# ilovepose/fast-human-pose-estimation.pytorch

Hardware: AMD Instinct MI355X
Metric: images/sec FPD train step (4-stack HG student, 8-stack teacher) 256x256 (higher is better)
Workload: dtype bf16; 1 GPU; configs[1]: hourglass student S=4 F=128 + teacher S=8 F=256, 256x256, batch 32/GPU, fused FPD step incl. Adam, teacher forward one batch ahead on a 2nd stream; global_batch=32, parallelism=dp1, backend=mfma, launch=one native plan call per phase, kernels launched eagerly on 3 streams, ranks=1, finite=True

## Files before the change

### fast-human-pose-estimation.pytorch_amd/csrc/api.hip

```cpp
#include <cstdarg>
#include <cstdio>
#include <cstdlib>
#include <cstring>
#include <string>
#include <vector>

#include "conv_dispatch.h"

int g_fpd_backend = FPD_BACKEND_MFMA;
static thread_local char g_err[512] = "";

static FILE* g_launch_log_file = nullptr;
static bool launch_log_open() {
    const char* path = getenv("FPD_LAUNCH_LOG");
    if (path == nullptr || path[0] == 0) return false;
    g_launch_log_file = fopen(path, "w");
    if (g_launch_log_file == nullptr) fprintf(stderr, "[fpd_amd] FPD_LAUNCH_LOG: cannot open %s\n", path);
    return g_launch_log_file != nullptr;
}
bool g_fpd_launch_log = launch_log_open();
static thread_local char g_op_tag[256] = "-";
void fpd_log_launch(const char* kernel, const dim3& grid, const dim3& block) {
    if (g_launch_log_file == nullptr) return;
    fprintf(g_launch_log_file, "%s\t%u\t%u\t%s\n", kernel, grid.x * grid.y * grid.z, block.x * block.y * block.z, g_op_tag);
// ... 16 lines not shown

static int validate_conv_dims(int N, int H, int W, int C, int K, int R, int S, int stride, int pad, int P, int Q) {
    FPD_REQUIRE(N > 0 && H > 0 && W > 0 && C > 0 && K > 0 && R > 0 && S > 0 && stride > 0 && pad >= 0,
                "conv: non-positive dimension");
    FPD_REQUIRE(P == (H + 2 * pad - R) / stride + 1 && Q == (W + 2 * pad - S) / stride + 1,
                "conv: output %dx%d inconsistent with input %dx%d k=%dx%d stride=%d pad=%d", P, Q, H, W, R, S, stride, pad);
    FPD_REQUIRE((int64_t)N * H * W * C < (1ll << 31) && (int64_t)N * P * Q * K < (1ll << 31), "conv: tensor too large for 32-bit indexing");
    return 0;
}

int fpd_bneck_blocks_option(int value);
int fpd_head_blocks_option(int value);

extern "C" {

const char* fpd_last_error(void) { return g_err; }
int fpd_abi_version(void) { return FPD_ABI_VERSION; }
int64_t fpd_stats_words(int32_t channels) { return FPD_STATS_WORDS(channels); }
int fpd_set_backend(int32_t backend) {
    const int prev = g_fpd_backend;
    if (backend == FPD_BACKEND_MFMA || backend == FPD_BACKEND_NAIVE || backend == FPD_BACKEND_MFMA_GENERIC) g_fpd_backend = backend;
    return prev;
}

static int g_wgrad_tile_only = 0;

int fpd_set_option(const char* name, int32_t value) {
    FPD_REQUIRE(name, "set_option: null name");
    if (!strcmp(name, "conv_pp")) return fpd_conv_pp_option(0, value);
    if (!strcmp(name, "conv_pp_blocks")) return fpd_conv_pp_option(1, value);
    if (!strcmp(name, "conv_c1")) return fpd_conv_c1_option(0, value);
    if (!strcmp(name, "conv_c1_blocks")) return fpd_conv_c1_option(1, value);
    if (!strcmp(name, "conv_c1_launches")) return fpd_conv_c1_option(2, value);
    if (!strcmp(name, "conv_c3")) return fpd_conv_c3_option(0, value);
    if (!strcmp(name, "conv_c3_blocks")) return fpd_conv_c3_option(1, value);
    if (!strcmp(name, "conv_c3_launches")) return fpd_conv_c3_option(2, value);
    if (!strcmp(name, "bneck_blocks")) return fpd_bneck_blocks_option(value);
    if (!strcmp(name, "head_blocks")) return fpd_head_blocks_option(value);
    if (!strcmp(name, "wgrad_tile_only")) { g_wgrad_tile_only = value; return 0; }
    return fpd_fail(-2, "set_option: unknown option '%s'", name);
}

int fpd_abi_sizeof(const char* n) {
#define SZ(T) if (!strcmp(n, #T)) return (int)sizeof(T)
    SZ(fpd_bn_t); SZ(fpd_conv_t); SZ(fpd_wgrad_t); SZ(fpd_stem_t); SZ(fpd_ew_t); SZ(fpd_loss_t); SZ(fpd_adam_t);
    SZ(fpd_wprep_entry_t); SZ(fpd_bnupd_entry_t); SZ(fpd_memset_t); SZ(fpd_table_t); SZ(fpd_wreduce_entry_t); SZ(fpd_bneck_t); SZ(fpd_conv_pair_t); SZ(fpd_bneck_pair_t); SZ(fpd_ew_pair_t); SZ(fpd_pck_t); SZ(fpd_head_t); SZ(fpd_affsum_t); SZ(fpd_layout_t);
    SZ(fpd_conv_f8_t); SZ(fpd_wquant_entry_t); SZ(fpd_flipmerge_t); SZ(fpd_finalpreds_t); SZ(fpd_targets_t); SZ(fpd_warp_src_t); SZ(fpd_warp_t);
    SZ(fpd_loss_ohkm_t); SZ(fpd_sgd_t);
#undef SZ
    return -1;
}

static int validate_conv(const fpd_conv_t* a) {
    FPD_REQUIRE(a && a->x && a->w && a->y, "conv: null pointer");
    int rc = validate_conv_dims(a->N, a->H, a->W, a->C, a->K, a->R, a->S, a->stride, a->pad, a->P, a->Q);
    if (rc) return rc;
    FPD_REQUIRE(a->dtype == FPD_F32 || a->dtype == FPD_BF16, "conv: bad dtype %d", a->dtype);
    FPD_REQUIRE(a->bn.mode == FPD_BN_NONE || (a->bn.gamma && a->bn.beta), "conv: BN prologue without gamma/beta");
    FPD_REQUIRE(a->bn.mode != FPD_BN_TRAIN || a->bn.stats, "conv: train-mode BN without statistics");
    FPD_REQUIRE(a->bn.mode != FPD_BN_EVAL || (a->bn.running_mean && a->bn.running_var), "conv: eval-mode BN without running stats");
    FPD_REQUIRE(a->epi == FPD_EPI_PLAIN || (a->epi_x && a->epi_stats && a->epi_bn.mode == FPD_BN_TRAIN && a->epi_bn.stats),
                "conv: BNRELU_BWD epilogue needs epi_x, epi_stats and a train-mode epi_bn");
    return 0;
}

constexpr unsigned ON_MFMA = 1u << FPD_BACKEND_MFMA, ON_GENERIC = ON_MFMA | 1u << FPD_BACKEND_MFMA_GENERIC, ON_ANY = ON_GENERIC | 1u << FPD_BACKEND_NAIVE;
struct ConvBackend {
    const char* name;
    unsigned backends;
    int (*route)(const fpd_conv_t& a, const fpd_conv_t* b, ConvAsk ask, ConvRoute& r);
    int (*launch)(const fpd_conv_t& a, const fpd_conv_t* b, hipStream_t st);
};
static const ConvBackend g_conv_backends[] = {
    {"conv_c1", ON_MFMA, fpd_conv_c1_route, fpd_conv_c1_launch},
    {"conv_c3", ON_MFMA, fpd_conv_c3_route, fpd_conv_c3_launch},
    {"conv_pp", ON_MFMA, fpd_conv_pp_route, fpd_conv_pp_launch},
    {"conv_tile", ON_MFMA, fpd_conv_tile_route, fpd_conv_tile_launch},
    {"conv_mfma", ON_GENERIC, nullptr, [](const fpd_conv_t& a, const fpd_conv_t*, hipStream_t st) { return fpd_conv_mfma_launch(a, st); }},
    {"conv_smallc", ON_GENERIC, nullptr, [](const fpd_conv_t& a, const fpd_conv_t*, hipStream_t st) { return fpd_conv_smallc_launch(a, st); }},
    {"conv_naive", ON_ANY, nullptr, [](const fpd_conv_t& a, const fpd_conv_t*, hipStream_t st) { return fpd_conv_naive_launch(a, st); }},
};
static bool eligible(unsigned backends) { return (backends >> g_fpd_backend & 1u) != 0; }

static const ConvBackend* route_conv(const fpd_conv_t& a, const fpd_conv_t* b, ConvAsk ask, ConvRoute& r) {
    r = ConvRoute{false, 0, 0};
    for (const ConvBackend& e : g_conv_backends) {
        if (!eligible(e.backends)) continue;
        if (e.route == nullptr ? b == nullptr : e.route(a, b, ask, r) == 0) return &e;
    }
    return nullptr;
}

static int launch_conv(const fpd_conv_t& a, const fpd_conv_t* b, hipStream_t st) {
    ConvRoute r;
    const ConvBackend* e = route_conv(a, b, fpd_conv_ask(a, b), r);
    if (e == nullptr) {
        const int rc = launch_conv(a, nullptr, st);
        return rc ? rc : launch_conv(*b, nullptr, st);
    }
    FPD_REQUIRE(!(a.wg_partial != nullptr && r.slabs_a == 0) && !(b != nullptr && b->wg_partial != nullptr && r.slabs_b == 0),
                "conv: the launch asks for a fused weight gradient (wg_partial), which its route (%s) does not offer; %s() reports 0 for it",
                e->name, b ? "fpd_conv_pair_fused_wgrad_partials" : "fpd_conv_fused_wgrad_partials");
    FPD_REQUIRE(r.folds || (a.fold_x == nullptr && (b == nullptr || b->fold_x == nullptr)),
                "conv: the launch asks for a folded BN-backward apply (fold_x), which its route (%s) does not offer; %s() reports 0 for it",
                e->name, b ? "fpd_conv_pair_fold_supported" : "fpd_conv_fold_supported");
    int rc = e->launch(a, b, st);
    for (++e; rc == 1 && e != std::end(g_conv_backends); ++e)
        if (e->route == nullptr && eligible(e->backends)) rc = e->launch(a, b, st);
    return rc;
}

int fpd_conv_forward(const fpd_conv_t* a, fpd_stream_t stream) {
    int rc = validate_conv(a);
    if (rc) return rc;
    rc = launch_conv(*a, nullptr, (hipStream_t)stream);
    return rc ? rc : check_launch();
}

int fpd_conv_fold_supported(const fpd_conv_t* a) {
    ConvRoute r;
    if (!a || validate_conv(a) != 0) return 0;
    route_conv(*a, nullptr, ConvAsk{true, a->wg_partial != nullptr}, r);
    return r.folds ? 1 : 0;
}
int fpd_conv_pair_fold_supported(const fpd_conv_pair_t* p) {
    ConvRoute r;
    if (!p || validate_conv(&p->a) != 0 || validate_conv(&p->b) != 0) return 0;
    if (route_conv(p->a, &p->b, ConvAsk{true, fpd_conv_ask(p->a, &p->b).wg}, r) != nullptr) return r.folds ? 1 : 0;
    return (fpd_conv_fold_supported(&p->a) && fpd_conv_fold_supported(&p->b)) ? 1 : 0;
}

int fpd_conv_fused_wgrad_partials(const fpd_conv_t* a) {
    ConvRoute r;
    if (!a || validate_conv(a) != 0) return 0;
    route_conv(*a, nullptr, ConvAsk{a->fold_x != nullptr, true}, r);
    return r.slabs_a;
}
int fpd_conv_pair_fused_wgrad_partials(const fpd_conv_pair_t* p, int32_t* n_a, int32_t* n_b) {
    FPD_REQUIRE(p && n_a && n_b, "conv_pair_fused_wgrad_partials: null pointer");
    *n_a = *n_b = 0;
    if (validate_conv(&p->a) != 0 || validate_conv(&p->b) != 0) return 0;
    ConvRoute r;
    route_conv(p->a, &p->b, ConvAsk{fpd_conv_ask(p->a, &p->b).fold, true}, r);
    *n_a = r.slabs_a; *n_b = r.slabs_b;
    return 0;
}

int fpd_conv_f8_in_domain(const fpd_conv_t* c) { return (c && fpd_conv_f8_domain(*c)) ? 1 : 0; }

int fpd_conv_forward_f8(const fpd_conv_f8_t* a, fpd_stream_t stream) {
    FPD_REQUIRE(a, "conv_f8: null pointer");
    int rc = validate_conv(&a->c);
    if (rc) return rc;
    FPD_REQUIRE(a->w8 && a->w8_scale, "conv_f8: null fp8 weights / scales");
    FPD_REQUIRE(((uintptr_t)a->w8 & 15) == 0, "conv_f8: w8 must be 16-byte aligned");
    rc = 1;
    if (g_fpd_backend == FPD_BACKEND_MFMA) rc = fpd_conv_tile_f8_launch(a->c, a->w8, a->w8_scale, (hipStream_t)stream);
    if (rc == 1) rc = launch_conv(a->c, nullptr, (hipStream_t)stream);
    return rc ? rc : check_launch();
}

int fpd_weight_quant_f8(const fpd_wquant_entry_t* t, int32_t n, fpd_stream_t stream) {
    FPD_REQUIRE(n == 0 || t != nullptr, "weight_quant_f8: null table");
    int rc = fpd_weight_quant_f8_launch(t, n, (hipStream_t)stream);
    return rc ? rc : check_launch();
}

int fpd_conv_forward_pair(const fpd_conv_pair_t* p, fpd_stream_t stream) {
    FPD_REQUIRE(p, "conv_pair: null pointer");
    int rc = validate_conv(&p->a);
    if (rc) return rc;
    rc = validate_conv(&p->b);
    if (rc) return rc;
    rc = launch_conv(p->a, &p->b, (hipStream_t)stream);
    return rc ? rc : check_launch();
}

static int validate_bneck_bns(const fpd_bneck_t* a) {
    const fpd_bn_t* bns[3] = {&a->bn1, &a->bn2, &a->bn3};
    for (int i = 0; i < 3; ++i)
        FPD_REQUIRE(bns[i]->mode == FPD_BN_EVAL && bns[i]->relu && bns[i]->gamma && bns[i]->beta && bns[i]->running_mean &&
                    bns[i]->running_var, "bottleneck: bn%d must be an eval-mode BN+ReLU with running statistics", i + 1);
    return 0;
}

int fpd_bottleneck_fold(const fpd_bneck_t* a, fpd_stream_t stream) {
    FPD_REQUIRE(a && a->folded, "bottleneck_fold: null pointer");
    int rc = validate_bneck_bns(a);
    if (rc) return rc;
    rc = fpd_bneck_fold_launch(*a, const_cast<float*>(a->folded), (hipStream_t)stream);
    if (rc == 1) return fpd_fail(-3, "bottleneck_fold: C=%d P=%d is outside the fused kernel's domain", a->C, a->P);
    return rc ? rc : check_launch();
}

int fpd_bottleneck_forward_pair(const fpd_bneck_pair_t* p, fpd_stream_t stream) {
    FPD_REQUIRE(p, "bottleneck_pair: null pointer");
    const fpd_bneck_t* ab[2] = {&p->a, &p->b};
    for (const fpd_bneck_t* a : ab) {
        FPD_REQUIRE(a->x && a->y && a->w1 && a->w2 && a->w3 && a->x != a->y, "bottleneck_pair: null pointer or y aliases x");
        FPD_REQUIRE((int64_t)a->N * a->H * a->W * a->C < ((int64_t)1 << 31), "bottleneck_pair: tensor too large for 32-bit indexing");
        int rc = validate_bneck_bns(a);
        if (rc) return rc;
    }
    int rc = fpd_bneck_fused_pair_launch(p->a, p->b, (hipStream_t)stream);
    if (rc == 1) {
        rc = fpd_bottleneck_forward(&p->a, stream);
// ... 23 lines not shown
};
static const WgradBackend g_wgrad_backends[] = {
    {ON_MFMA, fpd_wgrad_tile_partials, fpd_wgrad_tile_launch},
    {ON_GENERIC, fpd_wgrad_mfma_partials, fpd_wgrad_mfma_launch},
    {ON_GENERIC, fpd_wgrad_smallc_partials, fpd_wgrad_smallc_launch},
    {ON_ANY, fpd_wgrad_naive_partials, fpd_wgrad_naive_launch},
};

int fpd_conv_wgrad(const fpd_wgrad_t* a, fpd_stream_t stream) {
    FPD_REQUIRE(a && a->x && a->dy && a->dw, "wgrad: null pointer");
    int rc = validate_conv_dims(a->N, a->H, a->W, a->C, a->K, a->R, a->S, a->stride, a->pad, a->P, a->Q);
    if (rc) return rc;
    FPD_REQUIRE(a->dtype == FPD_F32 || a->dtype == FPD_BF16, "wgrad: bad dtype %d", a->dtype);
    FPD_REQUIRE(a->partial == nullptr || a->partial_stride >= (int64_t)a->K * a->R * a->S * a->C + a->K,
                "wgrad: partial_stride %lld smaller than weight + bias", (long long)a->partial_stride);
    rc = 1;
    for (const WgradBackend& e : g_wgrad_backends) {
        FPD_REQUIRE(!(g_wgrad_tile_only && &e != g_wgrad_backends), "wgrad: option wgrad_tile_only is set and the halo-tile kernel declines N=%d H=%d W=%d C=%d K=%d R=%d", a->N, a->H, a->W, a->C, a->K, a->R);
        if (eligible(e.backends)) rc = e.launch(*a, (hipStream_t)stream);
        if (rc != 1) break;
    }
    return rc ? rc : check_launch();
}

int fpd_wgrad_num_partials(const fpd_wgrad_t* a) {
    int n = 0;
    for (const WgradBackend& e : g_wgrad_backends)
        if (a && n == 0 && eligible(e.backends)) n = e.partials(*a);
    return n;
}

struct StemBackend {
    unsigned backends;
    int (*forward)(const fpd_stem_t& a, hipStream_t st);
    int (*wgrad_partials)(const fpd_stem_t& a);
    int (*wgrad)(const fpd_stem_t& a, hipStream_t st);
};
static const StemBackend g_stem_backends[] = {
    {ON_MFMA, fpd_stem_forward_s2d_launch, fpd_stem_wgrad_s2d_partials, fpd_stem_wgrad_s2d_launch},
    {ON_MFMA, fpd_stem_forward_mfma_launch, fpd_stem_wgrad_mfma_partials, fpd_stem_wgrad_mfma_launch},
    {ON_ANY, fpd_stem_forward_launch, fpd_stem_wgrad_partials, fpd_stem_wgrad_launch},
};

int fpd_stem_wgrad_num_partials(const fpd_stem_t* a) {
    int n = 0;
    for (const StemBackend& e : g_stem_backends)
        if (a && n == 0 && eligible(e.backends)) n = e.wgrad_partials(*a);
    return n;
}

int fpd_wgrad_reduce(const fpd_wreduce_entry_t* t, int32_t n, int64_t max_elems, fpd_stream_t stream) {
    int rc = fpd_wreduce_launch(t, n, max_elems, (hipStream_t)stream);
    return rc ? rc : check_launch();
}

int fpd_stem_forward(const fpd_stem_t* a, fpd_stream_t stream) {
    FPD_REQUIRE(a && a->x && a->w && a->bias && a->y, "stem: null pointer");
    FPD_REQUIRE(a->P == (a->H + 6 - 7) / 2 + 1 && a->Q == (a->W + 6 - 7) / 2 + 1, "stem: bad output size");
    int rc = 1;
    for (const StemBackend& e : g_stem_backends)
        if (rc == 1 && eligible(e.backends)) rc = e.forward(*a, (hipStream_t)stream);
    return rc ? rc : check_launch();
}

int fpd_stem_wgrad(const fpd_stem_t* a, fpd_stream_t stream) {
    FPD_REQUIRE(a && a->x && a->dy && a->dw, "stem wgrad: null pointer");
    FPD_REQUIRE(a->partial == nullptr || a->partial_stride >= (int64_t)a->K * 148, "stem wgrad: partial_stride %lld smaller than weight + bias",
                (long long)a->partial_stride);
    int rc = 1;
    for (const StemBackend& e : g_stem_backends)
        if (rc == 1 && eligible(e.backends)) rc = e.wgrad(*a, (hipStream_t)stream);
    return rc ? rc : check_launch();
}

int fpd_affsum(const fpd_affsum_t* a, fpd_stream_t stream) {
    FPD_REQUIRE(a && a->y, "affsum: null pointer");
    FPD_REQUIRE(a->nterms >= 1 && a->nterms <= FPD_AFFSUM_MAX, "affsum: %d terms (1..%d supported)", a->nterms, FPD_AFFSUM_MAX);
    FPD_REQUIRE(a->dtype == FPD_F32 || a->dtype == FPD_BF16, "affsum: bad dtype %d", a->dtype);
    for (int j = 0; j < a->nterms; ++j) {
        const int up = a->t[j].up;
        FPD_REQUIRE(a->t[j].x, "affsum: term %d has no input", j);
        FPD_REQUIRE((up == 1 || up == 2 || up == 4 || up == 8) && a->H % up == 0 && a->W % up == 0,
                    "affsum: term %d: up-sampling factor %d does not divide %dx%d", j, up, a->H, a->W);
        const fpd_bn_t& bn = a->t[j].bn;
        FPD_REQUIRE(bn.mode == FPD_BN_NONE || (bn.gamma && bn.beta), "affsum: term %d: BN without gamma/beta", j);
        FPD_REQUIRE(bn.mode != FPD_BN_TRAIN || bn.stats, "affsum: term %d: train-mode BN without statistics", j);
        FPD_REQUIRE(bn.mode != FPD_BN_EVAL || (bn.running_mean && bn.running_var), "affsum: term %d: eval-mode BN without running stats", j);
    }
    int rc = fpd_affsum_launch(*a, (hipStream_t)stream);
    return rc ? rc : check_launch();
}
// ... 227 lines not shown
    memcpy(&o.u, args, want);
    p->ops.push_back(o);
    p->sched.emplace_back();
    return (int)p->ops.size() - 1;
}

int fpd_plan_set_schedule(fpd_plan* p, int32_t op, int32_t lane, const int32_t* wait_ops, int32_t n_waits) {
    FPD_REQUIRE(p && op >= 0 && op < (int)p->ops.size(), "plan_set_schedule: bad op index %d", op);
    FPD_REQUIRE(lane >= 0 && lane < FPD_MAX_LANES, "plan_set_schedule: lane %d outside [0,%d)", lane, FPD_MAX_LANES);
    FPD_REQUIRE(n_waits >= 0 && (n_waits == 0 || wait_ops != nullptr), "plan_set_schedule: bad wait list");
    for (int i = 0; i < n_waits; ++i)
        FPD_REQUIRE(wait_ops[i] >= 0 && wait_ops[i] < op, "plan_set_schedule: op %d may only wait for earlier ops (got %d)", op, wait_ops[i]);
    fpd_sched& s = p->sched[op];
    s.lane = lane;
    s.waits.assign(wait_ops, wait_ops + n_waits);
    for (int i = 0; i < n_waits; ++i) p->sched[wait_ops[i]].record = true;
    return 0;
}

int fpd_plan_mark_event(fpd_plan* p, int32_t op) {
    FPD_REQUIRE(p && op >= 0 && op < (int)p->ops.size(), "plan_mark_event: bad op index %d", op);
    p->sched[op].record = true;
    return 0;
}

int fpd_plan_wait_op(fpd_plan* p, int32_t op, fpd_stream_t stream) {
    FPD_REQUIRE(p && op >= 0 && op < (int)p->ops.size(), "plan_wait_op: bad op index %d", op);
    FPD_REQUIRE(p->sched[op].record && p->sched[op].done, "plan_wait_op: op %d has no recorded event (mark it, then run its range)", op);
    FPD_CHECK_HIP(hipStreamWaitEvent((hipStream_t)stream, p->sched[op].done, 0));
    return 0;
}

static void conv_tag(char* p, size_t n, const char* what, const fpd_conv_t& c) {
    snprintf(p, n, "%s N=%d H=%d W=%d C=%d K=%d R=%d s=%d %s%s%s%s", what, c.N, c.H, c.W, c.C, c.K, c.R, c.stride,
             c.epi == FPD_EPI_BNRELU_BWD ? "dgrad" : "fwd", c.bn.mode == FPD_BN_EVAL ? " evalbn" : "", c.wg_partial ? " +wgrad" : "", c.fold_x ? " +fold" : "");
}
static void set_op_tag(int idx, const fpd_op& o) {
    char t[200] = "";
    static const char* ew_names[] = {"bnrelu_fwd", "bnrelu_bwd_r", "bn_bwd_apply", "maxpool_fwd", "maxpool_bwd", "upadd_fwd", "sumpool", "add", "relu_mask", "dilate2"};
    auto ewn = [&](int op) { return (op >= 0 && op < 10) ? ew_names[op] : "ew"; };
    switch (o.type) {
        case FPD_OP_CONV: conv_tag(t, sizeof(t), "conv", o.u.conv); break;
        case FPD_OP_CONV_F8: conv_tag(t, sizeof(t), "conv_f8", o.u.conv8.c); break;
        case FPD_OP_CONV_PAIR: {
            char a[90], b[90];
            conv_tag(a, sizeof(a), "conv2", o.u.pair.a);
            snprintf(b, sizeof(b), " | H=%d W=%d", o.u.pair.b.H, o.u.pair.b.W);
            snprintf(t, sizeof(t), "%s%s", a, b);
            break;
        }
        case FPD_OP_WGRAD: snprintf(t, sizeof(t), "wgrad N=%d H=%d W=%d C=%d K=%d R=%d s=%d", o.u.wgrad.N, o.u.wgrad.H, o.u.wgrad.W, o.u.wgrad.C, o.u.wgrad.K, o.u.wgrad.R, o.u.wgrad.stride); break;
        case FPD_OP_BNECK: snprintf(t, sizeof(t), "bneck N=%d H=%d W=%d C=%d P=%d", o.u.bneck.N, o.u.bneck.H, o.u.bneck.W, o.u.bneck.C, o.u.bneck.P); break;
        case FPD_OP_BNECK_PAIR: snprintf(t, sizeof(t), "bneck2 N=%d H=%d W=%d C=%d P=%d | H=%d W=%d", o.u.bpair.a.N, o.u.bpair.a.H, o.u.bpair.a.W, o.u.bpair.a.C, o.u.bpair.a.P, o.u.bpair.b.H, o.u.bpair.b.W); break;
        case FPD_OP_HEAD: snprintf(t, sizeof(t), "head N=%d H=%d W=%d C=%d J=%d", o.u.head.N, o.u.head.H, o.u.head.W, o.u.head.C, o.u.head.J); break;
        case FPD_OP_EW: snprintf(t, sizeof(t), "ew %s N=%d H=%d W=%d C=%d", ewn(o.u.ew.op), o.u.ew.N, o.u.ew.H, o.u.ew.W, o.u.ew.C); break;
        case FPD_OP_EW_PAIR: snprintf(t, sizeof(t), "ew2 %s N=%d H=%d W=%d C=%d | H=%d W=%d", ewn(o.u.epair.a.op), o.u.epair.a.N, o.u.epair.a.H, o.u.epair.a.W, o.u.epair.a.C, o.u.epair.b.H, o.u.epair.b.W); break;
        case FPD_OP_STEM_FWD: case FPD_OP_STEM_WGRAD: snprintf(t, sizeof(t), "%s N=%d H=%d W=%d K=%d", o.type == FPD_OP_STEM_FWD ? "stem_fwd" : "stem_wgrad", o.u.stem.N, o.u.stem.H, o.u.stem.W, o.u.stem.K); break;
        case FPD_OP_AFFSUM: snprintf(t, sizeof(t), "affsum N=%d H=%d W=%d C=%d terms=%d", o.u.affsum.N, o.u.affsum.H, o.u.affsum.W, o.u.affsum.C, o.u.affsum.nterms); break;
        case FPD_OP_LOSS: snprintf(t, sizeof(t), "loss B=%d J=%d H=%d W=%d S=%d", o.u.loss.B, o.u.loss.J, o.u.loss.H, o.u.loss.W, o.u.loss.S); break;
        case FPD_OP_LOSS_OHKM: snprintf(t, sizeof(t), "loss_ohkm B=%d J=%d H=%d W=%d S=%d k=%d,%d", o.u.lossk.base.B, o.u.lossk.base.J, o.u.lossk.base.H, o.u.lossk.base.W, o.u.lossk.base.S, o.u.lossk.topk_pose, o.u.lossk.topk_kd); break;
        case FPD_OP_ADAM: snprintf(t, sizeof(t), "adam n=%lld", (long long)o.u.adam.n); break;
        case FPD_OP_SGD: snprintf(t, sizeof(t), "sgd n=%lld momentum=%g wd=%g%s", (long long)o.u.sgd.n, (double)o.u.sgd.momentum, (double)o.u.sgd.weight_decay, o.u.sgd.nesterov ? " nesterov" : ""); break;
        case FPD_OP_WREDUCE: snprintf(t, sizeof(t), "wreduce entries=%d", o.u.table.n); break;
        case FPD_OP_WPREP: snprintf(t, sizeof(t), "wprep entries=%d", o.u.table.n); break;
        case FPD_OP_BNUPD: snprintf(t, sizeof(t), "bnupd entries=%d", o.u.table.n); break;
        default: snprintf(t, sizeof(t), "op%d", o.type); break;
    }
    snprintf(g_op_tag, sizeof(g_op_tag), "%d\t%s", idx, t);
}

static int run_op(const fpd_op& o, fpd_stream_t s) {
    switch (o.type) {
        case FPD_OP_CONV: return fpd_conv_forward(&o.u.conv, s);
        case FPD_OP_CONV_F8: return fpd_conv_forward_f8(&o.u.conv8, s);
        case FPD_OP_WQUANT: return fpd_weight_quant_f8((const fpd_wquant_entry_t*)o.u.table.table, o.u.table.n, s);
        case FPD_OP_WGRAD: return fpd_conv_wgrad(&o.u.wgrad, s);
        case FPD_OP_CONV_PAIR: return fpd_conv_forward_pair(&o.u.pair, s);
        case FPD_OP_BNECK_PAIR: return fpd_bottleneck_forward_pair(&o.u.bpair, s);
        case FPD_OP_EW_PAIR: return fpd_elementwise_pair(&o.u.epair, s);
        case FPD_OP_PCK: return fpd_pck(&o.u.pck, s);
        case FPD_OP_HEAD: return fpd_head_forward(&o.u.head, s);
        case FPD_OP_HEAD_FOLD: return fpd_head_fold(&o.u.head, s);
        case FPD_OP_BNECK: return fpd_bottleneck_forward(&o.u.bneck, s);
        case FPD_OP_BNECK_FOLD: return fpd_bottleneck_fold(&o.u.bneck, s);
        case FPD_OP_STEM_FWD: return fpd_stem_forward(&o.u.stem, s);
        case FPD_OP_STEM_WGRAD: return fpd_stem_wgrad(&o.u.stem, s);
        case FPD_OP_EW: return fpd_elementwise(&o.u.ew, s);
        case FPD_OP_LOSS: return fpd_loss(&o.u.loss, s);
        case FPD_OP_LOSS_OHKM: return fpd_loss_ohkm(&o.u.lossk, s);
        case FPD_OP_ADAM: return fpd_adam(&o.u.adam, s);
// ... 118 lines not shown
```

### fast-human-pose-estimation.pytorch_amd/csrc/conv_c1.hip

```cpp
#include <algorithm>
#include <cstdlib>
#include <type_traits>

#include "conv_dispatch.h"
#include "mfma_frag.h"

namespace {

constexpr int C1_NW = 8;

typedef short s16x2 __attribute__((ext_vector_type(2)));
__device__ __forceinline__ f32x2 c1_unpack(unsigned w) {
    f32x2 r = {__uint_as_float(w << 16), __uint_as_float(w & 0xffff0000u)};
    return r;
}
__device__ __forceinline__ unsigned c1_pack(f32x2 v) { return f2bf_pk(v[0], v[1]); }
__device__ __forceinline__ unsigned c1_floor(unsigned w, short lo) {
    s16x2 a = *reinterpret_cast<const s16x2*>(&w);
    const s16x2 b = {lo, lo};
    a = __builtin_elementwise_max(a, b);
    return *reinterpret_cast<const unsigned*>(&a);
}

template <int C, int K, bool BWD, bool WG>
struct C1Geo {
    static constexpr int CV = C / 8, KV = K / 8;
    static constexpr int NV = C / 16, NK = K / 16;
    static constexpr int KT = K / 32, KS = C / 16;
    static constexpr int PXA = C * 2 + 16, PXO = K * 2 + 16;
    static constexpr int TILE_A = 32 * PXA, TILE_O = 32 * PXO;
    static constexpr int WAVE_LDS = WG ? TILE_A + TILE_O : (TILE_A > TILE_O ? TILE_A : TILE_O);
    static constexpr int FLUSH = C1_NW * 64 * 16 * 4 + C1_NW * K * 4 + 8 * 2 * K * 8;
    static constexpr int REGION = C1_NW * WAVE_LDS > FLUSH ? C1_NW * WAVE_LDS : FLUSH;
    static constexpr int TABLES = (2 * C + (BWD ? 3 * C + 4 * K : 0) + K) * 4;
    static constexpr int LDS = TABLES + K * C * 2 + REGION;
    static constexpr int NT = (C / 32) * (K / 32);
    static constexpr int NTW = NT / C1_NW;
    static_assert(!WG || (BWD && NT % C1_NW == 0 && NTW >= 1), "fused weight gradient: every wave owns whole tiles of dW");
    static_assert(64 % CV == 0 && 64 % KV == 0, "a lane keeps its channel chunk");
};

#define C1_PHASE() do { asm volatile("" ::: "memory"); __builtin_amdgcn_sched_barrier(0); } while (0)

#ifdef FPD_C1_TIMING
#define C1_STAMP() do { if (lane == 0 && (wave == 0 || wave == 7) && c1_ns < 40) c1_stamp[(wave ? 40 : 0) + c1_ns++] = clock64(); } while (0)
#else
#define C1_STAMP() do { } while (0)
#endif

template <int C, int K, bool BWD, bool FOLD, bool WG, bool RES>
__device__ __forceinline__ void c1_body(const fpd_conv_t& a, const int bi, const int nblk) {
    using G = C1Geo<C, K, BWD, WG>;
    constexpr int CV = G::CV, KV = G::KV, NV = G::NV, NK = G::NK, KT = G::KT, KS = G::KS, PXA = G::PXA, PXO = G::PXO;
    constexpr int RPB = CV >= 16 ? 1 : 16 / CV;
    extern __shared__ __attribute__((aligned(16))) unsigned char smem[];

    const int tid = threadIdx.x, lane = tid & 63, l31 = lane & 31, hh = lane >> 5;
    const int wave = __builtin_amdgcn_readfirstlane(tid >> 6);
    const int M = a.N * a.H * a.W;
    const int ntile = M >> 5;
    const int nround = (ntile + C1_NW - 1) / C1_NW;
    const int r_beg = fpd_cut(bi, nround, nblk), r_end = fpd_cut(bi + 1, nround, nblk);

    float* s_scale = reinterpret_cast<float*>(smem);
    float* s_shift = s_scale + C;
    float* s_fold = s_shift + C;
    float* s_epi = s_fold + (BWD ? 3 * C : 0);
    float* s_bias = s_epi + (BWD ? 4 * K : 0);
    unsigned char* sW = reinterpret_cast<unsigned char*>(s_bias + K);
    unsigned char* sT = sW + K * C * 2;
    unsigned char* tA = sT + wave * G::WAVE_LDS;
    unsigned char* tO = WG ? tA + G::TILE_A : tA;

    const bf16_t* __restrict__ x = reinterpret_cast<const bf16_t*>(a.x);
    const bf16_t* __restrict__ w = reinterpret_cast<const bf16_t*>(a.w);
    bf16_t* y = reinterpret_cast<bf16_t*>(a.y);
    const bf16_t* res = reinterpret_cast<const bf16_t*>(a.residual);
    const bf16_t* ex = reinterpret_cast<const bf16_t*>(a.epi_x);
    const bf16_t* __restrict__ fx = reinterpret_cast<const bf16_t*>(a.fold_x != nullptr ? a.fold_x : a.x);
    const bool fold = FOLD && a.fold_x != nullptr;
    bf16_t* fo = fold ? reinterpret_cast<bf16_t*>(a.fold_out) : nullptr;
    const bool has_bn = !BWD && a.bn.mode != FPD_BN_NONE;
    constexpr bool has_res = RES;
    const bool want_stats = BWD || a.out_stats != nullptr;
    const bool wg = WG && a.wg_partial != nullptr;
    const bool wg_bias = wg && a.wg_bias;
#ifdef FPD_C1_TIMING
    long long* c1_stamp = reinterpret_cast<long long*>(smem + G::LDS);
    int c1_ns = 0;
#endif
    C1_STAMP();

    BnRaw braw;
    float bias_raw;
    const int te = tid - 128, tb = tid - 256;
    const bool r_bn = has_bn && tid < C;
    const bool r_fold = fold && tid < C;
    const bool r_epi = BWD && te >= 0 && te < K;
    const bool r_bias = tb >= 0 && tb < K;
    StatRaw fs1, fs2;
    if (r_bn) bn_request(a.bn, tid, C, braw);
    else if (r_fold) {
        bn_request(a.fold_bn, tid, C, braw);
        stat_request(a.fold_stats, C, 0, tid, fs1);
        stat_request(a.fold_stats, C, 1, tid, fs2);
    }
    else if (r_epi) bn_request(a.epi_bn, te, K, braw);
    else if (r_bias) { bias_raw = 0.f; if (a.bias != nullptr) bias_raw = a.bias[tb]; }
    __builtin_amdgcn_sched_barrier(0);

    uint4 rx[NV];
    uint4 ru[FOLD ? NV : 1];
    uint4 rr[NK];
    auto load_x = [&](int t) {
        const uint4* px = reinterpret_cast<const uint4*>(x) + ((size_t)t * 32 * CV + lane);
#pragma unroll
        for (int i = 0; i < NV; ++i) rx[i] = px[i * 64];
        if constexpr (FOLD) {
            const uint4* pu = reinterpret_cast<const uint4*>(fx) + ((size_t)t * 32 * CV + lane);
#pragma unroll
            for (int i = 0; i < NV; ++i) ru[i] = pu[i * 64];
        }
    };
    auto load_r = [&](int t) {
        const uint4* pr = reinterpret_cast<const uint4*>(BWD ? ex : res) + ((size_t)t * 32 * KV + lane);
#pragma unroll
        for (int i = 0; i < NK; ++i) rr[i] = pr[i * 64];
    };
    int tile = r_beg * C1_NW + wave;
    {
        constexpr int NWV = (K * CV + 511) / 512;
        uint4 rw[NWV];
#pragma unroll
        for (int i = 0; i < NWV; ++i) {
            const int v = tid + i * 512;
            rw[i] = make_uint4(0, 0, 0, 0);
            if (v < K * CV) rw[i] = *reinterpret_cast<const uint4*>(w + (size_t)v * 8);
        }
        __builtin_amdgcn_sched_barrier(0);
        {
            const int t0 = min(tile, ntile - 1);
            load_x(t0);
            if constexpr (BWD || has_res) load_r(t0);
        }
        __builtin_amdgcn_sched_barrier(0);
        if (r_bn) {
            float sc, sh, mu, is;
            bn_resolve(braw, (double)M, sc, sh, mu, is);
            s_scale[tid] = sc;
            s_shift[tid] = sh;
        } else if (r_fold) {
            const double s1 = stat_resolve(braw.s1), s2 = stat_resolve(braw.s2), b1 = stat_resolve(fs1), b2 = stat_resolve(fs2);
            const double cnt = (double)M, mu = s1 / cnt;
            double var = s2 / cnt - mu * mu;
            if (var < 0.0) var = 0.0;
            const double is = 1.0 / sqrt(var + (double)braw.eps), gi = (double)braw.g * is;
            const double m1 = b1 / cnt, m2 = b2 / cnt;
            s_fold[tid] = (float)gi;
            s_fold[C + tid] = (float)(-gi * is * m2);
            s_fold[2 * C + tid] = (float)(gi * (mu * is * m2 - m1));
            if (bi == 0) {
                if (a.fold_dgamma != nullptr) a.fold_dgamma[tid] = (float)b2;
                if (a.fold_dbeta != nullptr) a.fold_dbeta[tid] = (float)b1;
            }
        } else if (r_epi) {
            float sc, sh, mu, is;
            bn_resolve(braw, (double)M, sc, sh, mu, is);
            s_epi[te] = sc; s_epi[K + te] = sh; s_epi[2 * K + te] = mu; s_epi[3 * K + te] = is;
        } else if (r_bias) {
            s_bias[tb] = bias_raw;
        }
#pragma unroll
        for (int i = 0; i < NWV; ++i) {
            const int v = tid + i * 512;
            if (v < K * CV) {
                const int k = v / CV, ch = v % CV;
                const int sw = (k / RPB) & (CV - 1);
                *reinterpret_cast<uint4*>(sW + (k * CV + (ch ^ sw)) * 16) = rw[i];
            }
        }
    }
    C1_STAMP();
    __syncthreads();
    C1_STAMP();

    const int cch = lane % CV, kch = lane % KV;
    const int pxa0 = lane / CV, pxo0 = lane / KV;
    f32x2 p_sc[4], p_sh[4];
    if (has_bn) {
#pragma unroll
        for (int e = 0; e < 4; ++e) {
            p_sc[e] = *reinterpret_cast<const f32x2*>(s_scale + cch * 8 + 2 * e);
            p_sh[e] = *reinterpret_cast<const f32x2*>(s_shift + cch * 8 + 2 * e);
        }
    }
    const short relu_floor = a.bn.relu ? (short)0 : (short)-32768;
    const short epi_floor = a.epi_bn.relu ? (short)0 : (short)-32768;
    const float relu_gate = a.epi_bn.relu ? 0.f : -3.4e38f;
    f32x2 F1[4], F2[4], CS[4];
#pragma unroll
    for (int e = 0; e < 4; ++e) { F1[e] = f32x2{0.f, 0.f}; F2[e] = f32x2{0.f, 0.f}; CS[e] = f32x2{0.f, 0.f}; }
    const int wsw = (l31 / RPB) & (CV - 1);
    f32x16 wacc[WG ? G::NTW : 1], bacc[WG ? G::NTW : 1];
#pragma unroll
    for (int j = 0; j < (WG ? G::NTW : 1); ++j)
#pragma unroll
        for (int e = 0; e < 16; ++e) { wacc[j][e] = 0.f; bacc[j][e] = 0.f; }

    auto stage = [&](const int t, auto modec) {
        constexpr int MODE = decltype(modec)::value;
        f32x2 f_a[4], f_b[4], f_d[4];
// ... 3 lines not shown
                f_a[e] = *reinterpret_cast<const f32x2*>(s_fold + cch * 8 + 2 * e);
                f_b[e] = *reinterpret_cast<const f32x2*>(s_fold + C + cch * 8 + 2 * e);
                f_d[e] = *reinterpret_cast<const f32x2*>(s_fold + 2 * C + cch * 8 + 2 * e);
            }
        }
#pragma unroll
        for (int i = 0; i < NV; ++i) {
            uint4 val = rx[i];
            if constexpr (MODE == 2) {
                const uint4 uu = ru[i];
                const unsigned gw[4] = {val.x, val.y, val.z, val.w}, uw[4] = {uu.x, uu.y, uu.z, uu.w};
                unsigned ow[4];
#pragma unroll
                for (int e = 0; e < 4; ++e) {
                    const f32x2 tt = __builtin_elementwise_fma(f_b[e], c1_unpack(uw[e]), f_d[e]);
                    ow[e] = c1_pack(__builtin_elementwise_fma(f_a[e], c1_unpack(gw[e]), tt));
                }
                val = make_uint4(ow[0], ow[1], ow[2], ow[3]);
            } else if constexpr (MODE == 1) {
                val.x = c1_floor(c1_pack(__builtin_elementwise_fma(c1_unpack(val.x), p_sc[0], p_sh[0])), relu_floor);
                val.y = c1_floor(c1_pack(__builtin_elementwise_fma(c1_unpack(val.y), p_sc[1], p_sh[1])), relu_floor);
                val.z = c1_floor(c1_pack(__builtin_elementwise_fma(c1_unpack(val.z), p_sc[2], p_sh[2])), relu_floor);
                val.w = c1_floor(c1_pack(__builtin_elementwise_fma(c1_unpack(val.w), p_sc[3], p_sh[3])), relu_floor);
            }
            rx[i] = val;
            *reinterpret_cast<uint4*>(tA + (pxa0 + i * (64 / CV)) * PXA + cch * 16) = val;
        }
        if (MODE == 2 && fo != nullptr) {
            uint4* po = reinterpret_cast<uint4*>(fo) + ((size_t)t * 32 * CV + lane);
#pragma unroll
            for (int i = 0; i < NV; ++i) po[i * 64] = rx[i];
        }
    };
    auto finish = [&](const f32x16& accv, const int kt, auto resc) {
        constexpr bool HASRES = decltype(resc)::value;
        {
#pragma unroll
            for (int q = 0; q < 4; ++q) {
                unsigned char* p = tO + l31 * PXO + (kt * 32 + 8 * q + 4 * hh) * 2;
                f32x2 v0 = {accv[4 * q], accv[4 * q + 1]}, v1 = {accv[4 * q + 2], accv[4 * q + 3]};
                if constexpr (!BWD) {
                    if constexpr (HASRES) {
                        const uint2 r2 = *reinterpret_cast<const uint2*>(p);
                        v0 += c1_unpack(r2.x);
                        v1 += c1_unpack(r2.y);
                    }
                    const f32x4 b4 = *reinterpret_cast<const f32x4*>(s_bias + kt * 32 + 8 * q + 4 * hh);
                    v0 += f32x2{b4[0], b4[1]};
                    v1 += f32x2{b4[2], b4[3]};
                }
                *reinterpret_cast<uint2*>(p) = make_uint2(c1_pack(v0), c1_pack(v1));
            }
        }
    };
    auto perchan = [&](const int t, const bool first, auto statc) {
        constexpr bool STATS = decltype(statc)::value;
        uint4* py = reinterpret_cast<uint4*>(y) + ((size_t)t * 32 * KV + lane);
        f32x2 e_sc[4], e_sh[4], e_mu[4], e_is[4];
        if constexpr (BWD) {
#pragma unroll
            for (int e = 0; e < 4; ++e) {
                e_sc[e] = *reinterpret_cast<const f32x2*>(s_epi + kch * 8 + 2 * e);
                e_sh[e] = *reinterpret_cast<const f32x2*>(s_epi + K + kch * 8 + 2 * e);
                e_mu[e] = *reinterpret_cast<const f32x2*>(s_epi + 2 * K + kch * 8 + 2 * e);
                e_is[e] = *reinterpret_cast<const f32x2*>(s_epi + 3 * K + kch * 8 + 2 * e);
            }
        }
        if (!BWD && STATS && first) {
            const uint4 c4 = *reinterpret_cast<const uint4*>(tO + kch * 16);
            CS[0] = c1_unpack(c4.x); CS[1] = c1_unpack(c4.y); CS[2] = c1_unpack(c4.z); CS[3] = c1_unpack(c4.w);
        }
#pragma unroll
        for (int i = 0; i < NK; ++i) {
            unsigned char* p = tO + (pxo0 + i * (64 / KV)) * PXO + kch * 16;
            const uint4 o4 = *reinterpret_cast<const uint4*>(p);
            unsigned ow[4] = {o4.x, o4.y, o4.z, o4.w};
            if constexpr (BWD) {
                const unsigned xw[4] = {rr[i].x, rr[i].y, rr[i].z, rr[i].w};
                unsigned aw[4];
#pragma unroll
// ... 47 lines not shown
            for (int h = 0; h < 2; ++h) {
#pragma unroll
                for (int j = 0; j < (WG ? G::NTW : 1); ++j) {
                    wacc[j] = __builtin_amdgcn_mfma_f32_32x32x16_bf16(af[b][h][j], bfr[b][h][j], wacc[j], 0, 0, 0);
                    if constexpr (BIAS) bacc[j] = __builtin_amdgcn_mfma_f32_32x32x16_bf16(af[b][h][j], ones, bacc[j], 0, 0, 0);
                }
            }
        };
        if (round * C1_NW + C1_NW <= ntile) {
            wg_frags(0, af[0], bfr[0]);
#pragma unroll
            for (int s = 0; s < C1_NW; ++s) {
                if (s + 1 < C1_NW) wg_frags(s + 1, af[(s + 1) & 1], bfr[(s + 1) & 1]);
                mult(s & 1);
                __builtin_amdgcn_sched_barrier(0);
            }
        } else {
#pragma unroll 1
            for (int s = 0; s < C1_NW; ++s) {
                if (round * C1_NW + s < ntile) {
                    wg_frags(s, af[0], bfr[0]);
                    mult(0);
                }
            }
        }
    };

    bool first = true;
    for (int round = r_beg; round < r_end; ++round) {
        tile = round * C1_NW + wave;
        const bool live = tile < ntile;
        const bool pf = round + 1 < r_end && tile + C1_NW < ntile;
        if (live) {
            if (FOLD && fold) { if constexpr (FOLD) stage(tile, std::integral_constant<int, 2>{}); }
            else if (has_bn) { if constexpr (!BWD) stage(tile, std::integral_constant<int, 1>{}); }
            else stage(tile, std::integral_constant<int, 0>{});
            if (pf) load_x(tile + C1_NW);
            C1_PHASE();
            C1_STAMP();
            bf16x8 bf[KS];
#pragma unroll
            for (int kk = 0; kk < KS; ++kk) bf[kk] = *reinterpret_cast<const bf16x8*>(tA + l31 * PXA + kk * 32 + hh * 16);
            if constexpr (has_res) {
                C1_PHASE();
#pragma unroll
                for (int i = 0; i < NK; ++i)
                    *reinterpret_cast<uint4*>(tO + (pxo0 + i * (64 / KV)) * PXO + kch * 16) = make_uint4(rr[i].x, rr[i].y, rr[i].z, rr[i].w);
                C1_PHASE();
            }
#pragma unroll
            for (int k0 = 0; k0 < KT; k0 += 2) {
                f32x16 acc0, acc1;
#pragma unroll
                for (int e = 0; e < 16; ++e) { acc0[e] = 0.f; acc1[e] = 0.f; }
                const unsigned char* wrow0 = sW + (k0 * 32 + l31) * (C * 2);
#pragma unroll
                for (int kk = 0; kk < KS; ++kk) {
                    const bf16x8 wf0 = *reinterpret_cast<const bf16x8*>(wrow0 + ((2 * kk + hh) ^ wsw) * 16);
                    acc0 = __builtin_amdgcn_mfma_f32_32x32x16_bf16(wf0, bf[kk], acc0, 0, 0, 0);
                    if (k0 + 1 < KT) {
                        const bf16x8 wf1 = *reinterpret_cast<const bf16x8*>(wrow0 + 32 * (C * 2) + ((2 * kk + hh) ^ wsw) * 16);
                        acc1 = __builtin_amdgcn_mfma_f32_32x32x16_bf16(wf1, bf[kk], acc1, 0, 0, 0);
                    }
                }
                finish(acc0, k0, std::integral_constant<bool, has_res>{});
                if (k0 + 1 < KT) finish(acc1, k0 + 1, std::integral_constant<bool, has_res>{});
            }
            if constexpr (!BWD && has_res) { if (pf) load_r(tile + C1_NW); }
            C1_PHASE();
            C1_STAMP();
            if (want_stats) perchan(tile, first, std::true_type{}); else perchan(tile, first, std::false_type{});
            if (BWD && pf) load_r(tile + C1_NW);
            C1_PHASE();
            C1_STAMP();
            first = false;
        }
        if (WG) {
            __syncthreads();
            if (wg) {
                if (wg_bias && (wave % KT) == 0) wg_round(round, std::true_type{}); else wg_round(round, std::false_type{});
            }
            __syncthreads();
            C1_STAMP();
        }
    }
    C1_STAMP();

    if (WG && wg) {
        float* slab = a.wg_partial + (size_t)bi * a.wg_stride;
#pragma unroll
        for (int j = 0; j < (WG ? G::NTW : 1); ++j) {
            const int tw = wave + C1_NW * j, ci = tw / KT, ko = tw % KT;
#pragma unroll
            for (int e = 0; e < 16; ++e) {
                const int row = ci * 32 + (e & 3) + 8 * (e >> 2) + 4 * hh;
                slab[(size_t)row * K + ko * 32 + l31] = wacc[j][e];
                if (wg_bias && ko == 0 && l31 == 0) slab[(size_t)C * K + row] = bacc[j][e];
            }
        }
// ... 43 lines not shown
                    }
                }
                s_part[part * 2 * K + rem] = tot;
            }
        }
        __syncthreads();
        if (tid < 2 * K) {
            double tot = 0.0;
#pragma unroll
            for (int q = 0; q < NPART; ++q) tot += s_part[q * 2 * K + tid];
            stat_atomic_add(st, K, tid / K, tid % K, tot);
        }
    }
#ifdef FPD_C1_TIMING
    C1_STAMP();
    if (lane == 0 && (wave == 0 || wave == 7)) c1_stamp[(wave ? 40 : 0) + 39] = c1_ns;
    __syncthreads();
    if (tid == 0 && (blockIdx.x == 0 || blockIdx.x == gridDim.x / 2 + 1)) {
        for (int wv = 0; wv < 2; ++wv) {
            const long long* sp = c1_stamp + wv * 40;
            const long long t0 = c1_stamp[0];
            long long d[16];
            for (int q = 0; q < 16; ++q) d[q] = q < (int)sp[39] ? sp[q] - t0 : -1;
            printf("conv_c1 C=%d K=%d bwd %d fold %d wg %d blk %d wave %d rounds %d: %lld %lld %lld | %lld %lld %lld %lld | %lld %lld %lld %lld | %lld %lld %lld %lld %lld\n",
                   C, K, (int)BWD, (int)FOLD, (int)WG, (int)blockIdx.x, wv * 7, r_end - r_beg,
                   d[0], d[1], d[2], d[3], d[4], d[5], d[6], d[7], d[8], d[9], d[10], d[11], d[12], d[13], d[14], d[15]);
        }
    }
#endif
}

struct C1Args { fpd_conv_t c[2]; int nblk[2]; };

template <int C, int K, bool BWD, bool FOLD, bool WG, bool RES>
__global__ __launch_bounds__(512, 2) void c1_kernel(const C1Args p) {
    const int bid = blockIdx.x, n = gridDim.x, nb = p.nblk[1];
    const int fb0 = fpd_cut(bid, nb, n), fb1 = fpd_cut(bid + 1, nb, n);
    const int isb = fb1 > fb0 ? 1 : 0;
    const int u = isb ? fb0 : bid - fb0;
    c1_body<C, K, BWD, FOLD, WG, RES>(p.c[isb], u, p.nblk[isb]);
}

int g_c1_mode = -1, g_c1_blocks = -1;
std::atomic<int> g_c1_launches{0};
int c1_mode() {
    if (g_c1_mode < 0) { const char* e = getenv("FPD_C1"); g_c1_mode = e ? atoi(e) : 1; }
    return g_c1_mode;
}
int c1_blocks() {
    if (g_c1_blocks < 0) { const char* e = getenv("FPD_C1_BLOCKS"); g_c1_blocks = e ? atoi(e) : 192; }
    return g_c1_blocks < 1 ? 1 : g_c1_blocks;
}
int c1_min_px() {
    static int v = -1;
    if (v < 0) { const char* e = getenv("FPD_C1_MIN_PX"); v = e ? atoi(e) : 512; }
    return v;
}
int c1_min_px_bwd() {
    static int v = -1;
    if (v < 0) { const char* e = getenv("FPD_C1_MIN_PX_BWD"); v = e ? atoi(e) : 2048; }
    return v;
}
int c1_fuse_wgrad() { return 1; }

bool c1_chan(int c) { return c == 32 || c == 64 || c == 128; }
bool c1_aligned(const void* p) { return (reinterpret_cast<uintptr_t>(p) & 15) == 0; }

bool c1_domain(const fpd_conv_t& a, bool fold) {
    if (a.dtype != FPD_BF16 || a.R != 1 || a.S != 1 || a.stride != 1 || a.pad != 0 || a.P != a.H || a.Q != a.W) return false;
    if (!(c1_chan(a.C) || (a.C == 16 && a.K == 128)) || !c1_chan(a.K)) return false;
    const long long M = (long long)a.N * a.H * a.W;
    if (M % 32 != 0 || M > (1ll << 30)) return false;
    if (!c1_aligned(a.x) || !c1_aligned(a.y) || !c1_aligned(a.w) || !c1_aligned(a.residual) || !c1_aligned(a.epi_x) ||
        !c1_aligned(a.fold_x) || !c1_aligned(a.fold_out)) return false;
    if (a.epi == FPD_EPI_BNRELU_BWD) {
        if (a.bias != nullptr || a.residual != nullptr || a.bn.mode != FPD_BN_NONE) return false;
        if (a.C == 16) { if (fold) return false; }
        else if ((a.C / 32) * (a.K / 32) != C1_NW && !(a.C == 128 && a.K == 128 && !fold)) return false;
    } else {
        if (a.epi != FPD_EPI_PLAIN || a.y == a.x) return false;
    }
    return true;
}
int c1_rounds(const fpd_conv_t& a) { return cdiv(a.N * a.H * a.W / 32, C1_NW); }

struct C1Plan { int na, nb, grid; bool wg; };
bool c1_route(const fpd_conv_t& a, const fpd_conv_t* b, ConvAsk ask, ConvRoute& r, C1Plan& pl) {
    const int mode = c1_mode();
    if (mode == 0 || !c1_domain(a, ask.fold)) return false;
    const bool bwd = a.epi == FPD_EPI_BNRELU_BWD;
    long long px = (long long)a.N * a.H * a.W;
    if (b != nullptr) {
        if (!c1_domain(*b, ask.fold) || a.K != b->K || a.C != b->C || a.epi != b->epi) return false;
        if ((a.residual != nullptr) != (b->residual != nullptr)) return false;
        px += (long long)b->N * b->H * b->W;
    }
    if (mode == 1 && px < (bwd ? c1_min_px_bwd() : c1_min_px())) return false;
    const int ra = c1_rounds(a), rb = b ? c1_rounds(*b) : 0;
    int total = std::max(1, std::min(c1_blocks(), ra + rb));
    total = cdiv(ra + rb, cdiv(ra + rb, total));
    pl.nb = 0;
    if (b != nullptr) {
        if (total < 2) return false;
        pl.nb = std::max(1, std::min(total - 1, (int)((long long)total * rb / (ra + rb))));
    }
    pl.na = total - pl.nb;
    pl.grid = total;
    pl.wg = ask.wg && c1_fuse_wgrad() != 0 && bwd && (a.C / 32) * (a.K / 32) == C1_NW;
    r.folds = ask.fold && bwd;
    r.slabs_a = pl.wg ? pl.na : 0;
    r.slabs_b = pl.wg ? pl.nb : 0;
    return true;
}

template <int C, int K, bool BWD, bool FOLD, bool WG, bool RES>
int c1_launch_t(const fpd_conv_t& a, const fpd_conv_t* b, const C1Plan& pl, hipStream_t st) {
    static LdsAttr configured;
#ifdef FPD_C1_TIMING
    constexpr size_t lds = C1Geo<C, K, BWD, WG>::LDS + 1024;
#else
    constexpr size_t lds = C1Geo<C, K, BWD, WG>::LDS;
#endif
    static_assert(lds <= 160 * 1024, "conv_c1: LDS budget");
    if (int rc_ = configured.ensure(reinterpret_cast<const void*>(&c1_kernel<C, K, BWD, FOLD, WG, RES>), lds)) return rc_;
    C1Args args;
    args.c[0] = a; args.c[1] = b ? *b : a; args.nblk[0] = pl.na; args.nblk[1] = pl.nb;
    FPD_LAUNCH((c1_kernel<C, K, BWD, FOLD, WG, RES>), dim3(pl.grid), dim3(512), lds, st, args);
    g_c1_launches.fetch_add(1, std::memory_order_relaxed);
    return 0;
}

template <int C, int K>
int c1_launch_ck(const fpd_conv_t& a, const fpd_conv_t* b, const C1Plan& pl, hipStream_t st) {
    if (a.epi == FPD_EPI_BNRELU_BWD) {
        if constexpr ((C / 32) * (K / 32) == C1_NW) {
            if (a.fold_x != nullptr || (b != nullptr && b->fold_x != nullptr))
                return pl.wg ? c1_launch_t<C, K, true, true, true, false>(a, b, pl, st) : c1_launch_t<C, K, true, true, false, false>(a, b, pl, st);
            return pl.wg ? c1_launch_t<C, K, true, false, true, false>(a, b, pl, st) : c1_launch_t<C, K, true, false, false, false>(a, b, pl, st);
        } else if constexpr (C == 16 || (C == 128 && K == 128)) {
            return c1_launch_t<C, K, true, false, false, false>(a, b, pl, st);
        } else {
            return 1;
        }
    }
    if (a.residual != nullptr) return c1_launch_t<C, K, false, false, false, true>(a, b, pl, st);
    return c1_launch_t<C, K, false, false, false, false>(a, b, pl, st);
}

template <int C>
int c1_launch_c(const fpd_conv_t& a, const fpd_conv_t* b, const C1Plan& pl, hipStream_t st) {
    switch (a.K) {
        case 32: return c1_launch_ck<C, 32>(a, b, pl, st);
        case 64: return c1_launch_ck<C, 64>(a, b, pl, st);
        default: return c1_launch_ck<C, 128>(a, b, pl, st);
    }
}

}

int fpd_conv_c1_option(int which, int value) {
    if (which == 2) return g_c1_launches.load(std::memory_order_relaxed);
    int& g = which == 0 ? g_c1_mode : g_c1_blocks;
    const int prev = which == 0 ? c1_mode() : c1_blocks();
    g = value;
    return prev;
}

int fpd_conv_c1_route(const fpd_conv_t& a, const fpd_conv_t* b, ConvAsk ask, ConvRoute& r) {
    C1Plan pl;
    return c1_route(a, b, ask, r, pl) ? 0 : 1;
}
int fpd_conv_c1_launch(const fpd_conv_t& a, const fpd_conv_t* b, hipStream_t st) {
    ConvRoute r;
    C1Plan pl;
    if (!c1_route(a, b, fpd_conv_ask(a, b), r, pl)) return 1;
    if (int rc = fpd_conv_check_slabs(a, r.slabs_a, "conv_c1")) return rc;
    if (b != nullptr) {
        if (int rc = fpd_conv_check_slabs(*b, r.slabs_b, "conv_c1")) return rc;
        FPD_REQUIRE((a.wg_partial == nullptr) == (b->wg_partial == nullptr), "conv_pair: both or neither convolution of a pair take a fused weight gradient");
    }
    switch (a.C) {
        case 16: return c1_launch_ck<16, 128>(a, b, pl, st);
        case 32: return c1_launch_c<32>(a, b, pl, st);
        case 64: return c1_launch_c<64>(a, b, pl, st);
        default: return c1_launch_c<128>(a, b, pl, st);
    }
}
```

### fast-human-pose-estimation.pytorch_amd/csrc/conv_c3.hip

```cpp
#include <algorithm>
#include <atomic>
#include <cstdlib>
#include <type_traits>

#include "conv_dispatch.h"

namespace {

constexpr int C3_NW = 8, C3_C = 64, C3_STRIP = 256;
constexpr int C3_CV = C3_C / 8;
constexpr int C3_NVH = 6;
constexpr int C3_NK = C3_C / 16;
constexpr int C3_WBYTES = 9 * C3_C * C3_C * 2;
constexpr int C3_TILE_O = 32 * C3_C * 2;
constexpr int C3_TABLES = (2 * C3_C + 3 * C3_C + 4 * C3_C + C3_C) * 4;
constexpr int C3_FLUSH = C3_NW * 64 * 16 * 4 + C3_NW * C3_C * 4 + 8 * 2 * C3_C * 8;

typedef short s16x2 __attribute__((ext_vector_type(2)));
typedef unsigned u32x4 __attribute__((ext_vector_type(4)));
__device__ __forceinline__ f32x2 c3_unpack(unsigned w) {
    f32x2 r = {__uint_as_float(w << 16), __uint_as_float(w & 0xffff0000u)};
    return r;
}
__device__ __forceinline__ unsigned c3_pack(f32x2 v) { return f2bf_pk(v[0], v[1]); }
// ... 420 lines not shown
    return g;
}
struct C3Plan { C3Geo ga, gb; int grid; size_t lds; };
bool c3_plan(const fpd_conv_t& a, const fpd_conv_t* b, C3Plan& pl) {
    pl.ga = c3_geo(a);
    pl.gb = b ? c3_geo(*b) : pl.ga;
    pl.gb.nblk = 0;
    const int sa = pl.ga.nstrip, sb = b ? pl.gb.nstrip : 0;
    int total = std::max(1, std::min(c3_blocks(), sa + sb));
    total = cdiv(sa + sb, cdiv(sa + sb, total));
    if (b != nullptr) {
        if (total < 2) return false;
        pl.gb.nblk = std::max(1, std::min(total - 1, (int)((long long)total * sb / (sa + sb))));
    }
    pl.ga.nblk = total - pl.gb.nblk;
    pl.grid = total;
    const int img = std::max(pl.ga.img_bytes, b ? pl.gb.img_bytes : 0);
    pl.ga.img_bytes = pl.gb.img_bytes = img;
    pl.lds = (size_t)C3_TABLES + C3_WBYTES + std::max(img + C3_NW * C3_TILE_O, C3_FLUSH);
    return pl.lds <= 160 * 1024;
}

template <bool BWD, bool FOLD>
int c3_launch_t(const fpd_conv_t& a, const fpd_conv_t* b, const C3Plan& pl, hipStream_t st) {
    static LdsAttr configured;
    if (int rc_ = configured.ensure(reinterpret_cast<const void*>(&c3_kernel<BWD, FOLD>), pl.lds)) return rc_;
    C3Args args;
    args.c[0] = a; args.c[1] = b ? *b : a; args.g[0] = pl.ga; args.g[1] = pl.gb;
    FPD_LAUNCH((c3_kernel<BWD, FOLD>), dim3(pl.grid), dim3(512), pl.lds, st, args);
    g_c3_launches.fetch_add(1, std::memory_order_relaxed);
    return 0;
}
bool c3_route(const fpd_conv_t& a, const fpd_conv_t* b, ConvAsk ask, ConvRoute& r, C3Plan& pl) {
    if (!c3_takes(a, b) || !c3_plan(a, b, pl)) return false;
    r = ConvRoute{ask.fold && a.epi == FPD_EPI_BNRELU_BWD, 0, 0};
    return true;
}

}

int fpd_conv_c3_option(int which, int value) {
    if (which == 2) return g_c3_launches.load(std::memory_order_relaxed);
    int& g = which == 0 ? g_c3_mode : g_c3_blocks;
    const int prev = which == 0 ? c3_mode() : c3_blocks();
    g = value;
    return prev;
}
int fpd_conv_c3_route(const fpd_conv_t& a, const fpd_conv_t* b, ConvAsk ask, ConvRoute& r) {
    C3Plan pl;
    return c3_route(a, b, ask, r, pl) ? 0 : 1;
}
int fpd_conv_c3_launch(const fpd_conv_t& a, const fpd_conv_t* b, hipStream_t st) {
    ConvRoute r;
    C3Plan pl;
    if (!c3_route(a, b, fpd_conv_ask(a, b), r, pl)) return 1;
    if (a.epi != FPD_EPI_BNRELU_BWD) return c3_launch_t<false, false>(a, b, pl, st);
    return r.folds ? c3_launch_t<true, true>(a, b, pl, st) : c3_launch_t<true, false>(a, b, pl, st);
}
```

### fast-human-pose-estimation.pytorch_amd/csrc/conv_dispatch.h

```cpp
#pragma once
#include "common.h"

struct ConvAsk { bool fold, wg; };
struct ConvRoute { bool folds; int slabs_a, slabs_b; };
inline ConvAsk fpd_conv_ask(const fpd_conv_t& a, const fpd_conv_t* b) {
    return ConvAsk{a.fold_x != nullptr || (b != nullptr && b->fold_x != nullptr), a.wg_partial != nullptr || (b != nullptr && b->wg_partial != nullptr)};
}
inline int fpd_conv_check_slabs(const fpd_conv_t& c, int slabs, const char* unit) {
    if (c.wg_partial == nullptr) return 0;
    FPD_REQUIRE(c.wg_stride >= (int64_t)c.C * c.K + c.C, "conv: wg_stride %lld smaller than weight + bias", (long long)c.wg_stride);
    FPD_REQUIRE(c.wg_count == slabs, "conv: the launch writes %d weight-gradient slabs but the caller sized its workspace for %d "
                "(fpd_conv_fused_wgrad_partials: has a %s option changed since?)", slabs, c.wg_count, unit);
    return 0;
}
int fpd_conv_c1_route(const fpd_conv_t& a, const fpd_conv_t* b, ConvAsk ask, ConvRoute& r);
int fpd_conv_c1_launch(const fpd_conv_t& a, const fpd_conv_t* b, hipStream_t st);
int fpd_conv_c3_route(const fpd_conv_t& a, const fpd_conv_t* b, ConvAsk ask, ConvRoute& r);
int fpd_conv_c3_launch(const fpd_conv_t& a, const fpd_conv_t* b, hipStream_t st);
int fpd_conv_pp_route(const fpd_conv_t& a, const fpd_conv_t* b, ConvAsk ask, ConvRoute& r);
int fpd_conv_pp_launch(const fpd_conv_t& a, const fpd_conv_t* b, hipStream_t st);
int fpd_conv_tile_route(const fpd_conv_t& a, const fpd_conv_t* b, ConvAsk ask, ConvRoute& r);
int fpd_conv_tile_launch(const fpd_conv_t& a, const fpd_conv_t* b, hipStream_t st);
int fpd_conv_c1_option(int which, int value);
int fpd_conv_c3_option(int which, int value);
int fpd_conv_pp_option(int which, int value);
int fpd_conv_mfma_launch(const fpd_conv_t& a, hipStream_t st);
int fpd_conv_smallc_launch(const fpd_conv_t& a, hipStream_t st);
int fpd_conv_naive_launch(const fpd_conv_t& a, hipStream_t st);
bool fpd_conv_f8_domain(const fpd_conv_t& a);
int fpd_conv_tile_f8_launch(const fpd_conv_t& a, const void* w8, const float* wscale, hipStream_t st);
int fpd_weight_quant_f8_launch(const fpd_wquant_entry_t* table, int n, hipStream_t st);

int fpd_wgrad_tile_partials(const fpd_wgrad_t& a);
int fpd_wgrad_tile_launch(const fpd_wgrad_t& a, hipStream_t st);
int fpd_wgrad_mfma_partials(const fpd_wgrad_t& a);
int fpd_wgrad_mfma_launch(const fpd_wgrad_t& a, hipStream_t st);
int fpd_wgrad_smallc_partials(const fpd_wgrad_t& a);
int fpd_wgrad_smallc_launch(const fpd_wgrad_t& a, hipStream_t st);
int fpd_wgrad_naive_partials(const fpd_wgrad_t& a);
int fpd_wgrad_naive_launch(const fpd_wgrad_t& a, hipStream_t st);
int fpd_wreduce_launch(const fpd_wreduce_entry_t* table, int n, int64_t max_elems, hipStream_t st);

int fpd_stem_forward_s2d_launch(const fpd_stem_t& a, hipStream_t st);
int fpd_stem_wgrad_s2d_partials(const fpd_stem_t& a);
int fpd_stem_wgrad_s2d_launch(const fpd_stem_t& a, hipStream_t st);
int fpd_stem_forward_mfma_launch(const fpd_stem_t& a, hipStream_t st);
int fpd_stem_wgrad_mfma_partials(const fpd_stem_t& a);
int fpd_stem_wgrad_mfma_launch(const fpd_stem_t& a, hipStream_t st);
int fpd_stem_forward_launch(const fpd_stem_t& a, hipStream_t st);
int fpd_stem_wgrad_partials(const fpd_stem_t& a);
int fpd_stem_wgrad_launch(const fpd_stem_t& a, hipStream_t st);

int fpd_bneck_fused_launch(const fpd_bneck_t& a, hipStream_t st);
int fpd_bneck_fused_pair_launch(const fpd_bneck_t& a, const fpd_bneck_t& b, hipStream_t st);
int fpd_bneck_fold_launch(const fpd_bneck_t& a, float* out, hipStream_t st);
int fpd_head_fused_launch(const fpd_head_t& a, hipStream_t st);
int fpd_head_fold_launch(const fpd_head_t& a, float* out, hipStream_t st);
int fpd_pck_launch(const fpd_pck_t& a, hipStream_t st);
int fpd_flip_w_launch(const float* x, float* y, int64_t rows, int W, hipStream_t st);
int fpd_flip_merge_launch(const fpd_flipmerge_t& p, hipStream_t st);
int fpd_final_preds_launch(const fpd_finalpreds_t& p, hipStream_t st);
int fpd_render_targets_launch(const fpd_targets_t& a, hipStream_t st);
int fpd_warp_affine_launch(const fpd_warp_t& a, hipStream_t st);
int fpd_elementwise_launch(const fpd_ew_t& a, hipStream_t st);
int fpd_elementwise_pair_launch(const fpd_ew_t& a, const fpd_ew_t& b, hipStream_t st);
int fpd_affsum_launch(const fpd_affsum_t& a, hipStream_t st);
int fpd_loss_launch(const fpd_loss_t& a, hipStream_t st);
int fpd_loss_ohkm_launch(const fpd_loss_ohkm_t& a, hipStream_t st);
int64_t fpd_loss_ohkm_scratch_size(const fpd_loss_t& a);
int fpd_adam_launch(const fpd_adam_t& a, hipStream_t st);
int fpd_sgd_launch(const fpd_sgd_t& a, hipStream_t st);
int fpd_weight_prep_launch(const fpd_wprep_entry_t* table, int n, int64_t max_elems, int dtype, hipStream_t st);
int fpd_bn_update_running_launch(const fpd_bnupd_entry_t* table, int n, hipStream_t st);
int fpd_cast_launch(const void* src, void* dst, int64_t n, int sd, int dd, hipStream_t st);
int fpd_nchw_to_nhwc_launch(const float* src, void* dst, int N, int C, int H, int W, int dtype, hipStream_t st);
int fpd_nhwc_to_nchw_launch(const void* src, float* dst, int N, int C, int H, int W, int dtype, hipStream_t st);
// ... 1 lines not shown
```

### fast-human-pose-estimation.pytorch_amd/csrc/conv_pp.hip

```cpp
#include <algorithm>
#include <cstdlib>
#include <type_traits>

#include "conv_dispatch.h"
#include "conv_epilogue.h"
#include "mfma_frag.h"

namespace {

constexpr int pp_ilog2(int v) { return v <= 1 ? 0 : 1 + pp_ilog2(v / 2); }

struct PPGeo {
    int nrows;
    int ntiles;
    int nblk;
    int region;
    unsigned mW, mWV, mH;
};
__device__ __forceinline__ int pp_qdiv(int v, unsigned magic) { return (int)__umulhi((unsigned)v, magic); }
static inline unsigned pp_magic(int d) { return (unsigned)((0x100000000ull / (unsigned long long)d) + 1ull); }

__device__ __forceinline__ int pp_fresh(int v) {
    asm volatile("" : "+v"(v));
    return v;
// ... 690 lines not shown

template <int R, int C, int KH, bool BWD, bool WG>
static int pp_launch_t(const fpd_conv_t& a, const fpd_conv_t* b, const PPPlan& pl, hipStream_t st) {
    static LdsAttr configured;
    if (int rc_ = configured.ensure(reinterpret_cast<const void*>(&conv_pp_kernel<R, C, KH, BWD, WG>), pl.lds)) return rc_;
    PPArgs args;
    args.c[0] = a; args.c[1] = b ? *b : a; args.g[0] = pl.ga; args.g[1] = pl.gb; args.ks = pl.ks;
    FPD_LAUNCH((conv_pp_kernel<R, C, KH, BWD, WG>), dim3(pl.grid), dim3(512), pl.lds, st, args);
    return 0;
}

template <int R, int C>
static int pp_launch_c(const fpd_conv_t& a, const fpd_conv_t* b, const PPPlan& pl, hipStream_t st) {
    const bool bwd = a.epi == FPD_EPI_BNRELU_BWD;
    if constexpr (R == 1 && C >= 32) {
        if (pl.wg) return a.K > 32 ? pp_launch_t<R, C, 2, true, true>(a, b, pl, st) : pp_launch_t<R, C, 1, true, true>(a, b, pl, st);
    }
    if (a.K > 32) return bwd ? pp_launch_t<R, C, 2, true, false>(a, b, pl, st) : pp_launch_t<R, C, 2, false, false>(a, b, pl, st);
    return bwd ? pp_launch_t<R, C, 1, true, false>(a, b, pl, st) : pp_launch_t<R, C, 1, false, false>(a, b, pl, st);
}

static bool pp_takes(const fpd_conv_t& a, const fpd_conv_t* b) {
    const int mode = pp_mode();
    if (mode == 0 || !pp_domain(a)) return false;
    int tiles = pp_tiles(a);
    if (b != nullptr) {
        if (!pp_domain(*b) || a.K != b->K || a.C != b->C || a.R != b->R || a.epi != b->epi) return false;
        tiles += pp_tiles(*b);
    }
    return mode != 1 || tiles >= pp_min_tiles();
}

static bool pp_route(const fpd_conv_t& a, const fpd_conv_t* b, ConvAsk ask, ConvRoute& r, PPPlan& pl) {
    if (!pp_takes(a, b) || !pp_plan(a, b, ask, pl)) return false;
    auto foldable = [](const fpd_conv_t& c) { return c.epi == FPD_EPI_BNRELU_BWD && c.bn.mode == FPD_BN_NONE; };
    PPPlan other;
    r.folds = ask.fold && foldable(a) && (b == nullptr || foldable(*b)) &&
              (!(pp_wg_shape(a) && (b == nullptr || pp_wg_shape(*b))) || pp_plan(a, b, ConvAsk{ask.fold, !ask.wg}, other));
    r.slabs_a = pl.wg ? pl.ga.nblk : 0;
    r.slabs_b = pl.wg ? pl.gb.nblk : 0;
    return true;
}

}

int fpd_conv_pp_option(int which, int value) {
    int& g = which == 0 ? g_pp_mode : g_pp_blocks;
    const int prev = which == 0 ? pp_mode() : pp_blocks();
    g = value;
    return prev;
}

int fpd_conv_pp_route(const fpd_conv_t& a, const fpd_conv_t* b, ConvAsk ask, ConvRoute& r) {
    PPPlan pl;
    return pp_route(a, b, ask, r, pl) ? 0 : 1;
}
int fpd_conv_pp_launch(const fpd_conv_t& a, const fpd_conv_t* b, hipStream_t st) {
    ConvRoute r;
    PPPlan pl;
    if (!pp_route(a, b, fpd_conv_ask(a, b), r, pl)) return 1;
    if (int rc = fpd_conv_check_slabs(a, r.slabs_a, "conv_pp")) return rc;
    if (b != nullptr) if (int rc = fpd_conv_check_slabs(*b, r.slabs_b, "conv_pp")) return rc;
    if (a.R == 3) {
        if (a.C == 64) return pp_launch_c<3, 64>(a, b, pl, st);
        if (a.C == 32) return pp_launch_c<3, 32>(a, b, pl, st);
        return pp_launch_c<3, 16>(a, b, pl, st);
    }
// ... 8 lines not shown
```

### fast-human-pose-estimation.pytorch_amd/csrc/conv_tile.hip

```cpp
#include <algorithm>
#include <cstdlib>

#include "conv_dispatch.h"
#include "conv_epilogue.h"

namespace {

template <typename T>
struct TapMma;
template <>
struct TapMma<bf16_t> {
    template <int TN, int BK, int LD>
    static __device__ __forceinline__ void run(const bf16_t* arow, const bf16_t* sB, int lane, f32x16* acc) {
        const int koff = 8 * (lane >> 5);
        const bf16_t* brow = sB + (lane & 31) * LD + koff;
#pragma unroll
        for (int kk = 0; kk < BK / 16; ++kk) {
            const bf16x8 a = *reinterpret_cast<const bf16x8*>(arow + kk * 16 + koff);
#pragma unroll
            for (int tn = 0; tn < TN; ++tn) {
                const bf16x8 b = *reinterpret_cast<const bf16x8*>(brow + tn * 32 * LD + kk * 16);
                acc[tn] = __builtin_amdgcn_mfma_f32_32x32x16_bf16(a, b, acc[tn], 0, 0, 0);
            }
        }
// ... 339 lines not shown

constexpr size_t LDS_MAX = 160 * 1024;
static int tile_rows(int W) { return std::max(1, 128 / W); }
static int tiles_of(const fpd_conv_t& a) { return cdiv(a.N * a.H, tile_rows(a.W)); }
template <typename T, int BK>
static TileGeo make_geo(const fpd_conv_t& a) {
    constexpr int VPR = BK / DT<T>::VEC;
    TileGeo g;
    g.nrows = tile_rows(a.W);
    g.mW = magic_of(a.W);
    g.mWV = magic_of(a.W * VPR);
    return g;
}

static int tile_tn(int K, int mt) {
    int tn = K > 64 ? 4 : (K > 32 ? 2 : 1);
    while (tn > 1 && mt * cdiv(K, 32 * tn) < 128) tn >>= 1;
    return tn;
}

static bool tile_domain(const fpd_conv_t& a) {
    if ((long long)a.N * a.H * a.W * a.C >= (1ll << 31)) return false;
    if (a.stride != 1 || a.R != a.S || (a.R != 1 && a.R != 3) || a.pad != (a.R - 1) / 2) return false;
    if (a.P != a.H || a.Q != a.W || a.W > 128 || a.W < 2) return false;
    if (a.C % 16 != 0 || a.C > FPD_MAXC) return false;
    if (a.epi == FPD_EPI_BNRELU_BWD && a.K > FPD_MAXC) return false;
    return true;
}
static bool halo_fits(const fpd_conv_t& a, int vpr) { return (tile_rows(a.W) + a.R - 1) * a.W * vpr <= 2048; }

struct TilePlan { int esz, bk, tn, tiles; bool allw, fold; size_t lds; };

static bool tile_route(const fpd_conv_t& a, const fpd_conv_t* b, ConvAsk ask, ConvRoute& r, TilePlan& pl) {
    if (!tile_domain(a)) return false;
    if (b != nullptr && (!tile_domain(*b) || a.dtype != b->dtype || a.K != b->K || a.C != b->C || a.R != b->R)) return false;
    pl.esz = a.dtype == FPD_BF16 ? 2 : 4;
    const int vec = 16 / pl.esz;
    auto fits = [&](int bk) { return halo_fits(a, bk / vec) && (b == nullptr || halo_fits(*b, bk / vec)); };
    pl.bk = pl.esz == 2 ? 64 : 32;
    while (a.C % pl.bk != 0) pl.bk >>= 1;
    if (pl.esz == 2 && b == nullptr)
        while (pl.bk > 16 && !fits(pl.bk)) pl.bk >>= 1;
    if (!fits(pl.bk)) return false;
    pl.tiles = tiles_of(a) + (b ? tiles_of(*b) : 0);
    pl.tn = tile_tn(a.K, pl.tiles);
    const bool bwd = a.epi == FPD_EPI_BNRELU_BWD || (b != nullptr && b->epi == FPD_EPI_BNRELU_BWD);
    const int LD = pl.bk + vec;
    auto lds_of = [&](bool allw) {
        auto halo = [&](const fpd_conv_t& c) {
            return (size_t)((tile_rows(c.W) + c.R - 1) * (c.W + c.R - 1) + 3) * LD * pl.esz + (size_t)(allw ? 9 : 2) * 32 * pl.tn * LD * pl.esz;
        };
        const size_t epi = std::max((size_t)128 * (32 * pl.tn + 4) * sizeof(float), (size_t)4 * 32 * pl.tn * 2 * sizeof(double));
        return (size_t)((bwd ? 5 : 2) * a.C + 4 * 32 * pl.tn) * sizeof(float) + std::max({halo(a), b ? halo(*b) : (size_t)0, epi});
    };
    pl.allw = (pl.bk == 64 || (pl.bk == 32 && pl.esz == 4)) && a.R == 3 && a.C == pl.bk &&
              pl.tiles * cdiv(a.K, 32 * pl.tn) <= allw_max_blocks() && lds_of(true) <= LDS_MAX;
    pl.lds = lds_of(pl.allw);
    if (pl.lds > LDS_MAX) return false;
    auto foldable = [](const fpd_conv_t& c) { return c.epi == FPD_EPI_BNRELU_BWD && c.bn.mode == FPD_BN_NONE && c.C <= 128 && c.K <= 128; };
    pl.fold = ask.fold && pl.tn <= 2 && foldable(a) && (b == nullptr || foldable(*b));
    r = ConvRoute{pl.fold, 0, 0};
    return true;
}

template <typename T, int TN, int BK, bool ALLW>
int launch_tile_v(const fpd_conv_t& a, const fpd_conv_t* bp, const TilePlan& pl, hipStream_t st) {
    const size_t lds = pl.lds;
// ... 60 lines not shown
```

### fast-human-pose-estimation.pytorch_amd/csrc/stem_s2d.hip

```cpp
#include <algorithm>
#include <cstdlib>

#include "common.h"

namespace {

constexpr int S2_PIXB = 48;
constexpr int S2_WROW = 16 * 16 * 2 + 16;
constexpr int S2_NV = 4;

#ifdef S2_TIMING
__shared__ long long s2_stamp[48];
__shared__ int s2_ns;
#define S2_STAMP() do { if (threadIdx.x == 0 && blockIdx.x == 0 && s2_ns < 48) s2_stamp[s2_ns++] = clock64(); } while (0)
#else
#define S2_STAMP() do { } while (0)
#endif

template <int TN>
__global__ __launch_bounds__(256) void stem_s2d_fwd_kernel(const fpd_stem_t a, const int logQ, const int ntiles) {
    extern __shared__ __attribute__((aligned(16))) unsigned char smem[];
    const int tid = threadIdx.x, lane = tid & 63, wave = __builtin_amdgcn_readfirstlane(tid >> 6);
    const int l31 = lane & 31, hh = lane >> 5;
    const int K = a.K, P = a.P, Q = a.Q, H = a.H, W = a.W;
    const int rows = 128 >> logQ, QP = Q + 3, RING = 2 * rows + 3;
    const unsigned RSs = (unsigned)QP * S2_PIXB, RINGB = (unsigned)RING * RSs;
    const int M = a.N * P * Q;
    unsigned char* sS = smem;
    unsigned char* sW = sS + RINGB;
    const float* __restrict__ x = a.x;
    auto wrap = [&](unsigned v) { return min(v, v - RINGB); };

#ifdef S2_TIMING
    if (threadIdx.x == 0) s2_ns = 0;
    __syncthreads();
#endif
    S2_STAMP();
    const int t_beg = fpd_cut((int)blockIdx.x, ntiles, (int)gridDim.x), t_end = fpd_cut((int)blockIdx.x + 1, ntiles, (int)gridDim.x);
    if (t_beg >= t_end) return;

    {
        const int e = tid, tap = e >> 4, ch = e & 15;
        const int kr = tap >> 2, ks = tap & 3, dx = ch & 1, dc = ch >> 1, dy = dc >= 3 ? 1 : 0, cch = dc - 3 * dy;
        const int r = 2 * kr + dy - 1, s_ = 2 * ks + dx - 1;
        const bool tap_ok = ch < 12 && r >= 0 && s_ >= 0;
        const int woff = tap_ok ? (r * 7 + s_) * 3 + cch : 0;
        float wv[32 * TN];
#pragma unroll
        for (int k = 0; k < 32 * TN; ++k) wv[k] = a.w[(unsigned)(min(k, K - 1) * 147 + woff)];
#pragma unroll
        for (int k = 0; k < 32 * TN; ++k) *reinterpret_cast<bf16_t*>(sW + k * S2_WROW + tap * 32 + ch * 2) = f2bf((tap_ok && k < K) ? wv[k] : 0.f);
    }
// ... 18 lines not shown
            int rl[8], dcv[8], ccv[8];
#pragma unroll
            for (int i = 0; i < 8; ++i) {
                const int idx = min(base + tid + i * 256, total - 1);
                rl[i] = idx / per_row;
                const int rem = idx - rl[i] * per_row;
                dcv[i] = rem / QP; ccv[i] = rem - dcv[i] * QP;
                v[i] = s_load(n, R0 + rl[i], dcv[i], ccv[i]);
            }
#pragma unroll
            for (int i = 0; i < 8; ++i)
                if (base + tid + i * 256 < total) s_row_store(n, R0 + rl[i], dcv[i], ccv[i], v[i]);
        }
    };
    int v_rl[S2_NV], v_dc[S2_NV], v_cc[S2_NV];
    const int per_row = 6 * QP, nnew = rows * per_row;
#pragma unroll
    for (int i = 0; i < S2_NV; ++i) {
        const int idx = min(tid + i * 256, nnew - 1);
        v_rl[i] = idx / per_row;
        const int rem = idx - v_rl[i] * per_row;
        v_dc[i] = rem / QP;
        v_cc[i] = rem - v_dc[i] * QP;
    }
    float2 pv0, pv1, pv2, pv3;
#define S2_PREF(i, PV, n_, R0_) PV = (tid + i * 256 < nnew) ? s_load(n_, (R0_) + v_rl[i], v_dc[i], v_cc[i]) : make_float2(0.f, 0.f);
#define S2_PUT(i, PV, n_, R0_) if (tid + i * 256 < nnew) s_row_store(n_, (R0_) + v_rl[i], v_dc[i], v_cc[i], PV);

    const int ml = wave * 32 + l31, ti = ml >> logQ, tj = ml & (Q - 1);
    const unsigned a_lane = (unsigned)tj * S2_PIXB + (unsigned)hh * 16;
    const unsigned char* wrow = sW + l31 * S2_WROW + hh * 16;

    bf16_t* __restrict__ y = reinterpret_cast<bf16_t*>(a.y);
    const bool want_stats = a.out_stats != nullptr;
    f32x4 bias4[TN][4], f1[TN][4], f2[TN][4];
#pragma unroll
    for (int tn = 0; tn < TN; ++tn)
#pragma unroll
        for (int j = 0; j < 4; ++j) {
            const int k = 32 * tn + 8 * j + 4 * hh;
            bias4[tn][j] = (k < K) ? f32x4{a.bias[k], a.bias[k + 1], a.bias[k + 2], a.bias[k + 3]} : f32x4{0.f, 0.f, 0.f, 0.f};
            f1[tn][j] = f32x4{0.f, 0.f, 0.f, 0.f};
            f2[tn][j] = f32x4{0.f, 0.f, 0.f, 0.f};
        }

    int ring_n = -1, ring_hi = 0;
    bool pref = false;
    for (int t = t_beg; t < t_end; ++t) {
        const int g0 = t * rows, n = g0 / P, p0 = g0 - n * P;
        S2_STAMP();
        __syncthreads();
        if (pref && n == ring_n && p0 + 3 == ring_hi) {
            S2_PUT(0, pv0, n, ring_hi) S2_PUT(1, pv1, n, ring_hi) S2_PUT(2, pv2, n, ring_hi) S2_PUT(3, pv3, n, ring_hi)
        } else {
            full_load(n, p0, p0 + rows + 3);
        }
        ring_n = n; ring_hi = p0 + rows + 3;
        S2_STAMP();
        __syncthreads();
        pref = false;
        if (t + 1 < t_end && p0 + rows < P) {
            S2_PREF(0, pv0, n, ring_hi) S2_PREF(1, pv1, n, ring_hi) S2_PREF(2, pv2, n, ring_hi) S2_PREF(3, pv3, n, ring_hi)
            pref = true;
        }
        S2_STAMP();
        f32x16 acc[TN];
#pragma unroll
        for (int tn = 0; tn < TN; ++tn)
#pragma unroll
            for (int e = 0; e < 16; ++e) acc[tn][e] = 0.f;
        const unsigned r0 = (unsigned)((p0 + ti) % RING) * RSs;
#pragma unroll
        for (int kr = 0; kr < 4; ++kr) {
            const unsigned char* arow = sS + wrap(r0 + (unsigned)kr * RSs) + a_lane;
#pragma unroll
            for (int ks = 0; ks < 4; ++ks) {
                const bf16x8 av = *reinterpret_cast<const bf16x8*>(arow + ks * S2_PIXB);
#pragma unroll
                for (int tn = 0; tn < TN; ++tn) {
                    const bf16x8 bv = *reinterpret_cast<const bf16x8*>(wrow + tn * 32 * S2_WROW + (kr * 4 + ks) * 32);
                    acc[tn] = __builtin_amdgcn_mfma_f32_32x32x16_bf16(bv, av, acc[tn], 0, 0, 0);
                }
            }
        }
        S2_STAMP();
        bf16_t* yrow = y + (size_t)(t * 128 + ml) * K + 4 * hh;
#pragma unroll
        for (int tn = 0; tn < TN; ++tn)
#pragma unroll
            for (int j = 0; j < 4; ++j) {
                if (32 * tn + 8 * j < K) {
                    const f32x4 b = bias4[tn][j];
                    const float v0 = acc[tn][4 * j] + b[0], v1 = acc[tn][4 * j + 1] + b[1], v2 = acc[tn][4 * j + 2] + b[2], v3 = acc[tn][4 * j + 3] + b[3];
                    const unsigned p0 = f2bf_pk(v0, v1), p1 = f2bf_pk(v2, v3);
                    *reinterpret_cast<uint2*>(yrow + 32 * tn + 8 * j) = make_uint2(p0, p1);
                    if (want_stats) {
                        const f32x4 d = {__uint_as_float(p0 << 16) - b[0], __uint_as_float(p0 & 0xffff0000u) - b[1],
                                         __uint_as_float(p1 << 16) - b[2], __uint_as_float(p1 & 0xffff0000u) - b[3]};
                        f1[tn][j] += d;
                        f2[tn][j] = __builtin_elementwise_fma(d, d, f2[tn][j]);
                    }
                }
            }
    }
    if (want_stats) {
        float* s_t = reinterpret_cast<float*>(smem);
        __syncthreads();
#pragma unroll
        for (int tn = 0; tn < TN; ++tn)
#pragma unroll
            for (int j = 0; j < 4; ++j)
#pragma unroll
                for (int i = 0; i < 4; ++i) {
                    const int k = 32 * tn + 8 * j + 4 * hh + i;
                    s_t[((wave * 32 * TN + k) * 2 + 0) * 33 + l31] = f1[tn][j][i];
                    s_t[((wave * 32 * TN + k) * 2 + 1) * 33 + l31] = f2[tn][j][i];
                }
        __syncthreads();
        double* s_red2 = reinterpret_cast<double*>(s_t + 4 * 32 * TN * 2 * 33);
        for (int task = tid; task < 4 * 32 * TN * 2; task += 256) {
            float tot = 0.f;
#pragma unroll 8
            for (int l = 0; l < 32; ++l) tot += s_t[task * 33 + l];
            s_red2[task] = (double)tot;
        }
        __syncthreads();
        if (tid < K) {
// ... 174 lines not shown
        __syncthreads();
        for (int id = tid; id < 2 * 16 * 64; id += 256) {
            const int t2 = id >> 10, e = (id >> 6) & 15, l = id & 63;
            float sum = s_red[((0 * 2 + t2) * 16 + e) * 64 + l];
#pragma unroll
            for (int w = 1; w < 4; ++w) sum += s_red[((w * 2 + t2) * 16 + e) * 64 + l];
            const int k = (e & 3) + 8 * (e >> 2) + 4 * (l >> 5), col = l & 31;
            const int ks = t2 + 2 * (col >> 4), ch = col & 15, dx = ch & 1, dc = ch >> 1, dyy = dc >= 3 ? 1 : 0, c = dc - 3 * dyy;
            const int r = 2 * kr + dyy - 1, sx = 2 * ks + dx - 1;
            if (k < K && ch < 12 && r >= 0 && sx >= 0) {
                const size_t idx = ((size_t)(k * 7 + r) * 7 + sx) * 3 + c;
                if (slab != nullptr) slab[idx] = sum; else a.dw[idx] += sum;
            }
        }
    }
    if (do_bias) {
        __syncthreads();
        if ((lane & 15) < 2) {
#pragma unroll
            for (int e = 0; e < 4; ++e) s_red[wave * 32 + 16 * (lane & 15) + 4 * (lane >> 4) + e] = accb[e];
        }
        __syncthreads();
        if (tid < K) {
            float tot = 0.f;
#pragma unroll
            for (int w = 0; w < 4; ++w) tot += s_red[w * 32 + tid];
            if (slab != nullptr) slab[(size_t)K * 147 + tid] = tot; else a.dbias[tid] += tot;
        }
    }
}

}

int fpd_stem_forward_s2d_launch(const fpd_stem_t& a, hipStream_t st) {
    if (a.dtype != FPD_BF16 || a.K % 8 != 0 || a.K > 64) return 1;
    if (a.Q > 128 || a.Q < 16 || (a.Q & (a.Q - 1)) != 0 || a.H != 2 * a.P || a.W != 2 * a.Q) return 1;
    int logQ = 0;
    while ((1 << logQ) < a.Q) ++logQ;
    const int rows = 128 >> logQ;
    if (a.P % rows != 0) return 1;
    const int TN = a.K > 32 ? 2 : 1;
    const int ring = 2 * rows + 3;
    const size_t lds = std::max((size_t)ring * (a.Q + 3) * S2_PIXB + (size_t)32 * TN * S2_WROW,
                                (size_t)4 * 32 * TN * 2 * (33 * sizeof(float) + sizeof(double)));
    const int tiles = a.N * a.P * a.Q / 128;
    static const int cap = 0;
    const int blocks = std::max(1, std::min(tiles, cap > 0 ? cap : (TN == 1 ? 512 : 256)));
    static LdsAttr cfg1, cfg2;
    if (TN == 1) {
        if (int rc_ = cfg1.ensure(reinterpret_cast<const void*>(&stem_s2d_fwd_kernel<1>), lds)) return rc_;
        FPD_LAUNCH((stem_s2d_fwd_kernel<1>), dim3(blocks), dim3(256), lds, st, a, logQ, tiles);
    } else {
        if (int rc_ = cfg2.ensure(reinterpret_cast<const void*>(&stem_s2d_fwd_kernel<2>), lds)) return rc_;
        FPD_LAUNCH((stem_s2d_fwd_kernel<2>), dim3(blocks), dim3(256), lds, st, a, logQ, tiles);
    }
    return 0;
}

static bool s2d_wgrad_ok(const fpd_stem_t& a, int& logQ, int& blocks) {
    if (a.dtype != FPD_BF16 || a.K % 8 != 0 || a.K > 32) return false;
    if (a.Q > 128 || a.Q < 16 || (a.Q & (a.Q - 1)) != 0 || a.H != 2 * a.P || a.W != 2 * a.Q) return false;
    logQ = 0;
    while ((1 << logQ) < a.Q) ++logQ;
    if (a.P % (128 >> logQ) != 0) return false;
    const int tiles = a.N * a.P * a.Q / 128;
    static const int cap = 256;
    blocks = std::max(1, std::min(tiles, cap));
    return true;
}

int fpd_stem_wgrad_s2d_partials(const fpd_stem_t& a) {
    int logQ, blocks;
    return s2d_wgrad_ok(a, logQ, blocks) ? blocks : 0;
}

int fpd_stem_wgrad_s2d_launch(const fpd_stem_t& a, hipStream_t st) {
    int logQ, blocks;
    if (!s2d_wgrad_ok(a, logQ, blocks)) return 1;
    if (a.partial == nullptr) blocks = 1;
    const int rows = 128 >> logQ, ring = 2 * rows + 3;
    const size_t lds = std::max((size_t)ring * (a.Q + 3) * S2_PIXB + (size_t)128 * 64 + 1024, (size_t)4 * 2 * 16 * 64 * sizeof(float));
    const int tiles = a.N * a.P * a.Q / 128;
    static LdsAttr cfg;
    if (int rc_ = cfg.ensure(reinterpret_cast<const void*>(&stem_s2d_wgrad_kernel), lds)) return rc_;
    FPD_LAUNCH(stem_s2d_wgrad_kernel, dim3(blocks), dim3(256), lds, st, a, logQ, tiles);
    return 0;
}
// ... 1 lines not shown
```

### fast-human-pose-estimation.pytorch_amd/executor.py

```python
import ctypes as C
import os

import torch

from . import graph as G
from . import runtime as R
from .schedule import PhaseSchedule

_EW = {'bnrelu_fwd': R.EW_BNRELU_FWD, 'bnrelu_bwd_r': R.EW_BNRELU_BWD_R, 'bn_bwd_apply': R.EW_BN_BWD_APPLY,
       'maxpool_fwd': R.EW_MAXPOOL_FWD, 'maxpool_bwd': R.EW_MAXPOOL_BWD, 'upadd_fwd': R.EW_UPADD_FWD,
       'sumpool': R.EW_SUMPOOL, 'add': R.EW_ADD, 'relu_mask': R.EW_RELU_MASK, 'dilate2': R.EW_DILATE2}
_ARENA_DTYPE = {'param': torch.float32, 'grad': torch.float32, 'rstat': torch.float32, 'nbt': torch.int64,
                'stats': torch.int64, 'losses': torch.float64, 'image': torch.float32, 'target': torch.float32,
                'weight': torch.float32, 'adam_m': torch.float32, 'adam_v': torch.float32, 'fold': torch.float32,
                'w8': torch.uint8, 'w8s': torch.float32, 'ohkm_scratch': torch.float64, 'ohkm_masks': torch.int32}


def act_torch_dtype(dtype):
    return torch.bfloat16 if dtype == R.BF16 else torch.float32


_STAT_HI, _STAT_LO = float(2 ** 20), float(2 ** 60)


# ... 85 lines not shown

    def __init__(self, arenas, dtype):
        self.A, self.dtype = arenas, dtype
        self.keep = []
        self.use_partials = False
        self.partials, self.partial_elems = {}, 0
        self.fused = set()
        self.reduces = []

    def bn(self, bn):
        s = R.BnT()
        if bn is None:
            s.mode = R.BN_NONE
            return s
        s.mode = R.BN_TRAIN if bn.mode == 'train' else R.BN_EVAL
        s.relu = 1 if bn.relu else 0
        s.eps = G.BN_EPS
        s.stats = self.A.ptr(bn.stats) if bn.mode == 'train' else None
        s.gamma, s.beta = self.A.ptr(bn.gamma), self.A.ptr(bn.beta)
        s.running_mean, s.running_var = self.A.ptr(bn.rmean), self.A.ptr(bn.rvar)
        return s

    def conv(self, op, plain=False):
        s = R.ConvT()
        (s.N, s.H, s.W, s.C, s.K, s.R, s.S, s.stride, s.pad, s.P, s.Q) = op.dims
        s.dtype = self.dtype
        s.epi = R.EPI_BNRELU_BWD if op.epi == 'bnrelu_bwd' else R.EPI_PLAIN
        p = self.A.ptr
        s.x, s.w, s.bias, s.residual, s.y = p(_abuf(op.x)), p(op.w), p(op.bias), p(_abuf(op.residual)), p(_abuf(op.y))
        s.out_stats = p(op.out_stats)
        s.bn = self.bn(op.bn)
        s.epi_x, s.epi_bn, s.epi_stats = p(_abuf(op.epi_x)), self.bn(op.epi_bn), p(op.epi_stats)
        s.wg_partial, s.wg_stride, s.wg_bias, s.wg_count = None, 0, 0, 0
        if not plain and getattr(op, 'fused_wgrad', None) is not None and self.use_partials:
            n = R.lib().fpd_conv_fused_wgrad_partials(C.byref(s))
            if n > 0:
                self._fuse_wgrad(op, s, n)
        if not plain:
            self._fill_fold(op, s)
        if getattr(op, 'w8', None) is not None and not plain:
            f = R.ConvF8T()
            f.c, f.w8, f.w8_scale = s, p(op.w8), p(op.w8s)
            return R.OP_CONV_F8, f
        return R.OP_CONV, s

    def plan_folds(self, ops):
        if os.environ.get('FPD_FOLD_APPLY', '1') == '0':
            return
        l = R.lib()
        members_of = lambda top: [m for m in ((top.a, top.b) if top.kind in ('conv2', 'ew2', 'bneck2') else (top,)) if m is not None]
        for i, op in enumerate(ops):
            if op is None or op.kind not in ('conv', 'conv2'):
                continue
            members = members_of(op)
            cands = [m for m in members if getattr(m, 'fold_apply', None) is not None and not getattr(m.fold_apply, 'folded', False)]
            if not cands or any(getattr(m, 'w8', None) is not None for m in members):
                continue
            early = False
            for m in cands:
                y = _abuf(m.fold_apply.y)
                own = (id(m), id(m.fold_apply), id(getattr(m, 'fold_wgrad', None)))
                m.fold_other_readers = False
                for j, top in enumerate(ops):
                    if top is None:
                        continue
                    for o in members_of(top):
                        if id(o) in own or not any(_abuf(t) is y for t in o.acts_in()):
                            continue
                        if j < i:
                            early = True
                        m.fold_other_readers = True
            if early:
                continue
            if op.kind == 'conv2':
                ps = R.ConvPairT()
                ps.a, ps.b = self.conv(op.a, plain=True)[1], self.conv(op.b, plain=True)[1]
                ok = l.fpd_conv_pair_fold_supported(C.byref(ps)) == 1
            else:
                ok = l.fpd_conv_fold_supported(C.byref(self.conv(op, plain=True)[1])) == 1
            if ok:
                for m in cands:
                    m.fold_active = True
                    m.fold_apply.folded = True

    def _fill_fold(self, op, s):
        if not getattr(op, 'fold_active', False):
            return
        ap, p = op.fold_apply, self.A.ptr
        assert ap.add is None and _abuf(ap.y) is _abuf(op.x), 'fold: the apply must produce exactly this operand'
        s.x = p(_abuf(ap.dy))
        s.fold_x, s.fold_bn, s.fold_stats = p(_abuf(ap.x)), self.bn(ap.bn), p(ap.bstats)
        s.fold_dgamma, s.fold_dbeta = p(ap.dgamma), p(ap.dbeta)
        skip = getattr(op, 'fused_active', False) and not getattr(op, 'fold_other_readers', False)
        s.fold_out = None if skip else p(_abuf(ap.y))

    def _fuse_wgrad(self, op, s, n):
        fw = op.fused_wgrad
        numel = fw.dw.numel
        assert numel == s.C * s.K, (numel, s.C, s.K)
        stride = (numel + s.C + 63) // 64 * 64
        self.partials[id(fw)] = [s, fw.dw, numel, stride, n, self.partial_elems, fw.dbias, s.C]
        self.partial_elems += n * stride
        s.wg_bias = 1 if fw.dbias is not None else 0
        s.wg_count = n
        self.fused.add(id(fw))
        op.fused_active = True

    def wquant(self, entries):
        ents = []
        for w, q, sc in entries:
            e = R.WquantEntryT()
            e.w, e.w8, e.scale = self.A.ptr(w), self.A.ptr(q), self.A.ptr(sc)
            e.K, e.RSC = w.shape[0], w.numel // w.shape[0]
            ents.append(e)
        s = R.TableT()
        s.table, s.n, s.dtype, s.max_elems = self._table(ents, R.WquantEntryT), len(ents), self.dtype, 0
# ... 54 lines not shown
        ws = torch.empty(self.partial_elems, dtype=torch.float32, device=self.A.device)
        self.keep.append(ws)
        for s, dw, numel, stride, n, off, dbias, nbias in self.partials.values():
            if isinstance(s, R.ConvT):
                s.wg_partial, s.wg_stride = ws.data_ptr() + 4 * off, stride
            else:
                s.partial, s.partial_stride = ws.data_ptr() + 4 * off, stride
        for op, t in self.reduces:
            ents, mx = [], 0
            for w in op.wgrads:
                rec = self.partials.get(id(w))
                if rec is None:
                    continue
                s, dw, numel, stride, n, off, dbias, nbias = rec
                base = ws.data_ptr() + 4 * off
                e = R.WreduceEntryT()
                e.partial, e.dw, e.n, e.stride, e.count = base, self.A.ptr(dw), numel, stride, n
                ents.append(e)
                if dbias is not None:
                    e = R.WreduceEntryT()
                    e.partial, e.dw, e.n, e.stride, e.count = base + 4 * numel, self.A.ptr(dbias), nbias, stride, n
                    ents.append(e)
                mx = max(mx, numel)
            t.table, t.n, t.dtype, t.max_elems = self._table(ents, R.WreduceEntryT), len(ents), self.dtype, mx

    def stem(self, op):
        s = R.StemT()
        (s.N, s.H, s.W, s.K, s.P, s.Q) = op.dims
        s.dtype = self.dtype
        p = self.A.ptr
        s.x = p(op.image)
        if op.kind == 'stem_fwd':
            s.w, s.bias, s.y, s.out_stats = p(op.w), p(op.bias), p(_abuf(op.y)), p(op.out_stats)
            return R.OP_STEM_FWD, s
        s.dy, s.dw, s.dbias = p(_abuf(op.dy)), p(op.dw), p(op.dbias)
        s.partial, s.partial_stride = None, 0
        if self.use_partials:
            n = R.lib().fpd_stem_wgrad_num_partials(C.byref(s))
            if n > 0:
                numel = op.dw.numel
                stride = (numel + s.K + 63) // 64 * 64
                self.partials[id(op)] = [s, op.dw, numel, stride, n, self.partial_elems, op.dbias, s.K]
                self.partial_elems += n * stride
        return R.OP_STEM_WGRAD, s

    def ew(self, op):
        if getattr(op, 'folded', False):
            return R.OP_NOP, R.MemsetT()
        s = R.EwT()
        s.op, s.dtype = _EW[op.op], self.dtype
        (s.N, s.H, s.W, s.C) = op.dims
        p = self.A.ptr
        s.x, s.x2, s.dy, s.add, s.y = p(_abuf(op.x)), p(_abuf(op.x2)), p(_abuf(op.dy)), p(_abuf(op.add)), p(_abuf(op.y))
        s.out_stats, s.bstats, s.dgamma, s.dbeta = p(op.out_stats), p(op.bstats), p(op.dgamma), p(op.dbeta)
        s.bn = self.bn(op.bn)
        return R.OP_EW, s

    def _table(self, entries, cls):
        arr = (cls * len(entries))(*entries)
        raw = torch.frombuffer(bytearray(bytes(arr)), dtype=torch.uint8).to(self.A.device)
        self.keep.append(raw)
        return raw.data_ptr()

    def bnupd(self, op):
        ents = []
        for bn in op.bns:
            e = R.BnupdEntryT()
            e.stats, e.running_mean, e.running_var = self.A.ptr(bn.stats), self.A.ptr(bn.rmean), self.A.ptr(bn.rvar)
            e.num_batches_tracked = self.A.ptr(bn.nbt)
            e.count, e.momentum, e.C = float(bn.count), G.BN_MOMENTUM, bn.C
            ents.append(e)
        s = R.TableT()
        s.table, s.n, s.dtype, s.max_elems = self._table(ents, R.BnupdEntryT), len(ents), self.dtype, 0
        return R.OP_BNUPD, s

    def wprep(self, entries):
        ents, mx = [], 0
        for w, wf, wb in entries:
            e = R.WprepEntryT()
            e.w, e.w_fwd, e.w_bwd = self.A.ptr(w), self.A.ptr(wf), self.A.ptr(wb)
# ... 63 lines not shown
        if op.kind == 'grad_ready':
            return R.OP_NOP, R.MemsetT()
        return {'conv': self.conv, 'bneck': self.bneck, 'wgrad': self.wgrad, 'stem_fwd': self.stem, 'stem_wgrad': self.stem, 'ew': self.ew,
                'bnupd': self.bnupd}[op.kind](op)


class ModelState:

    def __init__(self, table, device, dtype):
        self.table, self.device, self.dtype = table, device, dtype
        self.A = Arenas(device, dtype)
        for name in ('param', 'rstat', 'nbt'):
            self.A.alloc(name, table.sizes[name])
        self.A.alloc('grad', table.sizes['param'])


class GraphInstance:

    def __init__(self, state, cfg, batch, height, width, train, image=None, share_weights_with=None):
        self.state, self.train = state, train
        self._wlp_owner = share_weights_with
        self.dtype = state.dtype
        env = os.environ.get
        if cfg.get('arch') == 'hrnet':
            self.g = G.HRNetGraph(state.table, cfg['extra'], cfg['J'], batch, height, width, train,
                                  wlp_is_master=(self.dtype == R.F32),
                                  wgrad_batch=int(env('FPD_WGRAD_BATCH')) if env('FPD_WGRAD_BATCH') else None,
                                  fp8=bool(cfg.get('fp8', False)))
        else:
            self.g = G.HourglassGraph(state.table, cfg['F'], cfg['S'], cfg['J'], batch, height, width, train,
                                      num_blocks=cfg.get('num_blocks', 1), wlp_is_master=(self.dtype == R.F32),
                                      fuse_bneck=(self.dtype == R.BF16 and not train and env('FPD_FUSE_BNECK', '1') != '0'),
                                      pair_branches=env('FPD_PAIR', '1') != '0', fuse_head=env('FPD_FUSE_HEAD', '1') != '0',
                                      wgrad_batch=int(env('FPD_WGRAD_BATCH')) if env('FPD_WGRAD_BATCH') else None)
        self.A = Arenas(state.device, self.dtype, parent=state.A)
        self.low = Lowering(self.A, self.dtype)
        self.low.train = train
        self.plan = R.Plan()
        self.rng = {}
        self.graphs = {}
        self._image_ext = image
        self._finalized = False
        self.mid_ops = []
        self.mid_native = []

    def _schedule(self, name, ir_ops):
        b, e = self.rng[name]
        assert e - b == len(ir_ops), (name, b, e, len(ir_ops))
        if not self.lanes_enabled or not any(o is not None and o.lane for o in ir_ops):
            return
        sch = PhaseSchedule([((o.lane or 0), o.accesses()) if o is not None else (0, None) for o in ir_ops], self.g.n_lanes)
        for k in range(len(ir_ops)):
            if sch.lanes[k] or sch.waits[k]:
                self.plan.set_schedule(b + k, sch.lanes[k], [b + w for w in sch.waits[k]])
        self.schedules[name] = sch

    def finalize(self):
        g = self.g
        ops = g.fwd + self.mid_ops + g.bwd
        self.lanes_enabled = os.environ.get('FPD_LANES', '1') != '0'
        self.schedules = {}
        delay = int(os.environ.get('FPD_REUSE_DELAY', '400')) if self.lanes_enabled else 0
        if not self.train:
            delay = 0
        act = G.plan_memory(ops, reuse_delay=delay)
        self.act_elems = act
# ... 7 lines not shown
        else:
            self.A.alloc('wlp', g.wlp_size)
            self.A.alloc('fold', g.fold_size)
        if self._image_ext is not None:
            self.A.t['image'] = self._image_ext
        else:
            self.A.alloc('image', g.N * 3 * g.H * g.W)
        p = self.plan
        b = len(p)
        p.add(*self.low.memset('stats'))
        entries = []
        for k in self.state.table.conv_keys():
            if k in g.MASTER_ONLY:
                continue
            wf, wb = g.wfwd.get(k), g.wbwd.get(k)
            if wf is not None or wb is not None:
                entries.append((self.state.table[k], wf, wb))
        if entries:
            p.add(*self.low.wprep(entries))
        w8 = getattr(g, 'w8', None)
        if w8:
            self.A.alloc('w8', g.w8_size)
            self.A.alloc('w8s', g.w8s_size)
            p.add(*self.low.wquant([(self.state.table[k], q, sc) for k, (q, sc) in w8.items()]))
        for op in g.fwd:
            for sub in ((op.a, op.b) if op.kind == 'bneck2' else (op,)):
                if sub.kind == 'bneck' and getattr(sub, 'folded', None) is not None:
                    p.add(*self.low.op(G.Op('bneck_fold', target=sub)))
                if sub.kind == 'head' and getattr(sub, 'folded', None) is not None:
                    p.add(*self.low.op(G.Op('head_fold', target=sub)))
        self.rng['prep'] = (b, len(p))
        b = len(p)
        self.op_index = {}
        for op in g.fwd:
            self.op_index[id(op)] = p.add(*self.low.op(op))
        self.rng['fwd'] = (b, len(p))
        self._schedule('fwd', list(g.fwd))
        b = len(p)
        for fn in self.mid_native:
            fn(p)
        self.rng['mid'] = (b, len(p))
        if self.train:
            b = len(p)
            p.add(*self.low.memset('grad'))
            self.low.use_partials = True
            bwd_ir = [op for op in g.bwd if op.kind != 'seed']
            self.low.plan_folds(bwd_ir)
            lowered = [self.low.op(op) for op in bwd_ir]
            self.low.finish_partials()
            self.bucket_ops = {}
            for ir, (code, st) in zip(bwd_ir, lowered):
                k = self.op_index[id(ir)] = p.add(code, st)
                if ir.kind == 'grad_ready':
                    self.bucket_ops[ir.bucket] = k
                    p.mark_event(k)
            self.rng['bwd'] = (b, len(p))
            self._schedule('bwd', [None] + bwd_ir)
        self._finalized = True
        return self

    def run(self, name, stream=None):
        gid = self.graphs.get(name)
        if gid is not None:
            self.plan.replay(gid, stream)
            return
        b, e = self.rng[name]
# ... 313 lines not shown
```

### fast-human-pose-estimation.pytorch_amd/graph.py

```python
import os
from collections import OrderedDict

BN_EPS = 1e-5
BN_MOMENTUM = 0.1
STATS_REPLICAS = int(os.environ.get('FPD_STATS_REPLICAS', '4'))
WGRAD_LANES = 1
LANE_LEVELS = 0
FOLD_APPLY = os.environ.get('FPD_FOLD_APPLY', '1') != '0'
WREDUCE_MODE = os.environ.get('FPD_WREDUCE_MODE', 'lag')
WGRAD_BATCH = 8


class Buf:
    __slots__ = ('arena', 'off', 'shape', 'name')

    def __init__(self, arena, off, shape, name=''):
        self.arena, self.off, self.shape, self.name = arena, off, tuple(shape), name

    @property
    def numel(self):
        n = 1
        for s in self.shape:
            n *= s
        return n
# ... 41 lines not shown
    return (max(1, 128 // w) + R - 1) * w * (bk // 8) <= 2048


class Op:

    def __init__(self, kind, **kw):
        self.kind = kind
        self.lane = None
        self.__dict__.update(kw)

    def accesses(self):
        def b(a):
            return a.buf if isinstance(a, Act) else a

        def bn_bufs(bn):
            if bn is None:
                return []
            return [bn.gamma, bn.beta] + ([bn.stats] if bn.mode == 'train' else [bn.rmean, bn.rvar])
        k = self.kind
        if k in ('conv2', 'bneck2', 'ew2'):
            (ra, wa), (rb, wb) = self.a.accesses(), self.b.accesses()
            return ra + rb, wa + wb
        if k == 'conv':
            rd = [b(self.x), self.w, self.bias, b(self.residual), b(self.epi_x)] + bn_bufs(self.bn) + bn_bufs(self.epi_bn)
            rd += [getattr(self, 'w8', None), getattr(self, 'w8s', None)]
            wr = [b(self.y), self.out_stats, self.epi_stats]
            fw = getattr(self, 'fused_wgrad', None)
            if fw is not None and getattr(self, 'fused_active', False):
                wr += [fw.dw, fw.dbias]
            fa = getattr(self, 'fold_apply', None)
            if fa is not None and getattr(self, 'fold_active', False):
                rd += [b(fa.x), b(fa.dy), fa.bstats] + bn_bufs(fa.bn)
                wr += [b(fa.y), fa.dgamma, fa.dbeta]
        elif k == 'head':
            rd = [b(self.y0), b(self.x), self.w_fc, self.b_fc, self.w_score, self.b_score, self.w_fc2, self.b_fc2,
                  self.w_score2, self.b_score2] + bn_bufs(self.bn)
            wr = [b(self.score), b(self.next)]
        elif k == 'bneck':
            rd = [b(self.x), self.w1, self.b1, self.w2, self.b2, self.w3, self.b3] + bn_bufs(self.bn1) + \
                bn_bufs(self.bn2) + bn_bufs(self.bn3)
            wr = [b(self.y)]
        elif k == 'wgrad':
            rd = [b(self.x), b(self.dy)] + bn_bufs(self.bn)
            wr = [self.dw, self.dbias]
        elif k == 'affsum':
            rd = [b(t) for t, _, _ in self.terms]
            for _, bn, _ in self.terms:
                rd += bn_bufs(bn)
            wr = [b(self.y), self.out_stats]
        elif k == 'nchw2nhwc':
            rd, wr = [self.image], [b(self.y)]
        elif k == 'wreduce':
            rd, wr = list(self.bufs), list(self.bufs)
        elif k == 'grad_ready':
            rd, wr = [self.region], []
        elif k == 'stem_fwd':
            rd, wr = [self.image, self.w, self.bias], [b(self.y), self.out_stats]
        elif k == 'stem_wgrad':
            rd, wr = [self.image, b(self.dy)], [self.dw, self.dbias]
        elif k == 'ew':
            rd = [b(self.x), b(self.x2), b(self.dy), b(self.add)] + bn_bufs(self.bn)
            wr = [b(self.y), self.out_stats, self.bstats, self.dgamma, self.dbeta]
        else:
            return None
        return [x for x in rd if x is not None], [x for x in wr if x is not None]

    def acts_in(self):
        if self.kind in ('conv2', 'bneck2', 'ew2'):
            return self.a.acts_in() + self.b.acts_in()
        if self.kind == 'head':
            return [t for t in (self.y0, self.x) if t is not None]
        fa = getattr(self, 'fold_apply', None)
        folded = [t for t in (fa.x, fa.dy) if isinstance(t, Act)] if fa is not None else []
        return [getattr(self, f) for f in ('x', 'x2', 'dy', 'add', 'residual', 'epi_x') if
                isinstance(getattr(self, f, None), Act)] + [a for a in getattr(self, 'extra_in', []) if a is not None] + folded

    def acts_out(self):
        if self.kind in ('conv2', 'bneck2', 'ew2'):
            return self.a.acts_out() + self.b.acts_out()
        if self.kind == 'head':
            return [t for t in (self.score, self.next) if t is not None]
        return [getattr(self, f) for f in ('y',) if isinstance(getattr(self, f, None), Act)] + \
               [a for a in getattr(self, 'extra_out', []) if a is not None]


class ParamTable:

    def __init__(self, keys, bucket_of=None):
        self.keys = list(keys)
        self.entries = OrderedDict()
        self.logical = dict(self.keys)
        self.sizes = {'param': 0, 'rstat': 0, 'nbt': 0}
        self.bucket = {k: (bucket_of(k) if bucket_of else 0) for k, _ in self.keys}
        placed = {}
        self.buckets = []
        for k, shp in sorted(self.keys, key=lambda ks: self.bucket[ks[0]]):
            if k.endswith('num_batches_tracked'):
                arena = 'nbt'
            elif k.endswith('running_mean') or k.endswith('running_var'):
                arena = 'rstat'
            else:
                arena = 'param'
            n = 1
            for s in shp:
                n *= s
            phys = (shp[0], shp[2], shp[3], shp[1]) if len(shp) == 4 else tuple(shp)
            off = self.sizes[arena]
            placed[k] = Buf(arena, off, phys, k)
            step = 4 if arena != 'nbt' else 2
            self.sizes[arena] = off + (n + step - 1) // step * step
            if arena == 'param':
                b = self.bucket[k]
                while len(self.buckets) <= b:
                    self.buckets.append([off, off])
                self.buckets[b][1] = self.sizes[arena]
        for k, _ in self.keys:
# ... 68 lines not shown
        while limbo and limbo[0][0] + reuse_delay <= i:
            _, o, n = limbo.pop(0)
            release(o, n)
        for a in op.acts_in() + op.acts_out():
            if a.buf is None:
                o, n = alloc(a.numel)
                a.buf = Buf('act', o, a.shape, a.name)
                sizes[id(a)] = n
        seen = set()
        for a in op.acts_in() + op.acts_out():
            if id(a) in seen:
                continue
            seen.add(id(a))
            if last[id(a)] == i and not a.persistent and id(a) in sizes:
                limbo.append((i, a.buf.off, sizes.pop(id(a))))
    return top


class _OpList(list):

    def __init__(self, owner):
        super().__init__()
        self.owner = owner

    def append(self, op):
        if op.lane is None:
            op.lane = self.owner._lane
        super().append(op)


class HourglassGraph:

    def __init__(self, params, num_feats, num_stacks, num_joints, batch, height, width, train, num_blocks=1,
                 depth=4, wlp_is_master=True, lane_levels=None, wgrad_batch=None, fuse_bneck=False, pair_branches=True, fuse_head=True):
        self.p = params
        self.F, self.S, self.J = num_feats, num_stacks, num_joints
        self.N, self.H, self.W = batch, height, width
        self.train, self.num_blocks, self.depth = train, num_blocks, depth
        self.wlp_is_master = wlp_is_master
        self.fuse_bneck = fuse_bneck and not train
        self.fuse_head = fuse_head and self.fuse_bneck
        self.pair_branches = pair_branches
        self._pair_op = None
        self._pair_ew = None
        self.stats_size = 0
        self.fold_size = 0
        self.wlp_size = 0
        self.wfwd, self.wbwd = {}, {}
        self._lane = 0
        self.lane_levels = LANE_LEVELS if lane_levels is None else lane_levels
        self.wgrad_batch = WGRAD_BATCH if wgrad_batch is None else wgrad_batch
        self._setup()

    MASTER_ONLY = ('conv1.weight',)

    def _setup(self):
        self._wg_pending = []
        self.n_lanes = 1 + self.depth + WGRAD_LANES
        self.fwd, self.bwd = _OpList(self), _OpList(self)
        self.bns = []
        self.image = Buf('image', 0, (self.N, 3, self.H, self.W), 'image')
        self.outputs = []
        self._bn_pending = {}
        self._bn_uses = {}
        for k in self.p.conv_keys():
            if k in self.MASTER_ONLY:
                continue
            b = self.p[k]
            if not self.wlp_is_master:
                self.wfwd[k] = self._wlp(b)
            if self.train:
                K, R, S, C = b.shape
                self.wbwd[k] = self._wlp(Buf('param', 0, (C, R, S, K)))
        self.build_forward()
        if self.train:
# ... 70 lines not shown
        self.fwd.append(op)
        return y

    def maxpool(self, x, name):
        n, h, w, c = x.shape
        return self.ew('maxpool_fwd', x.shape, (n, h // 2, w // 2, c), name, x=x)

    def upadd(self, a, b, name):
        assert a.shape[1] == 2 * b.shape[1] and a.shape[2] == 2 * b.shape[2] and a.shape[3] == b.shape[3]
        return self.ew('upadd_fwd', a.shape, a.shape, name, x=a, x2=b)

    def bottleneck(self, x, p, sink=None):
        c_in = x.shape[3]
        planes = self.p[p + 'conv1.weight'].shape[0]
        if self._fused(x, p):
            n, h, w, _ = x.shape
            y = Act(x.shape, p + 'out')
            wb = (lambda k: self.p[k]) if self.wlp_is_master else (lambda k: self.wfwd[k])
            fold = Buf('fold', self.fold_size, (3 * c_in + 4 * planes,), 'fold:' + p)
            self.fold_size += 3 * c_in + 4 * planes
            op = Op('bneck', x=x, y=y, dims=(n, h, w, c_in, planes), folded=fold,
                    w1=wb(p + 'conv1.weight'), b1=self.p[p + 'conv1.bias'], w2=wb(p + 'conv2.weight'),
                    b2=self.p[p + 'conv2.bias'], w3=wb(p + 'conv3.weight'), b3=self.p[p + 'conv3.bias'],
                    bn1=self._bn(p + 'bn1', c_in), bn2=self._bn(p + 'bn2', planes), bn3=self._bn(p + 'bn3', planes))
            y.producer = op
            (self.fwd if sink is None else sink).append(op)
            return y
        t = self.conv(x, p + 'conv1', bn=self._bn(p + 'bn1', c_in), sink=sink)
        t = self.conv(t, p + 'conv2', bn=self._bn(p + 'bn2', planes), pad=1, sink=sink)
        skip = x
        if (p + 'downsample.0.weight') in self.p.entries:
            assert sink is None
            skip = self.conv(x, p + 'downsample.0')
        return self.conv(t, p + 'conv3', bn=self._bn(p + 'bn3', planes), residual=skip, sink=sink)

    def _fused(self, x, p):
        planes = self.p[p + 'conv1.weight'].shape[0]
        return (self.fuse_bneck and self.bneck_fusable(x.shape, planes) and
                (p + 'downsample.0.weight') not in self.p.entries)

    def bottleneck_pair(self, xa, pa, xb, pb):
        la, lb = [], []
        ya = self.bottleneck(xa, pa, sink=la)
        yb = self.bottleneck(xb, pb, sink=lb)
        assert len(la) == len(lb) and len(la) in (1, 3)
        for oa, ob in zip(la, lb):
            self.fwd.append(Op('conv2' if oa.kind == 'conv' else 'bneck2', a=oa, b=ob))
        return ya, yb

    @staticmethod
    def bneck_fusable(shape, planes):
        n, h, w, c = shape
        return (c == 2 * planes and planes in (64, 128) and 4 <= w <= 64 and w & (w - 1) == 0 and
                ((h * w) % 128 == 0 or 128 % (h * w) == 0))

    def residual_seq(self, x, p, nb):
        for b in range(nb):
            x = self.bottleneck(x, '%s%d.' % (p, b))
        return x

    def hour_glass(self, x, p, n):
        q = '%s%d.' % (p, n - 1)
        nb = self.num_blocks
        laned = n > self.depth - self.lane_levels
        pa, pb = q + '0.0.', q + '1.0.'
        n_, h_, w_, c_ = x.shape
        if (self.pair_branches and nb == 1 and not laned and
                self._fused(x, pa) == self._fused(Act((n_, h_ // 2, w_ // 2, c_)), pb) and
                (pa + 'downsample.0.weight') not in self.p.entries and (pb + 'downsample.0.weight') not in self.p.entries):
            low = self.maxpool(x, q + 'pool')
            up1, low = self.bottleneck_pair(x, pa, low, pb)
        else:
            outer = self._lane
            if laned:
                self._lane = n
            up1 = self.residual_seq(x, q + '0.', nb)
            self._lane = outer
            low = self.maxpool(x, q + 'pool')
            low = self.residual_seq(low, q + '1.', nb)
        if n > 1:
            low = self.hour_glass(low, p, n - 1)
        else:
            low = self.residual_seq(low, q + '3.', nb)
        low = self.residual_seq(low, q + '2.', nb)
        return self.upadd(up1, low, q + 'upadd')

    def build_forward(self):
        K = self.p['conv1.weight'].shape[0]
        P, Q = (self.H + 6 - 7) // 2 + 1, (self.W + 6 - 7) // 2 + 1
        x = Act((self.N, P, Q, K), 'stem')
        op = Op('stem_fwd', image=self.image, w=self.p['conv1.weight'], bias=self.p['conv1.bias'], y=x, out_stats=None,
                dims=(self.N, self.H, self.W, K, P, Q))
        x.producer = op
        self.fwd.append(op)
        bn1 = self._bn('bn1', K)
        self._use_bn(x, bn1)
        x = self.ew('bnrelu_fwd', x.shape, x.shape, 'stem_act', x=x, bn=bn1)
        x = self.residual_seq(x, 'layer1.', 1)
        x = self.maxpool(x, 'pool1')
        x = self.residual_seq(x, 'layer2.', 1)
        x = self.residual_seq(x, 'layer3.', 1)
        ch = x.shape[3]
        for i in range(self.S):
            y = self.hour_glass(x, 'hg.%d.hg.' % i, self.depth)
            y = self.residual_seq(y, 'res.%d.' % i, self.num_blocks)
            if self.fuse_head and ch == 256 and self.J == 16:
                wb = (lambda k: self.p[k]) if self.wlp_is_master else (lambda k: self.wfwd[k])
                last = i == self.S - 1
                score = Act((y.shape[0], y.shape[1], y.shape[2], self.J), 'score.%d' % i)
                score.persistent = True
                nxt = None if last else Act(x.shape, 'stack%d.out' % i)
                fold = Buf('fold', self.fold_size, (3 * ch + 32,), 'fold:head%d' % i)
                self.fold_size += 3 * ch + 32
                op = Op('head', y0=y, x=None if last else x, score=score, next=nxt, dims=(y.shape[0], y.shape[1], y.shape[2], ch, self.J),
                        w_fc=wb('fc.%d.0.weight' % i), b_fc=self.p['fc.%d.0.bias' % i],
                        w_score=wb('score.%d.weight' % i), b_score=self.p['score.%d.bias' % i],
                        w_fc2=None if last else wb('fc_.%d.weight' % i), b_fc2=None if last else self.p['fc_.%d.bias' % i],
                        w_score2=None if last else wb('score_.%d.weight' % i),
                        b_score2=None if last else self.p['score_.%d.bias' % i],
                        bn=self._bn('fc.%d.1' % i, ch), folded=fold)
                score.producer = op
                if nxt is not None:
                    nxt.producer = op
                self.fwd.append(op)
                self.outputs.append(score)
                x = nxt
                continue
            y = self.conv(y, 'fc.%d.0' % i)
            fcbn = self._bn('fc.%d.1' % i, ch)
            score = self.conv(y, 'score.%d' % i, bn=fcbn)
# ... 402 lines not shown
```

### fast-human-pose-estimation.pytorch_amd/runtime.py

```python
import ctypes as C
import os

_HERE = os.path.dirname(os.path.abspath(__file__))
LIB_PATH = os.environ.get('FPD_AMD_LIB') or os.path.join(_HERE, 'csrc', 'libfpd_amd.so')

F32, BF16 = 0, 1
BN_NONE, BN_TRAIN, BN_EVAL = 0, 1, 2
EPI_PLAIN, EPI_BNRELU_BWD = 0, 1
BACKEND_MFMA, BACKEND_NAIVE, BACKEND_MFMA_GENERIC = 0, 1, 2
(EW_BNRELU_FWD, EW_BNRELU_BWD_R, EW_BN_BWD_APPLY, EW_MAXPOOL_FWD, EW_MAXPOOL_BWD, EW_UPADD_FWD, EW_SUMPOOL,
 EW_ADD, EW_RELU_MASK, EW_DILATE2) = range(10)
(OP_CONV, OP_WGRAD, OP_STEM_FWD, OP_STEM_WGRAD, OP_EW, OP_LOSS, OP_ADAM, OP_MEMSET, OP_WPREP, OP_BNUPD,
 OP_WREDUCE, OP_BNECK, OP_BNECK_FOLD, OP_CONV_PAIR, OP_BNECK_PAIR, OP_EW_PAIR, OP_PCK, OP_HEAD, OP_HEAD_FOLD,
 OP_NOP, OP_AFFSUM, OP_NCHW2NHWC, OP_CONV_F8, OP_WQUANT, OP_LOSS_OHKM, OP_SGD) = range(26)
AFFSUM_MAX = 4
MAX_STACKS = 8
MAXC = 512

_i32, _i64, _f32, _f64, _vp = C.c_int32, C.c_int64, C.c_float, C.c_double, C.c_void_p


class BnT(C.Structure):
    _fields_ = [('mode', _i32), ('relu', _i32), ('eps', _f32), ('_pad', _i32), ('stats', _vp), ('gamma', _vp),
                ('beta', _vp), ('running_mean', _vp), ('running_var', _vp)]


class ConvT(C.Structure):
    _fields_ = [('N', _i32), ('H', _i32), ('W', _i32), ('C', _i32), ('K', _i32), ('R', _i32), ('S', _i32),
                ('stride', _i32), ('pad', _i32), ('P', _i32), ('Q', _i32), ('dtype', _i32), ('epi', _i32),
                ('_pad', _i32), ('x', _vp), ('w', _vp), ('bias', _vp), ('residual', _vp), ('y', _vp),
                ('out_stats', _vp), ('bn', BnT), ('epi_x', _vp), ('epi_bn', BnT), ('epi_stats', _vp),
                ('wg_partial', _vp), ('wg_stride', _i64), ('wg_bias', _i32), ('wg_count', _i32),
                ('fold_x', _vp), ('fold_bn', BnT), ('fold_stats', _vp), ('fold_out', _vp), ('fold_dgamma', _vp), ('fold_dbeta', _vp)]


class ConvF8T(C.Structure):
    _fields_ = [('c', ConvT), ('w8', _vp), ('w8_scale', _vp)]


class WquantEntryT(C.Structure):
    _fields_ = [('w', _vp), ('w8', _vp), ('scale', _vp), ('K', _i32), ('RSC', _i32)]


class ConvPairT(C.Structure):
    _fields_ = [('a', ConvT), ('b', ConvT)]


class BneckT(C.Structure):
    _fields_ = [('N', _i32), ('H', _i32), ('W', _i32), ('C', _i32), ('P', _i32), ('dtype', _i32), ('_pad', _i32 * 2),
                ('x', _vp), ('y', _vp), ('w1', _vp), ('b1', _vp), ('w2', _vp), ('b2', _vp), ('w3', _vp), ('b3', _vp),
                ('bn1', BnT), ('bn2', BnT), ('bn3', BnT), ('folded', _vp)]


class BneckPairT(C.Structure):
    _fields_ = [('a', BneckT), ('b', BneckT)]


class WgradT(C.Structure):
    _fields_ = [('N', _i32), ('H', _i32), ('W', _i32), ('C', _i32), ('K', _i32), ('R', _i32), ('S', _i32),
                ('stride', _i32), ('pad', _i32), ('P', _i32), ('Q', _i32), ('dtype', _i32), ('x', _vp), ('dy', _vp),
                ('dw', _vp), ('dbias', _vp), ('bn', BnT), ('partial', _vp), ('partial_stride', _i64)]


class StemT(C.Structure):
    _fields_ = [('N', _i32), ('H', _i32), ('W', _i32), ('K', _i32), ('P', _i32), ('Q', _i32), ('dtype', _i32),
                ('_pad', _i32), ('x', _vp), ('w', _vp), ('bias', _vp), ('y', _vp), ('out_stats', _vp), ('dy', _vp),
                ('dw', _vp), ('dbias', _vp), ('partial', _vp), ('partial_stride', _i64)]


class EwT(C.Structure):
    _fields_ = [('op', _i32), ('dtype', _i32), ('N', _i32), ('H', _i32), ('W', _i32), ('C', _i32), ('x', _vp),
                ('x2', _vp), ('dy', _vp), ('add', _vp), ('y', _vp), ('out_stats', _vp), ('bstats', _vp),
                ('dgamma', _vp), ('dbeta', _vp), ('bn', BnT)]


class EwPairT(C.Structure):
    _fields_ = [('a', EwT), ('b', EwT)]


class HeadT(C.Structure):
    _fields_ = [('N', _i32), ('H', _i32), ('W', _i32), ('C', _i32), ('J', _i32), ('dtype', _i32), ('_pad', _i32 * 2),
                ('y0', _vp), ('x', _vp), ('score', _vp), ('next', _vp), ('w_fc', _vp), ('b_fc', _vp), ('w_score', _vp),
                ('b_score', _vp), ('w_fc2', _vp), ('b_fc2', _vp), ('w_score2', _vp), ('b_score2', _vp), ('bn', BnT),
                ('folded', _vp)]


class AffTermT(C.Structure):
    _fields_ = [('x', _vp), ('bn', BnT), ('up', _i32), ('_pad', _i32)]


class AffsumT(C.Structure):
    _fields_ = [('N', _i32), ('H', _i32), ('W', _i32), ('C', _i32), ('dtype', _i32), ('relu', _i32), ('nterms', _i32),
                ('_pad', _i32), ('t', AffTermT * 4), ('y', _vp)]


class LayoutT(C.Structure):
    _fields_ = [('src', _vp), ('dst', _vp), ('N', _i32), ('C', _i32), ('H', _i32), ('W', _i32), ('dtype', _i32), ('_pad', _i32)]


class PckT(C.Structure):
# ... 61 lines not shown
class WreduceEntryT(C.Structure):
    _fields_ = [('partial', _vp), ('dw', _vp), ('n', _i64), ('stride', _i64), ('count', _i32), ('_pad', _i32)]


class MemsetT(C.Structure):
    _fields_ = [('ptr', _vp), ('bytes', _i64)]


class TableT(C.Structure):
    _fields_ = [('table', _vp), ('n', _i32), ('dtype', _i32), ('max_elems', _i64)]


_STRUCTS = {'fpd_bn_t': BnT, 'fpd_conv_t': ConvT, 'fpd_wgrad_t': WgradT, 'fpd_stem_t': StemT, 'fpd_ew_t': EwT,
            'fpd_loss_t': LossT, 'fpd_adam_t': AdamT, 'fpd_wprep_entry_t': WprepEntryT,
            'fpd_bnupd_entry_t': BnupdEntryT, 'fpd_memset_t': MemsetT, 'fpd_table_t': TableT,
            'fpd_wreduce_entry_t': WreduceEntryT, 'fpd_bneck_t': BneckT, 'fpd_conv_pair_t': ConvPairT, 'fpd_bneck_pair_t': BneckPairT, 'fpd_ew_pair_t': EwPairT, 'fpd_pck_t': PckT, 'fpd_head_t': HeadT, 'fpd_affsum_t': AffsumT, 'fpd_layout_t': LayoutT,
            'fpd_conv_f8_t': ConvF8T, 'fpd_wquant_entry_t': WquantEntryT, 'fpd_flipmerge_t': FlipMergeT, 'fpd_finalpreds_t': FinalPredsT, 'fpd_targets_t': TargetsT,
            'fpd_warp_src_t': WarpSrcT, 'fpd_warp_t': WarpT, 'fpd_loss_ohkm_t': LossOhkmT, 'fpd_sgd_t': SgdT}

ABI_VERSION = 2

SYMBOLS = {
    'fpd_conv_forward': (C.c_int, [C.POINTER(ConvT), _vp]),
    'fpd_conv_forward_pair': (C.c_int, [C.POINTER(ConvPairT), _vp]),
    'fpd_conv_forward_f8': (C.c_int, [C.POINTER(ConvF8T), _vp]),
    'fpd_conv_f8_in_domain': (C.c_int, [C.POINTER(ConvT)]),
    'fpd_weight_quant_f8': (C.c_int, [_vp, _i32, _vp]),
    'fpd_bottleneck_forward': (C.c_int, [C.POINTER(BneckT), _vp]),
    'fpd_bottleneck_fold': (C.c_int, [C.POINTER(BneckT), _vp]),
    'fpd_bottleneck_forward_pair': (C.c_int, [C.POINTER(BneckPairT), _vp]),
    'fpd_conv_fused_wgrad_partials': (C.c_int, [C.POINTER(ConvT)]),
    'fpd_conv_fold_supported': (C.c_int, [_vp]),
    'fpd_conv_pair_fold_supported': (C.c_int, [_vp]),
    'fpd_conv_pair_fused_wgrad_partials': (C.c_int, [C.POINTER(ConvPairT), C.POINTER(C.c_int32), C.POINTER(C.c_int32)]),
    'fpd_conv_wgrad': (C.c_int, [C.POINTER(WgradT), _vp]),
    'fpd_wgrad_num_partials': (C.c_int, [C.POINTER(WgradT)]),
    'fpd_wgrad_reduce': (C.c_int, [_vp, _i32, _i64, _vp]),
    'fpd_stem_forward': (C.c_int, [C.POINTER(StemT), _vp]),
    'fpd_stem_wgrad': (C.c_int, [C.POINTER(StemT), _vp]),
    'fpd_stem_wgrad_num_partials': (C.c_int, [C.POINTER(StemT)]),
    'fpd_elementwise': (C.c_int, [C.POINTER(EwT), _vp]),
    'fpd_elementwise_pair': (C.c_int, [C.POINTER(EwPairT), _vp]),
    'fpd_pck': (C.c_int, [C.POINTER(PckT), _vp]),
    'fpd_affsum': (C.c_int, [C.POINTER(AffsumT), _vp]),
    'fpd_flip_w': (C.c_int, [_vp, _vp, _i64, _i32, _vp]),
    'fpd_flip_merge': (C.c_int, [C.POINTER(FlipMergeT), _vp]),
    'fpd_final_preds': (C.c_int, [C.POINTER(FinalPredsT), _vp]),
    'fpd_render_targets': (C.c_int, [C.POINTER(TargetsT), _vp]),
    'fpd_warp_affine': (C.c_int, [C.POINTER(WarpT), _vp]),
    'fpd_head_forward': (C.c_int, [C.POINTER(HeadT), _vp]),
    'fpd_head_fold': (C.c_int, [C.POINTER(HeadT), _vp]),
    'fpd_loss': (C.c_int, [C.POINTER(LossT), _vp]),
    'fpd_loss_ohkm': (C.c_int, [C.POINTER(LossOhkmT), _vp]),
    'fpd_loss_ohkm_scratch_bytes': (C.c_int64, [C.POINTER(LossT)]),
    'fpd_adam': (C.c_int, [C.POINTER(AdamT), _vp]),
    'fpd_sgd': (C.c_int, [C.POINTER(SgdT), _vp]),
    'fpd_weight_prep': (C.c_int, [_vp, _i32, _i64, _i32, _vp]),
    'fpd_bn_update_running': (C.c_int, [_vp, _i32, _vp]),
    'fpd_cast': (C.c_int, [_vp, _vp, _i64, _i32, _i32, _vp]),
    'fpd_nchw_to_nhwc': (C.c_int, [_vp, _vp, _i32, _i32, _i32, _i32, _i32, _vp]),
    'fpd_nhwc_to_nchw': (C.c_int, [_vp, _vp, _i32, _i32, _i32, _i32, _i32, _vp]),
    'fpd_plan_create': (_vp, []),
    'fpd_plan_destroy': (None, [_vp]),
    'fpd_plan_add': (C.c_int, [_vp, _i32, _vp, _i64]),
    'fpd_plan_size': (C.c_int, [_vp]),
    'fpd_plan_set_schedule': (C.c_int, [_vp, _i32, _i32, C.POINTER(C.c_int32), _i32]),
# ... 136 lines not shown
```

### include/fpd_amd.h

```cpp
#ifndef FPD_AMD_H
#define FPD_AMD_H

#include <stddef.h>
#include <stdint.h>

#ifdef __cplusplus
extern "C" {
#endif

typedef void* fpd_stream_t;

enum { FPD_F32 = 0, FPD_BF16 = 1 };
#ifndef FPD_STATS_REPLICAS
#define FPD_STATS_REPLICAS 4
#endif
typedef int64_t fpd_stat_t;
#define FPD_STATS_WORDS(C) ((int64_t)FPD_STATS_REPLICAS * 4 * (C))
enum { FPD_BN_NONE = 0, FPD_BN_TRAIN = 1, FPD_BN_EVAL = 2 };
enum { FPD_EPI_PLAIN = 0, FPD_EPI_BNRELU_BWD = 1 };
enum { FPD_BACKEND_MFMA = 0, FPD_BACKEND_NAIVE = 1, FPD_BACKEND_MFMA_GENERIC = 2 };

typedef struct {
    int32_t mode;
    int32_t relu;
// ... 4 lines not shown
    const float* beta;
    const float* running_mean;
    const float* running_var;
} fpd_bn_t;

typedef struct {
    int32_t N, H, W, C;
    int32_t K, R, S;
    int32_t stride, pad;
    int32_t P, Q;
    int32_t dtype;
    int32_t epi;
    int32_t _pad;
    const void* x;
    const void* w;
    const float* bias;
    const void* residual;
    void* y;
    fpd_stat_t* out_stats;
    fpd_bn_t bn;
    const void* epi_x;
    fpd_bn_t epi_bn;
    fpd_stat_t* epi_stats;
    float* wg_partial;
    int64_t wg_stride;
    int32_t wg_bias;
    int32_t wg_count;
    const void* fold_x;
    fpd_bn_t fold_bn;
    const fpd_stat_t* fold_stats;
    void* fold_out;
    float* fold_dgamma;
    float* fold_dbeta;
} fpd_conv_t;

typedef struct {
    int32_t N, H, W, C, P, dtype;
    int32_t _pad[2];
    const void* x;
    void* y;
    const void* w1;
    const float* b1;
    const void* w2;
    const float* b2;
    const void* w3;
    const float* b3;
    fpd_bn_t bn1, bn2, bn3;
    const float* folded;
} fpd_bneck_t;

typedef struct {
    int32_t N, H, W, C, J, dtype;
    int32_t _pad[2];
    const void* y0;
    const void* x;
    void* score;
    void* next;
    const void* w_fc;
    const float* b_fc;
    const void* w_score;
    const float* b_score;
    const void* w_fc2;
    const float* b_fc2;
    const void* w_score2;
    const float* b_score2;
    fpd_bn_t bn;
    const float* folded;
} fpd_head_t;
int fpd_head_forward(const fpd_head_t* a, fpd_stream_t stream);
int fpd_head_fold(const fpd_head_t* a, fpd_stream_t stream);

typedef struct { fpd_conv_t a, b; } fpd_conv_pair_t;

typedef struct { fpd_bneck_t a, b; } fpd_bneck_pair_t;

typedef struct {
    int32_t N, H, W, C, K, R, S, stride, pad, P, Q, dtype;
    const void* x;
    const void* dy;
    float* dw;
    float* dbias;
    fpd_bn_t bn;
    float* partial;
    int64_t partial_stride;
} fpd_wgrad_t;

typedef struct {
    int32_t N, H, W, K, P, Q, dtype, _pad;
    const float* x;
    const float* w;
    const float* bias;
    void* y;
    fpd_stat_t* out_stats;
    const void* dy;
    float* dw;
    float* dbias;
    float* partial;
    int64_t partial_stride;
} fpd_stem_t;

enum {
    FPD_EW_BNRELU_FWD = 0, FPD_EW_BNRELU_BWD_R = 1, FPD_EW_BN_BWD_APPLY = 2, FPD_EW_MAXPOOL_FWD = 3,
    FPD_EW_MAXPOOL_BWD = 4, FPD_EW_UPADD_FWD = 5, FPD_EW_SUMPOOL = 6, FPD_EW_ADD = 7, FPD_EW_RELU_MASK = 8,
    FPD_EW_DILATE2 = 9
};
typedef struct {
    int32_t op, dtype;
    int32_t N, H, W, C;
    const void* x;
    const void* x2;
    const void* dy;
    const void* add;
    void* y;
    fpd_stat_t* out_stats;
    fpd_stat_t* bstats;
    float* dgamma;
    float* dbeta;
    fpd_bn_t bn;
} fpd_ew_t;

#define FPD_AFFSUM_MAX 4
typedef struct { const void* x; fpd_bn_t bn; int32_t up; int32_t _pad; } fpd_affterm_t;
typedef struct {
    int32_t N, H, W, C;
    int32_t dtype, relu, nterms, _pad;
    fpd_affterm_t t[FPD_AFFSUM_MAX];
    void* y;
} fpd_affsum_t;
int fpd_affsum(const fpd_affsum_t* a, fpd_stream_t stream);

typedef struct { const float* src; void* dst; int32_t N, C, H, W, dtype, _pad; } fpd_layout_t;
// ... 41 lines not shown
    float lr, momentum, weight_decay;
    float grad_scale;
    int32_t nesterov;
    int32_t _pad;
    const float* lr_dev;
    int64_t* step_dev;
} fpd_sgd_t;

typedef struct {
    const float* w;
    void* w_fwd;
    void* w_bwd;
    int32_t K, R, S, C;
} fpd_wprep_entry_t;

typedef struct {
    const fpd_stat_t* stats;
    float* running_mean; float* running_var; int64_t* num_batches_tracked;
    double count; float momentum; int32_t C;
} fpd_bnupd_entry_t;

typedef struct {
    const float* partial; float* dw; int64_t n; int64_t stride; int32_t count; int32_t _pad;
} fpd_wreduce_entry_t;

int fpd_conv_forward(const fpd_conv_t* a, fpd_stream_t stream);
int fpd_conv_forward_pair(const fpd_conv_pair_t* p, fpd_stream_t stream);
int fpd_bottleneck_forward(const fpd_bneck_t* a, fpd_stream_t stream);
int fpd_bottleneck_fold(const fpd_bneck_t* a, fpd_stream_t stream);
int fpd_bottleneck_forward_pair(const fpd_bneck_pair_t* p, fpd_stream_t stream);
int fpd_conv_fused_wgrad_partials(const fpd_conv_t* a);
int fpd_conv_fold_supported(const fpd_conv_t* a);
int fpd_conv_pair_fold_supported(const fpd_conv_pair_t* p);
int fpd_conv_pair_fused_wgrad_partials(const fpd_conv_pair_t* p, int32_t* n_a, int32_t* n_b);
int fpd_conv_wgrad(const fpd_wgrad_t* a, fpd_stream_t stream);
int fpd_wgrad_num_partials(const fpd_wgrad_t* a);
int fpd_wgrad_reduce(const fpd_wreduce_entry_t* table_dev, int32_t n_entries, int64_t max_elems, fpd_stream_t stream);
int fpd_stem_forward(const fpd_stem_t* a, fpd_stream_t stream);
int fpd_stem_wgrad(const fpd_stem_t* a, fpd_stream_t stream);
int fpd_stem_wgrad_num_partials(const fpd_stem_t* a);
int fpd_elementwise(const fpd_ew_t* a, fpd_stream_t stream);
typedef struct { fpd_ew_t a, b; } fpd_ew_pair_t;
int fpd_elementwise_pair(const fpd_ew_pair_t* p, fpd_stream_t stream);
int fpd_loss(const fpd_loss_t* a, fpd_stream_t stream);
int fpd_loss_ohkm(const fpd_loss_ohkm_t* a, fpd_stream_t stream);
int64_t fpd_loss_ohkm_scratch_bytes(const fpd_loss_t* a);
int fpd_adam(const fpd_adam_t* a, fpd_stream_t stream);
int fpd_sgd(const fpd_sgd_t* a, fpd_stream_t stream);
int fpd_weight_prep(const fpd_wprep_entry_t* table_dev, int32_t n_entries, int64_t max_elems, int32_t dtype,
                    fpd_stream_t stream);
int fpd_bn_update_running(const fpd_bnupd_entry_t* table_dev, int32_t n_entries, fpd_stream_t stream);
int fpd_cast(const void* src, void* dst, int64_t n, int32_t src_dtype, int32_t dst_dtype, fpd_stream_t stream);
int fpd_nchw_to_nhwc(const float* src, void* dst, int32_t N, int32_t C, int32_t H, int32_t W, int32_t dtype,
                     fpd_stream_t stream);
int fpd_nhwc_to_nchw(const void* src, float* dst, int32_t N, int32_t C, int32_t H, int32_t W, int32_t dtype,
                     fpd_stream_t stream);

typedef struct {
    int32_t B, J, H, W, dtype, log_slots;
    float thr;
    int32_t _pad;
    const void* out;
    const float* target;
    float* counts;
    double* log;
    long long* cursor;
    const double* losses;
} fpd_pck_t;
int fpd_pck(const fpd_pck_t* a, fpd_stream_t stream);

typedef struct {
// ... 108 lines not shown
```

Baseline: 3658 images/s.

## Fuse downsample skip conv into conv3 and BN+ReLU into stem epilogue

Adds a second 1x1 source (x2, w2, bias2) to the c1 conv kernel so a bottleneck's downsample convolution is computed inside the conv3 launch rather than materialised as a separate residual. Also lets the stem forward kernel apply eval-mode BN+ReLU in its epilogue, removing a separate elementwise pass. The aim is fewer launches and less activation traffic. In exchange the kernel needs more LDS for the second weight tile, and both fusions carry new routing and validation logic. The stem fusion applies only in eval (teacher) forward, and the skip fusion applies to forward launches.

After: 3703 images/s, median of 6. 1.01x the previous value.

```diff
diff --git a/fast-human-pose-estimation.pytorch_amd/csrc/api.hip b/fast-human-pose-estimation.pytorch_amd/csrc/api.hip
--- a/fast-human-pose-estimation.pytorch_amd/csrc/api.hip
+++ b/fast-human-pose-estimation.pytorch_amd/csrc/api.hip
@@ -72,6 +72,8 @@
     if (!strcmp(name, "conv_c1")) return fpd_conv_c1_option(0, value);
     if (!strcmp(name, "conv_c1_blocks")) return fpd_conv_c1_option(1, value);
     if (!strcmp(name, "conv_c1_launches")) return fpd_conv_c1_option(2, value);
+    if (!strcmp(name, "conv_skip")) return fpd_conv_c1_option(3, value);
+    if (!strcmp(name, "stem_act")) return fpd_stem_s2d_option(0, value);
     if (!strcmp(name, "conv_c3")) return fpd_conv_c3_option(0, value);
     if (!strcmp(name, "conv_c3_blocks")) return fpd_conv_c3_option(1, value);
     if (!strcmp(name, "conv_c3_launches")) return fpd_conv_c3_option(2, value);
@@ -101,6 +103,8 @@
     FPD_REQUIRE(a->bn.mode != FPD_BN_EVAL || (a->bn.running_mean && a->bn.running_var), "conv: eval-mode BN without running stats");
     FPD_REQUIRE(a->epi == FPD_EPI_PLAIN || (a->epi_x && a->epi_stats && a->epi_bn.mode == FPD_BN_TRAIN && a->epi_bn.stats),
                 "conv: BNRELU_BWD epilogue needs epi_x, epi_stats and a train-mode epi_bn");
+    FPD_REQUIRE(a->x2 == nullptr || (a->w2 != nullptr && a->C2 > 0), "conv: a second source (x2) needs w2 and C2");
+    FPD_REQUIRE(a->x2 == nullptr || a->residual == nullptr, "conv: a second source (x2) and a residual exclude each other");
     return 0;
 }
 
@@ -123,7 +127,7 @@
 static bool eligible(unsigned backends) { return (backends >> g_fpd_backend & 1u) != 0; }
 
 static const ConvBackend* route_conv(const fpd_conv_t& a, const fpd_conv_t* b, ConvAsk ask, ConvRoute& r) {
-    r = ConvRoute{false, 0, 0};
+    r = ConvRoute{false, 0, 0, false};
     for (const ConvBackend& e : g_conv_backends) {
         if (!eligible(e.backends)) continue;
         if (e.route == nullptr ? b == nullptr : e.route(a, b, ask, r) == 0) return &e;
@@ -144,6 +148,8 @@
     FPD_REQUIRE(r.folds || (a.fold_x == nullptr && (b == nullptr || b->fold_x == nullptr)),
                 "conv: the launch asks for a folded BN-backward apply (fold_x), which its route (%s) does not offer; %s() reports 0 for it",
                 e->name, b ? "fpd_conv_pair_fold_supported" : "fpd_conv_fold_supported");
+    FPD_REQUIRE(r.skips || (a.x2 == nullptr && (b == nullptr || b->x2 == nullptr)),
+                "conv: the launch carries a second 1x1 source (x2), which its route (%s) does not offer; fpd_conv_skip_supported() reports 0 for it", e->name);
     int rc = e->launch(a, b, st);
     for (++e; rc == 1 && e != std::end(g_conv_backends); ++e)
         if (e->route == nullptr && eligible(e->backends)) rc = e->launch(a, b, st);
@@ -160,20 +166,27 @@
 int fpd_conv_fold_supported(const fpd_conv_t* a) {
     ConvRoute r;
     if (!a || validate_conv(a) != 0) return 0;
-    route_conv(*a, nullptr, ConvAsk{true, a->wg_partial != nullptr}, r);
+    route_conv(*a, nullptr, ConvAsk{true, a->wg_partial != nullptr, a->x2 != nullptr}, r);
     return r.folds ? 1 : 0;
 }
 int fpd_conv_pair_fold_supported(const fpd_conv_pair_t* p) {
     ConvRoute r;
     if (!p || validate_conv(&p->a) != 0 || validate_conv(&p->b) != 0) return 0;
-    if (route_conv(p->a, &p->b, ConvAsk{true, fpd_conv_ask(p->a, &p->b).wg}, r) != nullptr) return r.folds ? 1 : 0;
+    if (route_conv(p->a, &p->b, ConvAsk{true, fpd_conv_ask(p->a, &p->b).wg, fpd_conv_ask(p->a, &p->b).skip}, r) != nullptr) return r.folds ? 1 : 0;
     return (fpd_conv_fold_supported(&p->a) && fpd_conv_fold_supported(&p->b)) ? 1 : 0;
+}
+
+int fpd_conv_skip_supported(const fpd_conv_t* a) {
+    ConvRoute r;
+    if (!a || validate_conv(a) != 0) return 0;
+    route_conv(*a, nullptr, ConvAsk{a->fold_x != nullptr, a->wg_partial != nullptr, true}, r);
+    return r.skips ? 1 : 0;
 }
 
 int fpd_conv_fused_wgrad_partials(const fpd_conv_t* a) {
     ConvRoute r;
     if (!a || validate_conv(a) != 0) return 0;
-    route_conv(*a, nullptr, ConvAsk{a->fold_x != nullptr, true}, r);
+    route_conv(*a, nullptr, ConvAsk{a->fold_x != nullptr, true, a->x2 != nullptr}, r);
     return r.slabs_a;
 }
 int fpd_conv_pair_fused_wgrad_partials(const fpd_conv_pair_t* p, int32_t* n_a, int32_t* n_b) {
@@ -181,7 +194,7 @@
     *n_a = *n_b = 0;
     if (validate_conv(&p->a) != 0 || validate_conv(&p->b) != 0) return 0;
     ConvRoute r;
-    route_conv(p->a, &p->b, ConvAsk{fpd_conv_ask(p->a, &p->b).fold, true}, r);
+    route_conv(p->a, &p->b, ConvAsk{fpd_conv_ask(p->a, &p->b).fold, true, fpd_conv_ask(p->a, &p->b).skip}, r);
     *n_a = r.slabs_a; *n_b = r.slabs_b;
     return 0;
 }
@@ -212,6 +225,7 @@
     if (rc) return rc;
     rc = validate_conv(&p->b);
     if (rc) return rc;
+    FPD_REQUIRE(p->a.x2 == nullptr && p->b.x2 == nullptr, "conv_pair: a pair launch takes no second source (x2)");
     rc = launch_conv(p->a, &p->b, (hipStream_t)stream);
     return rc ? rc : check_launch();
 }
@@ -301,14 +315,15 @@
 
 struct StemBackend {
     unsigned backends;
+    bool (*takes_act)(const fpd_stem_t& a);
     int (*forward)(const fpd_stem_t& a, hipStream_t st);
     int (*wgrad_partials)(const fpd_stem_t& a);
     int (*wgrad)(const fpd_stem_t& a, hipStream_t st);
 };
 static const StemBackend g_stem_backends[] = {
-    {ON_MFMA, fpd_stem_forward_s2d_launch, fpd_stem_wgrad_s2d_partials, fpd_stem_wgrad_s2d_launch},
-    {ON_MFMA, fpd_stem_forward_mfma_launch, fpd_stem_wgrad_mfma_partials, fpd_stem_wgrad_mfma_launch},
-    {ON_ANY, fpd_stem_forward_launch, fpd_stem_wgrad_partials, fpd_stem_wgrad_launch},
+    {ON_MFMA, fpd_stem_forward_s2d_takes_act, fpd_stem_forward_s2d_launch, fpd_stem_wgrad_s2d_partials, fpd_stem_wgrad_s2d_launch},
+    {ON_MFMA, nullptr, fpd_stem_forward_mfma_launch, fpd_stem_wgrad_mfma_partials, fpd_stem_wgrad_mfma_launch},
+    {ON_ANY, nullptr, fpd_stem_forward_launch, fpd_stem_wgrad_partials, fpd_stem_wgrad_launch},
 };
 
 int fpd_stem_wgrad_num_partials(const fpd_stem_t* a) {
@@ -323,9 +338,18 @@
     return rc ? rc : check_launch();
 }
 
+int fpd_stem_act_supported(const fpd_stem_t* a) {
+    if (!a || a->act.mode != FPD_BN_EVAL || !a->act.gamma || !a->act.beta || !a->act.running_mean || !a->act.running_var || a->out_stats != nullptr) return 0;
+    for (const StemBackend& e : g_stem_backends)
+        if (eligible(e.backends)) return (e.takes_act != nullptr && e.takes_act(*a)) ? 1 : 0;
+    return 0;
+}
+
 int fpd_stem_forward(const fpd_stem_t* a, fpd_stream_t stream) {
     FPD_REQUIRE(a && a->x && a->w && a->bias && a->y, "stem: null pointer");
     FPD_REQUIRE(a->P == (a->H + 6 - 7) / 2 + 1 && a->Q == (a->W + 6 - 7) / 2 + 1, "stem: bad output size");
+    FPD_REQUIRE(a->act.mode == FPD_BN_NONE || fpd_stem_act_supported(a) == 1,
+                "stem: the launch asks for BN + ReLU in its epilogue (act), which is not offered for it; fpd_stem_act_supported() reports 0");
     int rc = 1;
     for (const StemBackend& e : g_stem_backends)
         if (rc == 1 && eligible(e.backends)) rc = e.forward(*a, (hipStream_t)stream);
@@ -619,8 +643,9 @@
 }
 
 static void conv_tag(char* p, size_t n, const char* what, const fpd_conv_t& c) {
-    snprintf(p, n, "%s N=%d H=%d W=%d C=%d K=%d R=%d s=%d %s%s%s%s", what, c.N, c.H, c.W, c.C, c.K, c.R, c.stride,
-             c.epi == FPD_EPI_BNRELU_BWD ? "dgrad" : "fwd", c.bn.mode == FPD_BN_EVAL ? " evalbn" : "", c.wg_partial ? " +wgrad" : "", c.fold_x ? " +fold" : "");
+    snprintf(p, n, "%s N=%d H=%d W=%d C=%d K=%d R=%d s=%d %s%s%s%s%s", what, c.N, c.H, c.W, c.C, c.K, c.R, c.stride,
+             c.epi == FPD_EPI_BNRELU_BWD ? "dgrad" : "fwd", c.bn.mode == FPD_BN_EVAL ? " evalbn" : "", c.wg_partial ? " +wgrad" : "", c.fold_x ? " +fold" : "",
+             c.x2 ? " +skip" : "");
 }
 static void set_op_tag(int idx, const fpd_op& o) {
     char t[200] = "";
@@ -642,7 +667,8 @@
         case FPD_OP_HEAD: snprintf(t, sizeof(t), "head N=%d H=%d W=%d C=%d J=%d", o.u.head.N, o.u.head.H, o.u.head.W, o.u.head.C, o.u.head.J); break;
         case FPD_OP_EW: snprintf(t, sizeof(t), "ew %s N=%d H=%d W=%d C=%d", ewn(o.u.ew.op), o.u.ew.N, o.u.ew.H, o.u.ew.W, o.u.ew.C); break;
         case FPD_OP_EW_PAIR: snprintf(t, sizeof(t), "ew2 %s N=%d H=%d W=%d C=%d | H=%d W=%d", ewn(o.u.epair.a.op), o.u.epair.a.N, o.u.epair.a.H, o.u.epair.a.W, o.u.epair.a.C, o.u.epair.b.H, o.u.epair.b.W); break;
-        case FPD_OP_STEM_FWD: case FPD_OP_STEM_WGRAD: snprintf(t, sizeof(t), "%s N=%d H=%d W=%d K=%d", o.type == FPD_OP_STEM_FWD ? "stem_fwd" : "stem_wgrad", o.u.stem.N, o.u.stem.H, o.u.stem.W, o.u.stem.K); break;
+        case FPD_OP_STEM_FWD: case FPD_OP_STEM_WGRAD: snprintf(t, sizeof(t), "%s N=%d H=%d W=%d K=%d%s", o.type == FPD_OP_STEM_FWD ? "stem_fwd" : "stem_wgrad", o.u.stem.N, o.u.stem.H, o.u.stem.W, o.u.stem.K,
+                                                              (o.type == FPD_OP_STEM_FWD && o.u.stem.act.mode != FPD_BN_NONE) ? " +act" : ""); break;
         case FPD_OP_AFFSUM: snprintf(t, sizeof(t), "affsum N=%d H=%d W=%d C=%d terms=%d", o.u.affsum.N, o.u.affsum.H, o.u.affsum.W, o.u.affsum.C, o.u.affsum.nterms); break;
         case FPD_OP_LOSS: snprintf(t, sizeof(t), "loss B=%d J=%d H=%d W=%d S=%d", o.u.loss.B, o.u.loss.J, o.u.loss.H, o.u.loss.W, o.u.loss.S); break;
         case FPD_OP_LOSS_OHKM: snprintf(t, sizeof(t), "loss_ohkm B=%d J=%d H=%d W=%d S=%d k=%d,%d", o.u.lossk.base.B, o.u.lossk.base.J, o.u.lossk.base.H, o.u.lossk.base.W, o.u.lossk.base.S, o.u.lossk.topk_pose, o.u.lossk.topk_kd); break;
diff --git a/fast-human-pose-estimation.pytorch_amd/csrc/conv_c1.hip b/fast-human-pose-estimation.pytorch_amd/csrc/conv_c1.hip
--- a/fast-human-pose-estimation.pytorch_amd/csrc/conv_c1.hip
+++ b/fast-human-pose-estimation.pytorch_amd/csrc/conv_c1.hip
@@ -22,7 +22,7 @@
     return *reinterpret_cast<const unsigned*>(&a);
 }
 
-template <int C, int K, bool BWD, bool WG>
+template <int C, int K, bool BWD, bool WG, bool SKIP = false>
 struct C1Geo {
     static constexpr int CV = C / 8, KV = K / 8;
     static constexpr int NV = C / 16, NK = K / 16;
@@ -32,12 +32,13 @@
     static constexpr int WAVE_LDS = WG ? TILE_A + TILE_O : (TILE_A > TILE_O ? TILE_A : TILE_O);
     static constexpr int FLUSH = C1_NW * 64 * 16 * 4 + C1_NW * K * 4 + 8 * 2 * K * 8;
     static constexpr int REGION = C1_NW * WAVE_LDS > FLUSH ? C1_NW * WAVE_LDS : FLUSH;
-    static constexpr int TABLES = (2 * C + (BWD ? 3 * C + 4 * K : 0) + K) * 4;
-    static constexpr int LDS = TABLES + K * C * 2 + REGION;
+    static constexpr int TABLES = (2 * C + (BWD ? 3 * C + 4 * K : 0) + K + (SKIP ? K : 0)) * 4;
+    static constexpr int LDS = TABLES + (SKIP ? 2 : 1) * K * C * 2 + REGION;
     static constexpr int NT = (C / 32) * (K / 32);
     static constexpr int NTW = NT / C1_NW;
     static_assert(!WG || (BWD && NT % C1_NW == 0 && NTW >= 1), "fused weight gradient: every wave owns whole tiles of dW");
     static_assert(64 % CV == 0 && 64 % KV == 0, "a lane keeps its channel chunk");
+    static_assert(!SKIP || (!BWD && !WG && K == 2 * C), "second source: forward launches C -> 2C only");
 };
 
 #define C1_PHASE() do { asm volatile("" ::: "memory"); __builtin_amdgcn_sched_barrier(0); } while (0)
@@ -48,9 +49,10 @@
 #define C1_STAMP() do { } while (0)
 #endif
 
-template <int C, int K, bool BWD, bool FOLD, bool WG, bool RES>
+template <int C, int K, bool BWD, bool FOLD, bool WG, bool RES, bool SKIP>
 __device__ __forceinline__ void c1_body(const fpd_conv_t& a, const int bi, const int nblk) {
-    using G = C1Geo<C, K, BWD, WG>;
+    static_assert(!(SKIP && RES), "the second source IS the residual");
+    using G = C1Geo<C, K, BWD, WG, SKIP>;
     constexpr int CV = G::CV, KV = G::KV, NV = G::NV, NK = G::NK, KT = G::KT, KS = G::KS, PXA = G::PXA, PXO = G::PXO;
     constexpr int RPB = CV >= 16 ? 1 : 16 / CV;
     extern __shared__ __attribute__((aligned(16))) unsigned char smem[];
@@ -67,13 +69,17 @@
     float* s_fold = s_shift + C;
     float* s_epi = s_fold + (BWD ? 3 * C : 0);
     float* s_bias = s_epi + (BWD ? 4 * K : 0);
-    unsigned char* sW = reinterpret_cast<unsigned char*>(s_bias + K);
-    unsigned char* sT = sW + K * C * 2;
+    float* s_bias2 = s_bias + K;
+    unsigned char* sW = reinterpret_cast<unsigned char*>(s_bias + K + (SKIP ? K : 0));
+    unsigned char* sW2 = sW + K * C * 2;
+    unsigned char* sT = sW + (SKIP ? 2 : 1) * K * C * 2;
     unsigned char* tA = sT + wave * G::WAVE_LDS;
     unsigned char* tO = WG ? tA + G::TILE_A : tA;
 
     const bf16_t* __restrict__ x = reinterpret_cast<const bf16_t*>(a.x);
     const bf16_t* __restrict__ w = reinterpret_cast<const bf16_t*>(a.w);
+    const bf16_t* __restrict__ x2 = reinterpret_cast<const bf16_t*>(a.x2);
+    const bf16_t* __restrict__ w2 = reinterpret_cast<const bf16_t*>(a.w2);
     bf16_t* y = reinterpret_cast<bf16_t*>(a.y);
     const bf16_t* res = reinterpret_cast<const bf16_t*>(a.residual);
     const bf16_t* ex = reinterpret_cast<const bf16_t*>(a.epi_x);
@@ -92,7 +98,7 @@
     C1_STAMP();
 
     BnRaw braw;
-    float bias_raw;
+    float bias_raw, bias2_raw;
     const int te = tid - 128, tb = tid - 256;
     const bool r_bn = has_bn && tid < C;
     const bool r_fold = fold && tid < C;
@@ -106,12 +112,21 @@
         stat_request(a.fold_stats, C, 1, tid, fs2);
     }
     else if (r_epi) bn_request(a.epi_bn, te, K, braw);
-    else if (r_bias) { bias_raw = 0.f; if (a.bias != nullptr) bias_raw = a.bias[tb]; }
+    else if (r_bias) {
+        bias_raw = 0.f; if (a.bias != nullptr) bias_raw = a.bias[tb];
+        if constexpr (SKIP) { bias2_raw = 0.f; if (a.bias2 != nullptr) bias2_raw = a.bias2[tb]; }
+    }
     __builtin_amdgcn_sched_barrier(0);
 
     uint4 rx[NV];
     uint4 ru[FOLD ? NV : 1];
-    uint4 rr[NK];
+    uint4 rr[SKIP ? 1 : NK];
+    uint4 rx2[SKIP ? NV : 1];
+    auto load_x2 = [&](int t) {
+        const uint4* px = reinterpret_cast<const uint4*>(x2) + ((size_t)t * 32 * CV + lane);
+#pragma unroll
+        for (int i = 0; i < (SKIP ? NV : 1); ++i) rx2[i] = px[i * 64];
+    };
     auto load_x = [&](int t) {
         const uint4* px = reinterpret_cast<const uint4*>(x) + ((size_t)t * 32 * CV + lane);
 #pragma unroll
@@ -125,21 +140,26 @@
     auto load_r = [&](int t) {
         const uint4* pr = reinterpret_cast<const uint4*>(BWD ? ex : res) + ((size_t)t * 32 * KV + lane);
 #pragma unroll
-        for (int i = 0; i < NK; ++i) rr[i] = pr[i * 64];
+        for (int i = 0; i < (SKIP ? 1 : NK); ++i) rr[i] = pr[i * 64];
     };
     int tile = r_beg * C1_NW + wave;
     {
         constexpr int NWV = (K * CV + 511) / 512;
-        uint4 rw[NWV];
+        uint4 rw[NWV], rw2[SKIP ? NWV : 1];
 #pragma unroll
         for (int i = 0; i < NWV; ++i) {
             const int v = tid + i * 512;
             rw[i] = make_uint4(0, 0, 0, 0);
             if (v < K * CV) rw[i] = *reinterpret_cast<const uint4*>(w + (size_t)v * 8);
+            if constexpr (SKIP) {
+                rw2[i] = make_uint4(0, 0, 0, 0);
+                if (v < K * CV) rw2[i] = *reinterpret_cast<const uint4*>(w2 + (size_t)v * 8);
+            }
         }
         __builtin_amdgcn_sched_barrier(0);
         {
             const int t0 = min(tile, ntile - 1);
+            if constexpr (SKIP) load_x2(t0);
             load_x(t0);
             if constexpr (BWD || has_res) load_r(t0);
         }
@@ -169,6 +189,7 @@
             s_epi[te] = sc; s_epi[K + te] = sh; s_epi[2 * K + te] = mu; s_epi[3 * K + te] = is;
         } else if (r_bias) {
             s_bias[tb] = bias_raw;
+            if constexpr (SKIP) s_bias2[tb] = bias2_raw;
         }
 #pragma unroll
         for (int i = 0; i < NWV; ++i) {
@@ -177,6 +198,7 @@
                 const int k = v / CV, ch = v % CV;
                 const int sw = (k / RPB) & (CV - 1);
                 *reinterpret_cast<uint4*>(sW + (k * CV + (ch ^ sw)) * 16) = rw[i];
+                if constexpr (SKIP) *reinterpret_cast<uint4*>(sW2 + (k * CV + (ch ^ sw)) * 16) = rw2[i];
             }
         }
     }
@@ -246,7 +268,12 @@
             for (int i = 0; i < NV; ++i) po[i * 64] = rx[i];
         }
     };
-    auto finish = [&](const f32x16& accv, const int kt, auto resc) {
+    auto stage2 = [&]() {
+#pragma unroll
+        for (int i = 0; i < (SKIP ? NV : 1); ++i)
+            *reinterpret_cast<uint4*>(tA + (pxa0 + i * (64 / CV)) * PXA + cch * 16) = make_uint4(rx2[i].x, rx2[i].y, rx2[i].z, rx2[i].w);
+    };
+    auto finish = [&](const f32x16& accv, const int kt, auto resc, const float* sb) {
         constexpr bool HASRES = decltype(resc)::value;
         {
 #pragma unroll
@@ -259,7 +286,7 @@
                         v0 += c1_unpack(r2.x);
                         v1 += c1_unpack(r2.y);
                     }
-                    const f32x4 b4 = *reinterpret_cast<const f32x4*>(s_bias + kt * 32 + 8 * q + 4 * hh);
+                    const f32x4 b4 = *reinterpret_cast<const f32x4*>(sb + kt * 32 + 8 * q + 4 * hh);
                     v0 += f32x2{b4[0], b4[1]};
                     v1 += f32x2{b4[2], b4[3]};
                 }
@@ -373,6 +400,15 @@
         const bool live = tile < ntile;
         const bool pf = round + 1 < r_end && tile + C1_NW < ntile;
         if (live) {
+            bf16x8 bf2[SKIP ? KS : 1];
+            if constexpr (SKIP) {
+                stage2();
+                if (pf) load_x2(tile + C1_NW);
+                C1_PHASE();
+#pragma unroll
+                for (int kk = 0; kk < KS; ++kk) bf2[kk] = *reinterpret_cast<const bf16x8*>(tA + l31 * PXA + kk * 32 + hh * 16);
+                C1_PHASE();
+            }
             if (FOLD && fold) { if constexpr (FOLD) stage(tile, std::integral_constant<int, 2>{}); }
             else if (has_bn) { if constexpr (!BWD) stage(tile, std::integral_constant<int, 1>{}); }
             else stage(tile, std::integral_constant<int, 0>{});
@@ -389,6 +425,26 @@
                     *reinterpret_cast<uint4*>(tO + (pxo0 + i * (64 / KV)) * PXO + kch * 16) = make_uint4(rr[i].x, rr[i].y, rr[i].z, rr[i].w);
                 C1_PHASE();
             }
+            if constexpr (SKIP) {
+                C1_PHASE();
+#pragma unroll
+                for (int k0 = 0; k0 < KT; k0 += 2) {
+                    f32x16 acc0, acc1;
+#pragma unroll
+                    for (int e = 0; e < 16; ++e) { acc0[e] = 0.f; acc1[e] = 0.f; }
+                    const unsigned char* wrow0 = sW2 + (k0 * 32 + l31) * (C * 2);
+#pragma unroll
+                    for (int kk = 0; kk < KS; ++kk) {
+                        const bf16x8 wf0 = *reinterpret_cast<const bf16x8*>(wrow0 + ((2 * kk + hh) ^ wsw) * 16);
+                        acc0 = __builtin_amdgcn_mfma_f32_32x32x16_bf16(wf0, bf2[kk], acc0, 0, 0, 0);
+                        const bf16x8 wf1 = *reinterpret_cast<const bf16x8*>(wrow0 + 32 * (C * 2) + ((2 * kk + hh) ^ wsw) * 16);
+                        acc1 = __builtin_amdgcn_mfma_f32_32x32x16_bf16(wf1, bf2[kk], acc1, 0, 0, 0);
+                    }
+                    finish(acc0, k0, std::false_type{}, s_bias2);
+                    finish(acc1, k0 + 1, std::false_type{}, s_bias2);
+                }
+                C1_PHASE();
+            }
 #pragma unroll
             for (int k0 = 0; k0 < KT; k0 += 2) {
                 f32x16 acc0, acc1;
@@ -404,8 +460,8 @@
                         acc1 = __builtin_amdgcn_mfma_f32_32x32x16_bf16(wf1, bf[kk], acc1, 0, 0, 0);
                     }
                 }
-                finish(acc0, k0, std::integral_constant<bool, has_res>{});
-                if (k0 + 1 < KT) finish(acc1, k0 + 1, std::integral_constant<bool, has_res>{});
+                finish(acc0, k0, std::integral_constant<bool, has_res || SKIP>{}, s_bias);
+                if (k0 + 1 < KT) finish(acc1, k0 + 1, std::integral_constant<bool, has_res || SKIP>{}, s_bias);
             }
             if constexpr (!BWD && has_res) { if (pf) load_r(tile + C1_NW); }
             C1_PHASE();
@@ -515,21 +571,25 @@
 
 struct C1Args { fpd_conv_t c[2]; int nblk[2]; };
 
-template <int C, int K, bool BWD, bool FOLD, bool WG, bool RES>
+template <int C, int K, bool BWD, bool FOLD, bool WG, bool RES, bool SKIP = false>
 __global__ __launch_bounds__(512, 2) void c1_kernel(const C1Args p) {
     const int bid = blockIdx.x, n = gridDim.x, nb = p.nblk[1];
     const int fb0 = fpd_cut(bid, nb, n), fb1 = fpd_cut(bid + 1, nb, n);
     const int isb = fb1 > fb0 ? 1 : 0;
     const int u = isb ? fb0 : bid - fb0;
-    c1_body<C, K, BWD, FOLD, WG, RES>(p.c[isb], u, p.nblk[isb]);
-}
-
-int g_c1_mode = -1, g_c1_blocks = -1;
+    c1_body<C, K, BWD, FOLD, WG, RES, SKIP>(p.c[isb], u, p.nblk[isb]);
+}
+
+int g_c1_mode = -1, g_c1_blocks = -1, g_c1_skip = -1;
 std::atomic<int> g_c1_launches{0};
 int c1_mode() {
     if (g_c1_mode < 0) { const char* e = getenv("FPD_C1"); g_c1_mode = e ? atoi(e) : 1; }
     return g_c1_mode;
 }
+int c1_skip() {
+    if (g_c1_skip < 0) { const char* e = getenv("FPD_FUSE_SKIP"); g_c1_skip = e ? atoi(e) : 1; }
+    return g_c1_skip;
+}
 int c1_blocks() {
     if (g_c1_blocks < 0) { const char* e = getenv("FPD_C1_BLOCKS"); g_c1_blocks = e ? atoi(e) : 192; }
     return g_c1_blocks < 1 ? 1 : g_c1_blocks;
@@ -549,7 +609,12 @@
 bool c1_chan(int c) { return c == 32 || c == 64 || c == 128; }
 bool c1_aligned(const void* p) { return (reinterpret_cast<uintptr_t>(p) & 15) == 0; }
 
-bool c1_domain(const fpd_conv_t& a, bool fold) {
+bool c1_domain(const fpd_conv_t& a, bool fold, bool skip = false) {
+    if (skip) {
+        if (c1_skip() == 0 || a.epi != FPD_EPI_PLAIN || a.residual != nullptr || a.x2 == nullptr || a.w2 == nullptr) return false;
+        if (a.C2 != a.C || a.K != 2 * a.C || a.C > 64 || !c1_chan(a.C)) return false;
+        if (!c1_aligned(a.x2) || !c1_aligned(a.w2) || a.y == a.x2) return false;
+    }
     if (a.dtype != FPD_BF16 || a.R != 1 || a.S != 1 || a.stride != 1 || a.pad != 0 || a.P != a.H || a.Q != a.W) return false;
     if (!(c1_chan(a.C) || (a.C == 16 && a.K == 128)) || !c1_chan(a.K)) return false;
     const long long M = (long long)a.N * a.H * a.W;
@@ -570,7 +635,7 @@
 struct C1Plan { int na, nb, grid; bool wg; };
 bool c1_route(const fpd_conv_t& a, const fpd_conv_t* b, ConvAsk ask, ConvRoute& r, C1Plan& pl) {
     const int mode = c1_mode();
-    if (mode == 0 || !c1_domain(a, ask.fold)) return false;
+    if (mode == 0 || !c1_domain(a, ask.fold, ask.skip) || (ask.skip && b != nullptr)) return false;
     const bool bwd = a.epi == FPD_EPI_BNRELU_BWD;
     long long px = (long long)a.N * a.H * a.W;
     if (b != nullptr) {
@@ -591,24 +656,25 @@
     pl.grid = total;
     pl.wg = ask.wg && c1_fuse_wgrad() != 0 && bwd && (a.C / 32) * (a.K / 32) == C1_NW;
     r.folds = ask.fold && bwd;
+    r.skips = ask.skip;
     r.slabs_a = pl.wg ? pl.na : 0;
     r.slabs_b = pl.wg ? pl.nb : 0;
     return true;
 }
 
-template <int C, int K, bool BWD, bool FOLD, bool WG, bool RES>
+template <int C, int K, bool BWD, bool FOLD, bool WG, bool RES, bool SKIP = false>
 int c1_launch_t(const fpd_conv_t& a, const fpd_conv_t* b, const C1Plan& pl, hipStream_t st) {
     static LdsAttr configured;
 #ifdef FPD_C1_TIMING
-    constexpr size_t lds = C1Geo<C, K, BWD, WG>::LDS + 1024;
+    constexpr size_t lds = C1Geo<C, K, BWD, WG, SKIP>::LDS + 1024;
 #else
-    constexpr size_t lds = C1Geo<C, K, BWD, WG>::LDS;
+    constexpr size_t lds = C1Geo<C, K, BWD, WG, SKIP>::LDS;
 #endif
     static_assert(lds <= 160 * 1024, "conv_c1: LDS budget");
-    if (int rc_ = configured.ensure(reinterpret_cast<const void*>(&c1_kernel<C, K, BWD, FOLD, WG, RES>), lds)) return rc_;
+    if (int rc_ = configured.ensure(reinterpret_cast<const void*>(&c1_kernel<C, K, BWD, FOLD, WG, RES, SKIP>), lds)) return rc_;
     C1Args args;
     args.c[0] = a; args.c[1] = b ? *b : a; args.nblk[0] = pl.na; args.nblk[1] = pl.nb;
-    FPD_LAUNCH((c1_kernel<C, K, BWD, FOLD, WG, RES>), dim3(pl.grid), dim3(512), lds, st, args);
+    FPD_LAUNCH((c1_kernel<C, K, BWD, FOLD, WG, RES, SKIP>), dim3(pl.grid), dim3(512), lds, st, args);
     g_c1_launches.fetch_add(1, std::memory_order_relaxed);
     return 0;
 }
@@ -626,6 +692,10 @@
             return 1;
         }
     }
+    if (a.x2 != nullptr) {
+        if constexpr (K == 2 * C && C >= 32 && C <= 64) return c1_launch_t<C, K, false, false, false, false, true>(a, nullptr, pl, st);
+        else return 1;
+    }
     if (a.residual != nullptr) return c1_launch_t<C, K, false, false, false, true>(a, b, pl, st);
     return c1_launch_t<C, K, false, false, false, false>(a, b, pl, st);
 }
@@ -643,6 +713,7 @@
 
 int fpd_conv_c1_option(int which, int value) {
     if (which == 2) return g_c1_launches.load(std::memory_order_relaxed);
+    if (which == 3) { const int prev = c1_skip(); g_c1_skip = value; return prev; }
     int& g = which == 0 ? g_c1_mode : g_c1_blocks;
     const int prev = which == 0 ? c1_mode() : c1_blocks();
     g = value;
diff --git a/fast-human-pose-estimation.pytorch_amd/csrc/conv_c3.hip b/fast-human-pose-estimation.pytorch_amd/csrc/conv_c3.hip
--- a/fast-human-pose-estimation.pytorch_amd/csrc/conv_c3.hip
+++ b/fast-human-pose-estimation.pytorch_amd/csrc/conv_c3.hip
@@ -476,7 +476,7 @@
     return 0;
 }
 bool c3_route(const fpd_conv_t& a, const fpd_conv_t* b, ConvAsk ask, ConvRoute& r, C3Plan& pl) {
-    if (!c3_takes(a, b) || !c3_plan(a, b, pl)) return false;
+    if (ask.skip || !c3_takes(a, b) || !c3_plan(a, b, pl)) return false;
     r = ConvRoute{ask.fold && a.epi == FPD_EPI_BNRELU_BWD, 0, 0};
     return true;
 }
diff --git a/fast-human-pose-estimation.pytorch_amd/csrc/conv_dispatch.h b/fast-human-pose-estimation.pytorch_amd/csrc/conv_dispatch.h
--- a/fast-human-pose-estimation.pytorch_amd/csrc/conv_dispatch.h
+++ b/fast-human-pose-estimation.pytorch_amd/csrc/conv_dispatch.h
@@ -1,10 +1,11 @@
 #pragma once
 #include "common.h"
 
-struct ConvAsk { bool fold, wg; };
-struct ConvRoute { bool folds; int slabs_a, slabs_b; };
+struct ConvAsk { bool fold, wg, skip; };
+struct ConvRoute { bool folds; int slabs_a, slabs_b; bool skips; };
 inline ConvAsk fpd_conv_ask(const fpd_conv_t& a, const fpd_conv_t* b) {
-    return ConvAsk{a.fold_x != nullptr || (b != nullptr && b->fold_x != nullptr), a.wg_partial != nullptr || (b != nullptr && b->wg_partial != nullptr)};
+    return ConvAsk{a.fold_x != nullptr || (b != nullptr && b->fold_x != nullptr), a.wg_partial != nullptr || (b != nullptr && b->wg_partial != nullptr),
+                   a.x2 != nullptr || (b != nullptr && b->x2 != nullptr)};
 }
 inline int fpd_conv_check_slabs(const fpd_conv_t& c, int slabs, const char* unit) {
     if (c.wg_partial == nullptr) return 0;
@@ -42,6 +43,8 @@
 int fpd_wreduce_launch(const fpd_wreduce_entry_t* table, int n, int64_t max_elems, hipStream_t st);
 
 int fpd_stem_forward_s2d_launch(const fpd_stem_t& a, hipStream_t st);
+bool fpd_stem_forward_s2d_takes_act(const fpd_stem_t& a);
+int fpd_stem_s2d_option(int which, int value);
 int fpd_stem_wgrad_s2d_partials(const fpd_stem_t& a);
 int fpd_stem_wgrad_s2d_launch(const fpd_stem_t& a, hipStream_t st);
 int fpd_stem_forward_mfma_launch(const fpd_stem_t& a, hipStream_t st);
diff --git a/fast-human-pose-estimation.pytorch_amd/csrc/conv_pp.hip b/fast-human-pose-estimation.pytorch_amd/csrc/conv_pp.hip
--- a/fast-human-pose-estimation.pytorch_amd/csrc/conv_pp.hip
+++ b/fast-human-pose-estimation.pytorch_amd/csrc/conv_pp.hip
@@ -746,7 +746,7 @@
 }
 
 static bool pp_route(const fpd_conv_t& a, const fpd_conv_t* b, ConvAsk ask, ConvRoute& r, PPPlan& pl) {
-    if (!pp_takes(a, b) || !pp_plan(a, b, ask, pl)) return false;
+    if (ask.skip || !pp_takes(a, b) || !pp_plan(a, b, ask, pl)) return false;
     auto foldable = [](const fpd_conv_t& c) { return c.epi == FPD_EPI_BNRELU_BWD && c.bn.mode == FPD_BN_NONE; };
     PPPlan other;
     r.folds = ask.fold && foldable(a) && (b == nullptr || foldable(*b)) &&
diff --git a/fast-human-pose-estimation.pytorch_amd/csrc/conv_tile.hip b/fast-human-pose-estimation.pytorch_amd/csrc/conv_tile.hip
--- a/fast-human-pose-estimation.pytorch_amd/csrc/conv_tile.hip
+++ b/fast-human-pose-estimation.pytorch_amd/csrc/conv_tile.hip
@@ -395,7 +395,7 @@
 struct TilePlan { int esz, bk, tn, tiles; bool allw, fold; size_t lds; };
 
 static bool tile_route(const fpd_conv_t& a, const fpd_conv_t* b, ConvAsk ask, ConvRoute& r, TilePlan& pl) {
-    if (!tile_domain(a)) return false;
+    if (ask.skip || !tile_domain(a)) return false;
     if (b != nullptr && (!tile_domain(*b) || a.dtype != b->dtype || a.K != b->K || a.C != b->C || a.R != b->R)) return false;
     pl.esz = a.dtype == FPD_BF16 ? 2 : 4;
     const int vec = 16 / pl.esz;
diff --git a/fast-human-pose-estimation.pytorch_amd/csrc/stem_s2d.hip b/fast-human-pose-estimation.pytorch_amd/csrc/stem_s2d.hip
--- a/fast-human-pose-estimation.pytorch_amd/csrc/stem_s2d.hip
+++ b/fast-human-pose-estimation.pytorch_amd/csrc/stem_s2d.hip
@@ -17,7 +17,7 @@
 #define S2_STAMP() do { } while (0)
 #endif
 
-template <int TN>
+template <int TN, bool ACT>
 __global__ __launch_bounds__(256) void stem_s2d_fwd_kernel(const fpd_stem_t a, const int logQ, const int ntiles) {
     extern __shared__ __attribute__((aligned(16))) unsigned char smem[];
     const int tid = threadIdx.x, lane = tid & 63, wave = __builtin_amdgcn_readfirstlane(tid >> 6);
@@ -102,16 +102,33 @@
     const unsigned char* wrow = sW + l31 * S2_WROW + hh * 16;
 
     bf16_t* __restrict__ y = reinterpret_cast<bf16_t*>(a.y);
-    const bool want_stats = a.out_stats != nullptr;
+    const bool want_stats = !ACT && a.out_stats != nullptr;
     f32x4 bias4[TN][4], f1[TN][4], f2[TN][4];
+    const int act_relu = a.act.relu;
+    if constexpr (ACT) {
+        float* s_act = reinterpret_cast<float*>(sW + 32 * TN * S2_WROW);
+        if (tid < 32 * TN) {
+            float sc = 0.f, sh = 0.f, mu, is;
+            if (tid < K) bn_coef(a.act, tid, K, 1.0, sc, sh, mu, is);
+            s_act[tid] = sc;
+            s_act[32 * TN + tid] = sh;
+        }
+        __syncthreads();
+    }
 #pragma unroll
     for (int tn = 0; tn < TN; ++tn)
 #pragma unroll
         for (int j = 0; j < 4; ++j) {
             const int k = 32 * tn + 8 * j + 4 * hh;
             bias4[tn][j] = (k < K) ? f32x4{a.bias[k], a.bias[k + 1], a.bias[k + 2], a.bias[k + 3]} : f32x4{0.f, 0.f, 0.f, 0.f};
-            f1[tn][j] = f32x4{0.f, 0.f, 0.f, 0.f};
-            f2[tn][j] = f32x4{0.f, 0.f, 0.f, 0.f};
+            if constexpr (ACT) {
+                const float* s_act = reinterpret_cast<const float*>(sW + 32 * TN * S2_WROW);
+                f1[tn][j] = *reinterpret_cast<const f32x4*>(s_act + k);
+                f2[tn][j] = *reinterpret_cast<const f32x4*>(s_act + 32 * TN + k);
+            } else {
+                f1[tn][j] = f32x4{0.f, 0.f, 0.f, 0.f};
+                f2[tn][j] = f32x4{0.f, 0.f, 0.f, 0.f};
+            }
         }
 
     int ring_n = -1, ring_hi = 0;
@@ -162,7 +179,14 @@
                 if (32 * tn + 8 * j < K) {
                     const f32x4 b = bias4[tn][j];
                     const float v0 = acc[tn][4 * j] + b[0], v1 = acc[tn][4 * j + 1] + b[1], v2 = acc[tn][4 * j + 2] + b[2], v3 = acc[tn][4 * j + 3] + b[3];
-                    const unsigned p0 = f2bf_pk(v0, v1), p1 = f2bf_pk(v2, v3);
+                    unsigned p0 = f2bf_pk(v0, v1), p1 = f2bf_pk(v2, v3);
+                    if constexpr (ACT) {
+                        const f32x4 sc = f1[tn][j], sh = f2[tn][j];
+                        const float r0 = bn_act(__uint_as_float(p0 << 16), sc[0], sh[0], act_relu), r1 = bn_act(__uint_as_float(p0 & 0xffff0000u), sc[1], sh[1], act_relu);
+                        const float r2 = bn_act(__uint_as_float(p1 << 16), sc[2], sh[2], act_relu), r3 = bn_act(__uint_as_float(p1 & 0xffff0000u), sc[3], sh[3], act_relu);
+                        p0 = f2bf_pk(r0, r1);
+                        p1 = f2bf_pk(r2, r3);
+                    }
                     *reinterpret_cast<uint2*>(yrow + 32 * tn + 8 * j) = make_uint2(p0, p1);
                     if (want_stats) {
                         const f32x4 d = {__uint_as_float(p0 << 16) - b[0], __uint_as_float(p0 & 0xffff0000u) - b[1],
@@ -403,27 +427,56 @@
 
 }
 
+static int g_stem_act = -1;
+static int stem_act_mode() {
+    if (g_stem_act < 0) { const char* e = getenv("FPD_STEM_ACT"); g_stem_act = e ? atoi(e) : 1; }
+    return g_stem_act;
+}
+int fpd_stem_s2d_option(int which, int value) {
+    (void)which;
+    const int prev = stem_act_mode();
+    g_stem_act = value;
+    return prev;
+}
+
+static bool s2d_fwd_ok(const fpd_stem_t& a, int& logQ) {
+    if (a.dtype != FPD_BF16 || a.K % 8 != 0 || a.K > 64) return false;
+    if (a.Q > 128 || a.Q < 16 || (a.Q & (a.Q - 1)) != 0 || a.H != 2 * a.P || a.W != 2 * a.Q) return false;
+    logQ = 0;
+    while ((1 << logQ) < a.Q) ++logQ;
+    return a.P % (128 >> logQ) == 0;
+}
+bool fpd_stem_forward_s2d_takes_act(const fpd_stem_t& a) {
+    int logQ;
+    return stem_act_mode() != 0 && a.act.mode == FPD_BN_EVAL && a.out_stats == nullptr && s2d_fwd_ok(a, logQ);
+}
+
 int fpd_stem_forward_s2d_launch(const fpd_stem_t& a, hipStream_t st) {
-    if (a.dtype != FPD_BF16 || a.K % 8 != 0 || a.K > 64) return 1;
-    if (a.Q > 128 || a.Q < 16 || (a.Q & (a.Q - 1)) != 0 || a.H != 2 * a.P || a.W != 2 * a.Q) return 1;
-    int logQ = 0;
-    while ((1 << logQ) < a.Q) ++logQ;
+    int logQ;
+    if (!s2d_fwd_ok(a, logQ)) return 1;
+    const bool act = a.act.mode != FPD_BN_NONE;
+    if (act && !fpd_stem_forward_s2d_takes_act(a)) return 1;
     const int rows = 128 >> logQ;
-    if (a.P % rows != 0) return 1;
     const int TN = a.K > 32 ? 2 : 1;
     const int ring = 2 * rows + 3;
-    const size_t lds = std::max((size_t)ring * (a.Q + 3) * S2_PIXB + (size_t)32 * TN * S2_WROW,
+    const size_t lds = std::max((size_t)ring * (a.Q + 3) * S2_PIXB + (size_t)32 * TN * S2_WROW + (act ? (size_t)2 * 32 * TN * sizeof(float) : 0),
                                 (size_t)4 * 32 * TN * 2 * (33 * sizeof(float) + sizeof(double)));
     const int tiles = a.N * a.P * a.Q / 128;
     static const int cap = 0;
     const int blocks = std::max(1, std::min(tiles, cap > 0 ? cap : (TN == 1 ? 512 : 256)));
-    static LdsAttr cfg1, cfg2;
-    if (TN == 1) {
-        if (int rc_ = cfg1.ensure(reinterpret_cast<const void*>(&stem_s2d_fwd_kernel<1>), lds)) return rc_;
-        FPD_LAUNCH((stem_s2d_fwd_kernel<1>), dim3(blocks), dim3(256), lds, st, a, logQ, tiles);
+    static LdsAttr cfg1, cfg2, cfg1a, cfg2a;
+    if (TN == 1 && !act) {
+        if (int rc_ = cfg1.ensure(reinterpret_cast<const void*>(&stem_s2d_fwd_kernel<1, false>), lds)) return rc_;
+        FPD_LAUNCH((stem_s2d_fwd_kernel<1, false>), dim3(blocks), dim3(256), lds, st, a, logQ, tiles);
+    } else if (!act) {
+        if (int rc_ = cfg2.ensure(reinterpret_cast<const void*>(&stem_s2d_fwd_kernel<2, false>), lds)) return rc_;
+        FPD_LAUNCH((stem_s2d_fwd_kernel<2, false>), dim3(blocks), dim3(256), lds, st, a, logQ, tiles);
+    } else if (TN == 1) {
+        if (int rc_ = cfg1a.ensure(reinterpret_cast<const void*>(&stem_s2d_fwd_kernel<1, true>), lds)) return rc_;
+        FPD_LAUNCH((stem_s2d_fwd_kernel<1, true>), dim3(blocks), dim3(256), lds, st, a, logQ, tiles);
     } else {
-        if (int rc_ = cfg2.ensure(reinterpret_cast<const void*>(&stem_s2d_fwd_kernel<2>), lds)) return rc_;
-        FPD_LAUNCH((stem_s2d_fwd_kernel<2>), dim3(blocks), dim3(256), lds, st, a, logQ, tiles);
+        if (int rc_ = cfg2a.ensure(reinterpret_cast<const void*>(&stem_s2d_fwd_kernel<2, true>), lds)) return rc_;
+        FPD_LAUNCH((stem_s2d_fwd_kernel<2, true>), dim3(blocks), dim3(256), lds, st, a, logQ, tiles);
     }
     return 0;
 }
diff --git a/fast-human-pose-estimation.pytorch_amd/executor.py b/fast-human-pose-estimation.pytorch_amd/executor.py
--- a/fast-human-pose-estimation.pytorch_amd/executor.py
+++ b/fast-human-pose-estimation.pytorch_amd/executor.py
@@ -141,6 +141,10 @@
         s.bn = self.bn(op.bn)
         s.epi_x, s.epi_bn, s.epi_stats = p(_abuf(op.epi_x)), self.bn(op.epi_bn), p(op.epi_stats)
         s.wg_partial, s.wg_stride, s.wg_bias, s.wg_count = None, 0, 0, 0
+        if not plain and getattr(op, 'skip_fused', False):
+            return R.OP_NOP, R.MemsetT()
+        if not plain and getattr(op, 'skip_active', False):
+            self._fill_skip(op, s)
         if not plain and getattr(op, 'fused_wgrad', None) is not None and self.use_partials:
             n = R.lib().fpd_conv_fused_wgrad_partials(C.byref(s))
             if n > 0:
@@ -191,6 +195,56 @@
                 for m in cands:
                     m.fold_active = True
                     m.fold_apply.folded = True
+
+    def _fill_skip(self, op, s):
+        sc, p = op.skip_conv, self.A.ptr
+        assert _abuf(sc.y) is _abuf(op.residual) and sc.bn is None, 'skip: the downsample convolution must produce exactly this residual'
+        s.x2, s.w2, s.bias2, s.C2 = p(_abuf(sc.x)), p(sc.w), p(sc.bias), sc.dims[3]
+        s.residual = None
+
+    def plan_skips(self, ops, readers=None):
+        if os.environ.get('FPD_FUSE_SKIP', '1') == '0':
+            return
+        l = R.lib()
+        readers = ops if readers is None else readers
+        members_of = lambda top: [m for m in ((top.a, top.b) if top.kind in ('conv2', 'ew2', 'bneck2') else (top,)) if m is not None]
+        for op in ops:
+            sc = getattr(op, 'skip_conv', None) if op is not None and op.kind == 'conv' else None
+            if sc is None or not any(o is sc for o in ops) or (op.lane or 0) != (sc.lane or 0):
+                continue
+            if getattr(op, 'w8', None) is not None or getattr(sc, 'w8', None) is not None or sc.bn is not None:
+                continue
+            if _abuf(sc.y) is not _abuf(op.residual) or sc.out_stats is not None:
+                continue
+            y = _abuf(sc.y)
+            if any(o is not op and any(_abuf(t) is y for t in o.acts_in()) for top in readers if top is not None for o in members_of(top)):
+                continue
+            s = self.conv(op, plain=True)[1]
+            self._fill_skip(op, s)
+            if l.fpd_conv_skip_supported(C.byref(s)) == 1:
+                op.skip_active = True
+                sc.skip_fused = True
+
+    def plan_stem_act(self, ops, readers=None):
+        if os.environ.get('FPD_STEM_ACT', '1') == '0':
+            return
+        readers = ops if readers is None else readers
+        members_of = lambda top: [m for m in ((top.a, top.b) if top.kind in ('conv2', 'ew2', 'bneck2') else (top,)) if m is not None]
+        for op in ops:
+            ae = getattr(op, 'act_ew', None) if op is not None and op.kind == 'stem_fwd' else None
+            if ae is None or not any(o is ae for o in ops) or (op.lane or 0) != (ae.lane or 0):
+                continue
+            if ae.op != 'bnrelu_fwd' or ae.bn is None or ae.bn.mode != 'eval' or _abuf(ae.x) is not _abuf(op.y):
+                continue
+            if op.out_stats is not None or ae.out_stats is not None:
+                continue
+            y = _abuf(op.y)
+            if any(o is not ae and any(_abuf(t) is y for t in o.acts_in()) for top in readers if top is not None for o in members_of(top)):
+                continue
+            op.act_active = True
+            ok = R.lib().fpd_stem_act_supported(C.byref(self.stem(op)[1])) == 1
+            op.act_active = ok
+            ae.stem_fused = ok
 
     def _fill_fold(self, op, s):
         if not getattr(op, 'fold_active', False):
@@ -311,6 +365,8 @@
         s.x = p(op.image)
         if op.kind == 'stem_fwd':
             s.w, s.bias, s.y, s.out_stats = p(op.w), p(op.bias), p(_abuf(op.y)), p(op.out_stats)
+            if getattr(op, 'act_active', False):
+                s.act, s.y = self.bn(op.act_ew.bn), p(_abuf(op.act_ew.y))
             return R.OP_STEM_FWD, s
         s.dy, s.dw, s.dbias = p(_abuf(op.dy)), p(op.dw), p(op.dbias)
         s.partial, s.partial_stride = None, 0
@@ -325,6 +381,8 @@
 
     def ew(self, op):
         if getattr(op, 'folded', False):
+            return R.OP_NOP, R.MemsetT()
+        if getattr(op, 'stem_fused', False):
             return R.OP_NOP, R.MemsetT()
         s = R.EwT()
         s.op, s.dtype = _EW[op.op], self.dtype
@@ -454,6 +512,8 @@
                                       num_blocks=cfg.get('num_blocks', 1), wlp_is_master=(self.dtype == R.F32),
                                       fuse_bneck=(self.dtype == R.BF16 and not train and env('FPD_FUSE_BNECK', '1') != '0'),
                                       pair_branches=env('FPD_PAIR', '1') != '0', fuse_head=env('FPD_FUSE_HEAD', '1') != '0',
+                                      fuse_skip=(self.dtype == R.BF16 and env('FPD_FUSE_SKIP', '1') != '0'),
+                                      fuse_stem_act=(self.dtype == R.BF16 and env('FPD_STEM_ACT', '1') != '0'),
                                       wgrad_batch=int(env('FPD_WGRAD_BATCH')) if env('FPD_WGRAD_BATCH') else None)
         self.A = Arenas(state.device, self.dtype, parent=state.A)
         self.low = Lowering(self.A, self.dtype)
@@ -527,6 +587,8 @@
         self.rng['prep'] = (b, len(p))
         b = len(p)
         self.op_index = {}
+        self.low.plan_skips(g.fwd, readers=ops)
+        self.low.plan_stem_act(g.fwd, readers=ops)
         for op in g.fwd:
             self.op_index[id(op)] = p.add(*self.low.op(op))
         self.rng['fwd'] = (b, len(p))
diff --git a/fast-human-pose-estimation.pytorch_amd/graph.py b/fast-human-pose-estimation.pytorch_amd/graph.py
--- a/fast-human-pose-estimation.pytorch_amd/graph.py
+++ b/fast-human-pose-estimation.pytorch_amd/graph.py
@@ -97,6 +97,9 @@
             if fa is not None and getattr(self, 'fold_active', False):
                 rd += [b(fa.x), b(fa.dy), fa.bstats] + bn_bufs(fa.bn)
                 wr += [b(fa.y), fa.dgamma, fa.dbeta]
+            sc = getattr(self, 'skip_conv', None)
+            if sc is not None and getattr(self, 'skip_active', False):
+                rd += [b(sc.x), sc.w, sc.bias]
         elif k == 'head':
             rd = [b(self.y0), b(self.x), self.w_fc, self.b_fc, self.w_score, self.b_score, self.w_fc2, self.b_fc2,
                   self.w_score2, self.b_score2] + bn_bufs(self.bn)
@@ -121,6 +124,10 @@
             rd, wr = [self.region], []
         elif k == 'stem_fwd':
             rd, wr = [self.image, self.w, self.bias], [b(self.y), self.out_stats]
+            ae = getattr(self, 'act_ew', None)
+            if ae is not None and getattr(self, 'act_active', False):
+                rd += bn_bufs(ae.bn)
+                wr += [b(ae.y)]
         elif k == 'stem_wgrad':
             rd, wr = [self.image, b(self.dy)], [self.dw, self.dbias]
         elif k == 'ew':
@@ -137,6 +144,9 @@
             return [t for t in (self.y0, self.x) if t is not None]
         fa = getattr(self, 'fold_apply', None)
         folded = [t for t in (fa.x, fa.dy) if isinstance(t, Act)] if fa is not None else []
+        sc = getattr(self, 'skip_conv', None)
+        if sc is not None and isinstance(sc.x, Act):
+            folded = folded + [sc.x]
         return [getattr(self, f) for f in ('x', 'x2', 'dy', 'add', 'residual', 'epi_x') if
                 isinstance(getattr(self, f, None), Act)] + [a for a in getattr(self, 'extra_in', []) if a is not None] + folded
 
@@ -145,8 +155,9 @@
             return self.a.acts_out() + self.b.acts_out()
         if self.kind == 'head':
             return [t for t in (self.score, self.next) if t is not None]
+        ae = getattr(self, 'act_ew', None)
         return [getattr(self, f) for f in ('y',) if isinstance(getattr(self, f, None), Act)] + \
-               [a for a in getattr(self, 'extra_out', []) if a is not None]
+               [a for a in getattr(self, 'extra_out', []) if a is not None] + ([ae.y] if ae is not None else [])
 
 
 class ParamTable:
@@ -281,7 +292,8 @@
 class HourglassGraph:
 
     def __init__(self, params, num_feats, num_stacks, num_joints, batch, height, width, train, num_blocks=1,
-                 depth=4, wlp_is_master=True, lane_levels=None, wgrad_batch=None, fuse_bneck=False, pair_branches=True, fuse_head=True):
+                 depth=4, wlp_is_master=True, lane_levels=None, wgrad_batch=None, fuse_bneck=False, pair_branches=True, fuse_head=True,
+                 fuse_skip=False, fuse_stem_act=False):
         self.p = params
         self.F, self.S, self.J = num_feats, num_stacks, num_joints
         self.N, self.H, self.W = batch, height, width
@@ -290,6 +302,7 @@
         self.fuse_bneck = fuse_bneck and not train
         self.fuse_head = fuse_head and self.fuse_bneck
         self.pair_branches = pair_branches
+        self.fuse_skip, self.fuse_stem_act = fuse_skip, fuse_stem_act and not train
         self._pair_op = None
         self._pair_ew = None
         self.stats_size = 0
@@ -426,7 +439,10 @@
         if (p + 'downsample.0.weight') in self.p.entries:
             assert sink is None
             skip = self.conv(x, p + 'downsample.0')
-        return self.conv(t, p + 'conv3', bn=self._bn(p + 'bn3', planes), residual=skip, sink=sink)
+        y = self.conv(t, p + 'conv3', bn=self._bn(p + 'bn3', planes), residual=skip, sink=sink)
+        if skip is not x and getattr(self, 'fuse_skip', False):
+            y.producer.skip_conv = skip.producer
+        return y
 
     def _fused(self, x, p):
         planes = self.p[p + 'conv1.weight'].shape[0]
@@ -490,6 +506,8 @@
         bn1 = self._bn('bn1', K)
         self._use_bn(x, bn1)
         x = self.ew('bnrelu_fwd', x.shape, x.shape, 'stem_act', x=x, bn=bn1)
+        if bn1.mode == 'eval' and self.fuse_stem_act:
+            op.act_ew = x.producer
         x = self.residual_seq(x, 'layer1.', 1)
         x = self.maxpool(x, 'pool1')
         x = self.residual_seq(x, 'layer2.', 1)
diff --git a/fast-human-pose-estimation.pytorch_amd/runtime.py b/fast-human-pose-estimation.pytorch_amd/runtime.py
--- a/fast-human-pose-estimation.pytorch_amd/runtime.py
+++ b/fast-human-pose-estimation.pytorch_amd/runtime.py
@@ -31,7 +31,8 @@
                 ('_pad', _i32), ('x', _vp), ('w', _vp), ('bias', _vp), ('residual', _vp), ('y', _vp),
                 ('out_stats', _vp), ('bn', BnT), ('epi_x', _vp), ('epi_bn', BnT), ('epi_stats', _vp),
                 ('wg_partial', _vp), ('wg_stride', _i64), ('wg_bias', _i32), ('wg_count', _i32),
-                ('fold_x', _vp), ('fold_bn', BnT), ('fold_stats', _vp), ('fold_out', _vp), ('fold_dgamma', _vp), ('fold_dbeta', _vp)]
+                ('fold_x', _vp), ('fold_bn', BnT), ('fold_stats', _vp), ('fold_out', _vp), ('fold_dgamma', _vp), ('fold_dbeta', _vp),
+                ('x2', _vp), ('w2', _vp), ('bias2', _vp), ('C2', _i32), ('_pad2', _i32)]
 
 
 class ConvF8T(C.Structure):
@@ -65,7 +66,7 @@
 class StemT(C.Structure):
     _fields_ = [('N', _i32), ('H', _i32), ('W', _i32), ('K', _i32), ('P', _i32), ('Q', _i32), ('dtype', _i32),
                 ('_pad', _i32), ('x', _vp), ('w', _vp), ('bias', _vp), ('y', _vp), ('out_stats', _vp), ('dy', _vp),
-                ('dw', _vp), ('dbias', _vp), ('partial', _vp), ('partial_stride', _i64)]
+                ('dw', _vp), ('dbias', _vp), ('partial', _vp), ('partial_stride', _i64), ('act', BnT)]
 
 
 class EwT(C.Structure):
@@ -193,6 +194,8 @@
     'fpd_conv_fused_wgrad_partials': (C.c_int, [C.POINTER(ConvT)]),
     'fpd_conv_fold_supported': (C.c_int, [_vp]),
     'fpd_conv_pair_fold_supported': (C.c_int, [_vp]),
+    'fpd_conv_skip_supported': (C.c_int, [_vp]),
+    'fpd_stem_act_supported': (C.c_int, [_vp]),
     'fpd_conv_pair_fused_wgrad_partials': (C.c_int, [C.POINTER(ConvPairT), C.POINTER(C.c_int32), C.POINTER(C.c_int32)]),
     'fpd_conv_wgrad': (C.c_int, [C.POINTER(WgradT), _vp]),
     'fpd_wgrad_num_partials': (C.c_int, [C.POINTER(WgradT)]),
diff --git a/include/fpd_amd.h b/include/fpd_amd.h
--- a/include/fpd_amd.h
+++ b/include/fpd_amd.h
@@ -60,6 +60,11 @@
     void* fold_out;
     float* fold_dgamma;
     float* fold_dbeta;
+    const void* x2;
+    const void* w2;
+    const float* bias2;
+    int32_t C2;
+    int32_t _pad2;
 } fpd_conv_t;
 
 typedef struct {
@@ -125,6 +130,7 @@
     float* dbias;
     float* partial;
     int64_t partial_stride;
+    fpd_bn_t act;
 } fpd_stem_t;
 
 enum {
@@ -232,11 +238,13 @@
 int fpd_conv_fused_wgrad_partials(const fpd_conv_t* a);
 int fpd_conv_fold_supported(const fpd_conv_t* a);
 int fpd_conv_pair_fold_supported(const fpd_conv_pair_t* p);
+int fpd_conv_skip_supported(const fpd_conv_t* a);
 int fpd_conv_pair_fused_wgrad_partials(const fpd_conv_pair_t* p, int32_t* n_a, int32_t* n_b);
 int fpd_conv_wgrad(const fpd_wgrad_t* a, fpd_stream_t stream);
 int fpd_wgrad_num_partials(const fpd_wgrad_t* a);
 int fpd_wgrad_reduce(const fpd_wreduce_entry_t* table_dev, int32_t n_entries, int64_t max_elems, fpd_stream_t stream);
 int fpd_stem_forward(const fpd_stem_t* a, fpd_stream_t stream);
+int fpd_stem_act_supported(const fpd_stem_t* a);
 int fpd_stem_wgrad(const fpd_stem_t* a, fpd_stream_t stream);
 int fpd_stem_wgrad_num_partials(const fpd_stem_t* a);
 int fpd_elementwise(const fpd_ew_t* a, fpd_stream_t stream);
```
